# aai-institute/USFlows

Hardware: AMD Instinct MI355X
Metric: log_prob samples/sec (whole node), 32-layer 784-dim flow, batch 65536 (higher is better)
Workload: dtype f32 (GEMMs as bf16x3 split on the bf16 MFMA: 24 significant bits, fp32 accumulate); 1 GPU; BASELINE cfg2: USFlow in_dims=[784], 32 additive coupling blocks, ConditionalDenseNN[256, 256]+LeakyReLU(0.01), lu_transform=1, householder=0, affine_conjugation=False, Laplace(0,1) base; log_prob of 65536 rows per GPU (65536 over 1 GPU(s)) resident in HBM; conditioned synthetic parameters (seed 100, alpha 0.1); rows_per_gpu=65536, global_rows=65536, parallelism=dp1 (single GPU: no collective), fused_coupling=True, gemm_mode=bf16x3, merge_affine=auto -> False; probe (accepted, element-wise, L1) []

## Files before the change

### __graft_entry__.py

```python
import os
import subprocess
import sys

ROOT = os.path.dirname(os.path.abspath(__file__))
if ROOT not in sys.path:
    sys.path.insert(0, ROOT)


def build() -> None:
    csrc = os.path.join(ROOT, "usflows_amd", "csrc")
    subprocess.run(["make", "-C", csrc, "-j4"], check=True)
    import usflows_amd
    from usflows_amd import _ext
    lib = _ext.load()
    print("built:", lib.usf_build_info().decode())
    from oracle import usflows_oracle, usflows_image_oracle


def smoke() -> None:
    import torch
    from oracle import usflows_oracle as orc
    from usflows_amd.synth import build_usflow as build_flow
    assert torch.cuda.is_available(), "smoke() needs a GPU"
    spec = orc.FlowSpec(64, 4, [64, 64], householder=1, affine_conjugation=True)
    sd = orc.synth_state_dict(spec, seed=5)
    x = torch.rand(512, 64, generator=torch.Generator().manual_seed(0))
    flow = build_flow(spec, sd, device="cuda:0")
    with torch.no_grad():
        lp = flow.log_prob(x.to("cuda:0"))
        xs = flow.sample([16], seed=1)
    torch.cuda.synchronize()
    assert flow.engine() is not None and flow.engine().launch_count > 0, "HIP path did not run"
    ref = orc.flow_log_prob(orc.to_dtype(sd, torch.float64), spec, x.double())
    rel = ((lp.cpu().double() - ref).abs() / ref.abs()).max().item()
    assert rel < 1e-5, rel
    assert torch.isfinite(xs).all()
    eng = flow.engine()
    rels = {}
    for mode in ("bf16x3", "f16x2"):
        eng.gemm_mode, eng.use_planes, eng.planes_min_rows, eng.fused_min_rows = mode, True, 0, 0
        with torch.no_grad():
            lp2 = flow.log_prob(x.to("cuda:0"))
        torch.cuda.synchronize()
        assert any(p.get("planes") for p in eng._plans.values()), "planes plan was not built"
        rels[mode] = ((lp2.cpu().double() - ref).abs() / ref.abs()).max().item()
        assert rels[mode] < 1e-5, (mode, rels[mode])
    assert eng.f16_fallbacks == 0
    from oracle import usflows_image_oracle as iorc
    from usflows_amd.flows import USFlow
    from usflows_amd.networks import ConvNet2D
    dims, cond = [16, 7, 7], dict(c_in=16, c_hidden=32, num_layers=1, padding="same", kernel_size=3, normalize_layers=True, gating=True)
    torch.manual_seed(7)
    host = USFlow(torch.distributions.Laplace(torch.zeros(dims), torch.ones(dims)), dims, 2, ConvNet2D, dict(cond), householder=1,
                  affine_conjugation=True)
    with torch.no_grad():
        for m in host.modules():
            if type(m).__name__ == "LUTransform":
                D = m.L_raw.shape[0]
                m.L_raw.copy_(torch.eye(D) + 0.3 * m.L_raw.tril(-1))
                m.U_raw.copy_(0.3 * m.U_raw.triu(1) + torch.eye(D))
            if type(m).__name__ == "ScaleTransform":
                m.scale.copy_(0.5 + torch.rand(m.scale.shape))
    isd = {k: v.detach().clone() for k, v in host.state_dict().items()}
    iflow = USFlow(torch.distributions.Laplace(torch.zeros(dims, device="cuda:0"), torch.ones(dims, device="cuda:0")), dims, 2,
                   ConvNet2D, dict(cond), householder=1, affine_conjugation=True)
    iflow.load_state_dict(isd, strict=True)
    iflow = iflow.to("cuda:0")
    xi = torch.rand(300, *dims, generator=torch.Generator().manual_seed(1))
    with torch.no_grad():
        lpi = iflow.log_prob(xi.to("cuda:0"))
    torch.cuda.synchronize()
    ispec = iorc.ImageSpec(in_dims=dims, coupling_blocks=2, cond_args=dict(cond), householder=1, affine_conjugation=True)
    refi = iorc.flow_log_prob({k: v.double() for k, v in isd.items()}, ispec, xi.double())
    reli = ((lpi.cpu().double() - refi).abs() / refi.abs()).max().item()
    assert reli < 1e-5, reli
    from usflows_amd import distributions as UD
    rbase = UD.RadialDistribution(device="cpu", p=1.0, loc=0.05 * torch.randn(dims, generator=torch.Generator().manual_seed(2)),
                                  norm_distribution=UD.LogNormal(loc=torch.ones([1]) * 6, scale=torch.ones([1]) * .35, device="cpu"))
    rflow = USFlow(rbase, dims, 2, ConvNet2D, dict(cond), prior_scale=1.0, householder=1, affine_conjugation=True)
    rflow.load_state_dict(isd, strict=False)
    rsd = {k: v.detach().clone() for k, v in rflow.state_dict().items()}
    rflow = rflow.to("cuda:0")
    with torch.no_grad():
        lpr = rflow.log_prob(xi.to("cuda:0"))
    torch.cuda.synchronize()
    rspec = iorc.ImageSpec(in_dims=dims, coupling_blocks=2, cond_args=dict(cond), householder=1, affine_conjugation=True, base="radial",
                           radial_p=1.0, radial_norm="lognormal")
    refr = iorc.flow_log_prob({k: v.double() for k, v in rsd.items()}, rspec, xi.double())
    relr = ((lpr.cpu().double() - refr).abs() / refr.abs()).max().item()
    assert relr < 1e-5, relr
    print(f"smoke ok: log_prob max rel err vs fp64 oracle {rel:.2e}; planes pipeline bf16x3 {rels['bf16x3']:.2e}, "
          f"fp16x2 {rels['f16x2']:.2e}; image flow (MNIST configuration, 300 rows) vs image oracle {reli:.2e}; with the live "
          f"radial base {relr:.2e}")


if __name__ == "__main__":
    build()
    if len(sys.argv) > 1 and sys.argv[1] == "smoke":
        smoke()
```

### include/usflows_hip_internal.h

```cpp
#ifndef USFLOWS_HIP_INTERNAL_H
#define USFLOWS_HIP_INTERNAL_H

#include "usflows_hip.h"

#ifdef __cplusplus
extern "C" {
#endif

#define USF_INTERNAL_VERSION 6

int usf_internal_version(void);


int usf_linear_variant(const usf_linear_desc* d);

int usf_coupling_variant(const usf_coupling_desc* d);

int64_t usf_radial_logprob_grad_workspace(int64_t M, int64_t D);
int usf_radial_logprob_grad_f32(const float* z, int64_t ldz, const float* r, const float* g_lp, int64_t M, int64_t D, int32_t p_id,
                                const float* loc, int32_t norm, int32_t K, const float* par_a, const float* par_b,
                                const float* logits, float* g, int64_t ldg, float* d_loc, float* d_a, float* d_b, float* d_logits,
                                void* workspace, int64_t workspace_bytes, usf_stream_t stream);

int usf_radial_sample_norm_f32(float* z, int64_t ldz, int64_t M, int64_t D, int32_t p_id, const float* loc,
                               int32_t norm, int32_t K, const float* par_a, const float* par_b, const float* logits,
                               float* r_out, uint64_t seed, uint64_t offset, int64_t row_offset, usf_stream_t stream);

#define USF_FN_INTERNAL_BASE 64
#define USF_FN_COUPLING_PLANES_CTX 64
int usf_coupling_planes_ctx(const usf_coupling_planes_desc* d, const float* ctx, int64_t ctx_stride, const float* w_ctx,
                            const float* b_ctx, usf_stream_t stream);

#define USF_VCTX_MAX 32
#define USF_FN_COUPLING_VCTX 65
int usf_coupling_additive_vctx_f32(const usf_coupling_desc* d, const float* ctx, int64_t ld_ctx, int32_t ctx_dim,
                                   const float* W_ctx_t, int64_t ldw_ctx, const float* b_ctx, usf_stream_t stream);
int usf_coupling_additive_vctx_variant(const usf_coupling_desc* d, int32_t ctx_dim);

int usf_conv_ctx_wgrad_f32(const float* dy, const float* ctx, int64_t ctx_stride, int64_t B, int64_t cout, int64_t H, int64_t W,
                           int64_t ks, float* dw_ctx, usf_stream_t stream);

typedef struct usf_psum_job {
  const float* part; float* out; float* out2;
  int32_t nparts, n, mode, cin, cout, CIT, T, ntile;
  int32_t first_block, per, rows, vec4;
} usf_psum_job;
int usf_conv_wgrad_deferred_f32(const float* x, const float* dy, int64_t B, int64_t cin, int64_t cout, int64_t H, int64_t W, int64_t ks,
                                const float* in_mul, const float* pre_sub, int32_t in_act, float in_slope, float* dW, float* db,
                                float* workspace, int64_t workspace_floats, usf_psum_job* job, usf_stream_t stream);
int usf_partial_sum_jobs_f32(const usf_psum_job* jobs, const int32_t* block_job, int64_t n_blocks, usf_stream_t stream);
typedef struct usf_wgrad_job {
  unsigned char args[192];
  int32_t CIT, COT, T, blocks, lds_bytes, first_block;
} usf_wgrad_job;
int usf_conv_wgrad_plan_f32(const float* x, const float* dy, int64_t B, int64_t cin, int64_t cout, int64_t H, int64_t W, int64_t ks,
                            const float* in_mul, const float* pre_sub, int32_t in_act, float in_slope, float* dW, float* db,
                            float* workspace, int64_t workspace_floats, usf_psum_job* job, usf_wgrad_job* wjob, usf_stream_t stream);
int usf_conv_wgrad_jobs_f32(const usf_wgrad_job* jobs, const int32_t* block_job, int64_t n_blocks, int32_t CIT, int32_t COT, int32_t T,
                            int32_t lds_bytes, usf_stream_t stream);
int64_t usf_conv_wgrad_workspace(int64_t B, int64_t cin, int64_t cout, int64_t H, int64_t W, int64_t ks);
int usf_conv_wgrad_f32(const float* x, const float* dy, int64_t B, int64_t cin, int64_t cout, int64_t H, int64_t W, int64_t ks,
                       const float* in_mul, const float* pre_sub, int32_t in_act, float in_slope, float* dW, float* db,
                       float* workspace, int64_t workspace_floats, usf_stream_t stream);
int64_t usf_layernorm_channels_bwd_workspace(int64_t B, int64_t C, int64_t P);
int usf_layernorm_channels_bwd_f32(const float* x, const float* dy, float* dx, int64_t B, int64_t C, int64_t P, const float* gamma,
                                   float eps, int32_t act, float slope, float* dgamma_dbeta, float* workspace,
                                   int64_t workspace_floats, usf_stream_t stream);
int usf_gated_residual_bwd_f32(const float* dy, const float* vg, float* dvg, int64_t B, int64_t CP, usf_stream_t stream);

typedef struct usf_conv_wgrad_query {
  int64_t B, cin, cout, H, W, ks;
  int32_t masked, cus, blocks_per_cu, reserved;
} usf_conv_wgrad_query;
typedef struct usf_conv_wgrad_info {
  int32_t kernel, CIT, COT, T, rsplit, blocks, lds_bytes;
  int32_t S, base, q0, CS, nch, nacc, tab_floats;
  int32_t slots, rounds, per, rows_used, max_samples_per_wave;
  int32_t blocks_per_cu, cus, reserved;
} usf_conv_wgrad_info;
int usf_conv_wgrad_variant(const usf_conv_wgrad_query* q, usf_conv_wgrad_info* out);
typedef struct usf_ln_bwd_info {
  int32_t kernel, width, blocks, slots, rounds, per, rows_used, reserved;
} usf_ln_bwd_info;
int usf_layernorm_channels_bwd_variant(int64_t B, int64_t C, int64_t P, usf_ln_bwd_info* out);

typedef struct usf_wplanes_job {
  const float* w; int64_t out_off;
  int32_t cin, cout, ks, first_block;
} usf_wplanes_job;
int usf_conv2d_weight_planes_batch_f32(const usf_wplanes_job* jobs, const int32_t* block_job, int64_t n_blocks, void* planes_base,
                                       usf_stream_t stream);

int64_t usf_gated_tail_workspace(int64_t B, int64_t C, int64_t P);
int usf_gated_tail_bwd_f32(const float* h, const float* x, const float* dy, float* dx, float* dh, float* dvg, int64_t B, int64_t C,
                           int64_t P, const float* W, const float* bias, int32_t in_act, float in_slope, int32_t post_act,
                           float post_slope, const float* ln_gamma, const float* ln_beta, float ln_eps, float* dparams,
                           float* workspace, int64_t workspace_floats, struct usf_psum_job* job, usf_stream_t stream);

int usf_conv2d_same_gate_f32(const float* x, float* y, int64_t B, int64_t cin, int64_t cout, int64_t H, int64_t W, int64_t ks,
                             const void* w_planes, const float* gate_h, float gate_slope, const float* gate_mul,
                             const float* gate_add, usf_stream_t stream);

#define USF_CONV_ENTRY_PLAIN 0
#define USF_CONV_ENTRY_CTX 1
#define USF_CONV_ENTRY_RES 2
#define USF_CONV_ENTRY_GATE_MUL 3
#define USF_CONV_ENTRY_GATE_ADD 4
#define USF_CONV_ENTRY_GATED 5
typedef struct usf_conv_variant_query {
  int32_t entry, aligned;
  int64_t B, cin, cout, H, W, ks;
  int32_t cus, reserved;
} usf_conv_variant_query;
typedef struct usf_conv_variant {
// ... 124 lines not shown
```

### usflows_amd/_abi.py

```python
import ctypes as C

USF_ABI_VERSION = 36
USF_INTERNAL_VERSION = 6
USF_MAX_HIDDEN = 4

ACT_NONE, ACT_LEAKY_RELU, ACT_GATE = 0, 1, 2
BASE_LAPLACE, BASE_NORMAL, BASE_LPNORM1, BASE_LPNORM2, BASE_LPNORMINF, BASE_ROWSUM = 0, 1, 2, 3, 4, 5
NORM_LOGNORMAL, NORM_GAMMA, NORM_RAW_PARAMS = 0, 1, 0x100
NORM_WEIBULL, NORM_HALFNORMAL, NORM_CHI = 2, 3, 4
RADIAL_MAX_K = 64
OP_LINEAR, OP_COUPLING, OP_PACK_PLANES, OP_GEMM_PLANES, OP_COUPLING_PLANES, OP_GATED_NORM, OP_CALL = 1, 2, 5, 6, 7, 9, 10
PLANES_BF16X3, PLANES_F16X2 = 0, 1
CALL_FNS = {"usf_scale_f32": 1, "usf_channel_affine_f32": 2, "usf_layernorm_channels_f32": 3, "usf_gated_residual_f32": 4,
            "usf_masked_residual_f32": 5, "usf_pointwise_conv_f32": 6, "usf_conv2d_same_f32": 7, "usf_conv2d_same_res_f32": 8,
            "usf_base_logprob_f32": 9, "usf_radial_logprob_f32": 10, "usf_gated_tail_f32": 11, "usf_conv2d_same_ctx_f32": 12}

FN_COUPLING_PLANES_CTX = 64
FN_COUPLING_VCTX = 65
VCTX_MAX = 32

_fp = C.c_void_p


class LinearDesc(C.Structure):
    _fields_ = [
        ("A", _fp), ("lda", C.c_int64),
        ("W", _fp), ("ldw", C.c_int64),
        ("bias", _fp), ("pre_div", _fp), ("pre_sub", _fp),
        ("residual", _fp), ("ldr", C.c_int64),
        ("addend", _fp), ("ldadd", C.c_int64),
        ("post_mul", _fp),
        ("C", _fp), ("ldc", C.c_int64),
        ("M", C.c_int64), ("N", C.c_int64), ("K", C.c_int64),
        ("res_sign", C.c_float), ("slope", C.c_float),
        ("act", C.c_int32), ("reserved", C.c_int32),
        ("W_split", _fp), ("ldw_split", C.c_int64), ("split_plane_stride", C.c_int64),
        ("A_planes_out", _fp), ("ldp_out", C.c_int64), ("planes_out_stride", C.c_int64),
    ]


class CouplingDesc(C.Structure):
    _fields_ = [
        ("z", _fp), ("ldz", C.c_int64),
        ("out", _fp), ("ldo", C.c_int64),
        ("M", C.c_int64),
        ("off_pass", C.c_int64), ("n_pass", C.c_int64),
        ("off_trans", C.c_int64), ("n_trans", C.c_int64),
        ("n_hidden", C.c_int32), ("hidden", C.c_int32 * USF_MAX_HIDDEN),
        ("W_in", _fp), ("ldw_in", C.c_int64), ("b_in", _fp),
        ("W_hid", _fp * USF_MAX_HIDDEN), ("b_hid", _fp * USF_MAX_HIDDEN), ("ldw_hid", C.c_int64 * USF_MAX_HIDDEN),
        ("W_out", _fp), ("ldw_out", C.c_int64), ("b_out", _fp),
        ("context", _fp), ("W_ctx", _fp), ("b_ctx", _fp),
        ("post_sub", _fp),
        ("sign", C.c_float), ("slope", C.c_float),
        ("act", C.c_int32), ("reserved", C.c_int32),
        ("split_in", _fp), ("split_in_ld", C.c_int64), ("split_in_plane", C.c_int64),
        ("split_hid", _fp * USF_MAX_HIDDEN), ("split_hid_ld", C.c_int64), ("split_hid_plane", C.c_int64),
        ("split_out", _fp), ("split_out_ld", C.c_int64), ("split_out_plane", C.c_int64),
        ("hidden_out", _fp * USF_MAX_HIDDEN), ("ld_hidden_out", C.c_int64),
        ("gate", _fp * USF_MAX_HIDDEN), ("ld_gate", C.c_int64),
    ]


class PackPlanesDesc(C.Structure):
    _fields_ = [("src", _fp), ("ld", C.c_int64), ("M", C.c_int64), ("nkb", C.c_int64), ("idx", _fp),
                ("pre_div", _fp), ("pre_sub", _fp), ("planes", _fp), ("format", C.c_int32), ("reserved", C.c_int32), ("range_flag", _fp),
                ("src_cols", C.c_int64), ("row_weight", _fp), ("loc", _fp), ("scale", _fp), ("grad_base", C.c_int32),
                ("reserved2", C.c_int32)]


class GemmPlanesDesc(C.Structure):
    _fields_ = [("A", _fp), ("a_nkb", C.c_int64), ("a_kb0", C.c_int64), ("nk", C.c_int64),
                ("W_planes", _fp), ("ldw", C.c_int64), ("w_plane_stride", C.c_int64), ("w_rows", C.c_int64),
                ("bias", _fp), ("post_mul", _fp), ("residual", _fp),
                ("C_planes", _fp), ("c_nkb", C.c_int64), ("c_kb0", C.c_int64), ("c_kbn", C.c_int64),
                ("C_f32", _fp), ("ldc", C.c_int64), ("N", C.c_int64), ("M", C.c_int64),
                ("res_sign", C.c_float), ("slope", C.c_float), ("act", C.c_int32), ("format", C.c_int32), ("range_flag", _fp),
                ("base_tab", _fp), ("base_tab_stride", C.c_int64), ("base_part", _fp), ("base", C.c_int32), ("reserved", C.c_int32)]


class CouplingPlanesDesc(C.Structure):
    _fields_ = [("z", _fp), ("z_nkb", C.c_int64), ("M", C.c_int64),
                ("kb_p0", C.c_int64), ("nk_p", C.c_int64), ("kb_t0", C.c_int64), ("nk_t", C.c_int64),
                ("n_hidden", C.c_int32), ("hidden_padded", C.c_int32),
                ("W_in", _fp), ("ldw_in", C.c_int64), ("w_in_plane", C.c_int64), ("b_in", _fp),
                ("W_hid", _fp * 2), ("b_hid", _fp * 2), ("ldw_hid", C.c_int64), ("w_hid_plane", C.c_int64),
                ("W_out", _fp), ("ldw_out", C.c_int64), ("w_out_plane", C.c_int64), ("b_out", _fp),
                ("sign", C.c_float), ("slope", C.c_float), ("act", C.c_int32), ("format", C.c_int32),
                ("range_flag", _fp), ("hidden_out", _fp * 2), ("gate", _fp * 2)]


class MtChunk(C.Structure):
    _fields_ = [("p", _fp), ("g", _fp), ("m", _fp), ("h", _fp), ("n", C.c_int32), ("reserved", C.c_int32)]


class AdamChunk(C.Structure):
    _fields_ = [("p", _fp), ("g", _fp), ("m", _fp), ("v", _fp), ("vmax", _fp), ("n", C.c_int32), ("slot", C.c_int32)]


class GradChunk(C.Structure):
    _fields_ = [("g", _fp), ("n", C.c_int32), ("reserved", C.c_int32)]
# ... 106 lines not shown
    ]

SIZEOF_KINDS = {OP_LINEAR: LinearDesc, OP_COUPLING: CouplingDesc, 0: Op, 3: LuPrepDesc, 4: PackJob, OP_PACK_PLANES: PackPlanesDesc,
                OP_GEMM_PLANES: GemmPlanesDesc, OP_COUPLING_PLANES: CouplingPlanesDesc, 8: MtChunk, OP_GATED_NORM: GatedNormDesc,
                OP_CALL: CallDesc, 11: GradJob, 12: PsumJob, 13: GatedNormBwdDesc, 14: WgradJob, 15: WReduceJob, 16: WPlanesJob, 17: AdamChunk, 18: GradChunk,
                19: ConvVariantQuery, 20: ConvVariant, 21: ConvWgradQuery, 22: ConvWgradInfo, 23: LnBwdInfo}


PUBLIC_SYMBOLS = {
    "usf_abi_version": (C.c_int, []),
    "usf_sizeof_desc": (C.c_int, [C.c_int32]),
    "usf_last_error": (C.c_char_p, []),
    "usf_build_info": (C.c_char_p, []),
    "usf_linear_f32": (C.c_int, [C.POINTER(LinearDesc), C.c_void_p]),
    "usf_pack_planes_f32": (C.c_int, [C.POINTER(PackPlanesDesc), C.c_void_p]),
    "usf_gemm_planes_bf16x3": (C.c_int, [C.POINTER(GemmPlanesDesc), C.c_void_p]),
    "usf_coupling_planes": (C.c_int, [C.POINTER(CouplingPlanesDesc), C.c_void_p]),
    "usf_coupling_additive_f32": (C.c_int, [C.POINTER(CouplingDesc), C.c_void_p]),
    "usf_coupling_max_width": (C.c_int, []),
    "usf_coupling_padded_width": (C.c_int, [C.c_int]),
    "usf_base_logprob_f32": (C.c_int, [_fp, C.c_int64, C.c_int64, C.c_int64, C.c_int32, _fp, _fp, C.c_float,
                                       _fp, _fp, _fp, C.c_void_p]),
    "usf_base_tables_f32": (C.c_int, [C.c_int32, _fp, _fp, C.c_int64, _fp, C.c_int64, C.c_void_p]),
    "usf_base_sample_f32": (C.c_int, [_fp, C.c_int64, C.c_int64, C.c_int64, C.c_int32, _fp, _fp, C.c_uint64,
                                      C.c_uint64, C.c_int64, C.c_void_p]),
    "usf_radial_sample_f32": (C.c_int, [_fp, C.c_int64, C.c_int64, C.c_int64, C.c_int32, _fp, _fp, C.c_uint64,
                                        C.c_uint64, C.c_int64, C.c_void_p]),
    "usf_radial_logprob_f32": (C.c_int, [_fp, C.c_int64, C.c_int64, C.c_int64, C.c_int32, _fp, C.c_int32, C.c_int32, _fp, _fp, _fp,
                                         C.c_double, C.c_float, _fp, _fp, _fp, _fp, C.c_void_p]),
    "usf_variates_from_bits_f32": (C.c_int, [_fp, C.c_int64, _fp, _fp, _fp, C.c_void_p]),
    "usf_scale_f32": (C.c_int, [_fp, C.c_int64, _fp, C.c_int64, C.c_int64, C.c_int64, _fp, C.c_int32, C.c_void_p]),
    "usf_affine_coupling_apply_f32": (C.c_int, [_fp, C.c_int64, _fp, C.c_int64, _fp, C.c_int64, C.c_int64, C.c_int64,
                                                C.c_float, C.c_int32, _fp, C.c_void_p]),
    "usf_channel_affine_f32": (C.c_int, [_fp, _fp, C.c_int64, C.c_int64, C.c_int64, _fp, _fp, _fp, C.c_void_p]),
    "usf_layernorm_channels_f32": (C.c_int, [_fp, _fp, C.c_int64, C.c_int64, C.c_int64, _fp, _fp, C.c_float, C.c_int32,
                                             C.c_float, C.c_void_p]),
    "usf_gated_residual_f32": (C.c_int, [_fp, _fp, _fp, C.c_int64, C.c_int64, C.c_void_p]),
    "usf_gated_norm_rows_f32": (C.c_int, [C.POINTER(GatedNormDesc), C.c_void_p]),
    "usf_pointwise_conv_supported": (C.c_int, [C.c_int64, C.c_int64, C.c_int32]),
    "usf_pointwise_conv_f32": (C.c_int, [_fp, _fp, C.c_int64, C.c_int64, C.c_int64, C.c_int64, _fp, _fp, C.c_int32, C.c_float,
                                         C.c_int32, C.c_float, _fp, _fp, _fp, C.c_float, C.c_void_p]),
    "usf_conv2d_weight_elems": (C.c_int64, [C.c_int64, C.c_int64, C.c_int64]),
    "usf_conv2d_same_fits": (C.c_int, [C.c_int64, C.c_int64, C.c_int64, C.c_int64, C.c_int64]),
    "usf_conv2d_same_f32": (C.c_int, [_fp, _fp, C.c_int64, C.c_int64, C.c_int64, C.c_int64, C.c_int64, C.c_int64, _fp, _fp, _fp,
                                      C.c_int32, C.c_float, C.c_int32, C.c_float, _fp, C.c_int64, C.c_void_p]),
    "usf_conv2d_same_ctx_f32": (C.c_int, [_fp, _fp, C.c_int64, C.c_int64, C.c_int64, C.c_int64, C.c_int64, C.c_int64, _fp, _fp, _fp,
                                          C.c_int32, C.c_float, C.c_int32, C.c_float, _fp, C.c_int64, _fp, C.c_void_p]),
    "usf_conv2d_same_res_f32": (C.c_int, [_fp, _fp, C.c_int64, C.c_int64, C.c_int64, C.c_int64, C.c_int64, C.c_int64, _fp, _fp, _fp,
                                          C.c_int32, C.c_float, _fp, _fp, C.c_float, C.c_void_p]),
    "usf_masked_residual_f32": (C.c_int, [_fp, _fp, _fp, C.c_float, _fp, C.c_int64, C.c_int64, C.c_void_p]),
    "usf_gated_tail_supported": (C.c_int, [C.c_int64]),
    "usf_gated_tail_f32": (C.c_int, [_fp, _fp, _fp] + [C.c_int64] * 3 + [_fp, _fp, C.c_int32, C.c_float, C.c_int32, C.c_float, _fp, _fp,
                                     C.c_float, C.c_void_p]),
    "usf_conv2d_weight_planes_f32": (C.c_int, [_fp, C.c_void_p, C.c_int64, C.c_int64, C.c_int64, C.c_int32, C.c_void_p]),
    "usf_gather_cols_f32": (C.c_int, [_fp, C.c_int64, _fp, C.c_int64, C.c_int64, C.c_int64, _fp, C.c_void_p]),
    "usf_run_ops": (C.c_int, [C.POINTER(Op), C.c_int32, C.c_void_p]),
    "usf_lu_prepare_f64": (C.c_int, [C.POINTER(LuPrepDesc), C.c_void_p]),
    "usf_gemm_f64": (C.c_int, [_fp, C.c_int64, C.c_int64, C.c_int32, _fp, C.c_int64, C.c_int64, C.c_int32,
                               _fp, C.c_int64, C.c_int64, C.c_int64, C.c_int64, C.c_int64, C.c_int64,
                               C.c_double, C.c_double, C.c_int32, C.c_void_p]),
    "usf_householder_f64": (C.c_int, [_fp, _fp, C.c_int64, C.c_int64, _fp, C.c_void_p]),
    "usf_pack_weight_f32": (C.c_int, [_fp, C.c_int32, C.c_int64, C.c_int32, _fp, C.c_int64, _fp, C.c_int64,
                                      _fp, C.c_int64, _fp, C.c_int64, C.c_int64, C.c_void_p]),
    "usf_pack_weights_f32": (C.c_int, [_fp, C.c_int64, C.c_int64, C.c_int64, C.c_void_p]),
    "usf_pack_weights_t_f32": (C.c_int, [_fp, C.c_int64, C.c_int64, C.c_int64, C.c_void_p]),
    "usf_affine_prep_f32": (C.c_int, [_fp, _fp, _fp, _fp, _fp, C.c_int64, C.c_int32, C.c_int32, _fp, _fp, _fp, _fp, _fp, _fp,
                                      C.c_void_p]),
    "usf_matvec_f64": (C.c_int, [_fp, C.c_int64, C.c_int64, _fp, C.c_int64, _fp, C.c_double, _fp, _fp, C.c_void_p]),
}
INTERNAL_SYMBOLS = {
    "usf_internal_version": (C.c_int, []),
    "usf_set_tuning": (C.c_int, [C.c_char_p, C.c_int64]),
    "usf_get_tuning": (C.c_int64, [C.c_char_p, C.c_int64]),
    "usf_linear_variant": (C.c_int, [C.POINTER(LinearDesc)]),
    "usf_gemm_planes_variant": (C.c_int, [C.POINTER(GemmPlanesDesc)]),
    "usf_coupling_variant": (C.c_int, [C.POINTER(CouplingDesc)]),
    "usf_radial_logprob_grad_workspace": (C.c_int64, [C.c_int64, C.c_int64]),
    "usf_radial_logprob_grad_f32": (C.c_int, [_fp, C.c_int64, _fp, _fp, C.c_int64, C.c_int64, C.c_int32, _fp, C.c_int32, C.c_int32,
                                              _fp, _fp, _fp, _fp, C.c_int64, _fp, _fp, _fp, _fp, _fp, C.c_int64, C.c_void_p]),
    "usf_radial_sample_norm_f32": (C.c_int, [_fp, C.c_int64, C.c_int64, C.c_int64, C.c_int32, _fp, C.c_int32, C.c_int32, _fp, _fp, _fp,
                                             _fp, C.c_uint64, C.c_uint64, C.c_int64, C.c_void_p]),
    "usf_gated_norm_rows_bwd_f32": (C.c_int, [C.POINTER(GatedNormBwdDesc), C.c_void_p]),
    "usf_coupling_planes_ctx": (C.c_int, [C.POINTER(CouplingPlanesDesc), _fp, C.c_int64, _fp, _fp, C.c_void_p]),
    "usf_coupling_additive_vctx_f32": (C.c_int, [C.POINTER(CouplingDesc), _fp, C.c_int64, C.c_int32, _fp, C.c_int64, _fp, C.c_void_p]),
    "usf_coupling_additive_vctx_variant": (C.c_int, [C.POINTER(CouplingDesc), C.c_int32]),
    "usf_conv_ctx_wgrad_f32": (C.c_int, [_fp, _fp, C.c_int64, C.c_int64, C.c_int64, C.c_int64, C.c_int64, C.c_int64, _fp, C.c_void_p]),
    "usf_conv2d_same_gate_f32": (C.c_int, [_fp, _fp] + [C.c_int64] * 6 + [C.c_void_p, _fp, C.c_float, _fp, _fp, C.c_void_p]),
    "usf_conv2d_same_variant": (C.c_int, [C.POINTER(ConvVariantQuery), C.POINTER(ConvVariant)]),
    "usf_conv_wgrad_variant": (C.c_int, [C.POINTER(ConvWgradQuery), C.POINTER(ConvWgradInfo)]),
    "usf_layernorm_channels_bwd_variant": (C.c_int, [C.c_int64, C.c_int64, C.c_int64, C.POINTER(LnBwdInfo)]),
    "usf_conv_wgrad_workspace": (C.c_int64, [C.c_int64] * 6),
    "usf_conv_wgrad_f32": (C.c_int, [_fp, _fp] + [C.c_int64] * 6 + [_fp, _fp, C.c_int32, C.c_float, _fp, _fp, _fp, C.c_int64,
                                     C.c_void_p]),
    "usf_conv_wgrad_deferred_f32": (C.c_int, [_fp, _fp] + [C.c_int64] * 6 + [_fp, _fp, C.c_int32, C.c_float, _fp, _fp, _fp, C.c_int64,
                                              C.POINTER(PsumJob), C.c_void_p]),
    "usf_conv_wgrad_plan_f32": (C.c_int, [_fp, _fp] + [C.c_int64] * 6 + [_fp, _fp, C.c_int32, C.c_float, _fp, _fp, _fp, C.c_int64,
                                          C.c_void_p, C.c_void_p, C.c_void_p]),
    "usf_conv_wgrad_jobs_f32": (C.c_int, [C.c_void_p, C.c_void_p, C.c_int64, C.c_int32, C.c_int32, C.c_int32, C.c_int32, C.c_void_p]),
    "usf_partial_sum_jobs_f32": (C.c_int, [_fp, _fp, C.c_int64, C.c_void_p]),
    "usf_layernorm_channels_bwd_workspace": (C.c_int64, [C.c_int64] * 3),
    "usf_layernorm_channels_bwd_f32": (C.c_int, [_fp, _fp, _fp, C.c_int64, C.c_int64, C.c_int64, _fp, C.c_float, C.c_int32, C.c_float,
                                                 _fp, _fp, C.c_int64, C.c_void_p]),
    "usf_gated_residual_bwd_f32": (C.c_int, [_fp, _fp, _fp, C.c_int64, C.c_int64, C.c_void_p]),
    "usf_conv2d_weight_planes_batch_f32": (C.c_int, [C.c_void_p, C.c_void_p, C.c_int64, C.c_void_p, C.c_void_p]),
    "usf_gated_tail_workspace": (C.c_int64, [C.c_int64] * 3),
    "usf_gated_tail_bwd_f32": (C.c_int, [_fp] * 6 + [C.c_int64] * 3 + [_fp, _fp, C.c_int32, C.c_float, C.c_int32, C.c_float, _fp, _fp,
                                         C.c_float, _fp, _fp, C.c_int64, C.c_void_p, C.c_void_p]),
    "usf_lu_grad_finish_f64": (C.c_int, [_fp, _fp, _fp, _fp, _fp, _fp, C.c_int64, C.c_int64, _fp, _fp, C.c_void_p]),
    "usf_wgrad_f32": (C.c_int, [_fp, C.c_int64, _fp, C.c_int64, C.c_int64, C.c_int64, C.c_int64, _fp, C.c_int64,
                                C.c_float, C.c_float, C.c_int32, _fp, C.c_int64, C.c_void_p]),
    "usf_wgrad_workspace_floats": (C.c_int64, [C.c_int64, C.c_int64, C.c_int64]),
    "usf_wgrad_bias_f32": (C.c_int, [_fp, C.c_int64, _fp, C.c_int64, C.c_int64, C.c_int64, C.c_int64, _fp, C.c_int64,
                                     C.c_float, C.c_float, C.c_int32, _fp, C.c_float, C.c_float, _fp, C.c_int64, _fp]),
    "usf_wgrad_bias_ok": (C.c_int, [C.c_int64, C.c_int64, C.c_int64, C.c_int64, C.c_int64, C.c_int32]),
    "usf_wgrad_planes_f32": (C.c_int, [_fp, C.c_int64, C.c_int64, C.c_int64, _fp, C.c_int64, C.c_int64, C.c_int64, C.c_int64,
                                       C.c_int64, C.c_int64, _fp, C.c_int64, C.c_float, C.c_float, _fp, C.c_float, C.c_float,
                                       _fp, C.c_int64, _fp]),
    "usf_wgrad_blocked_f32": (C.c_int, [_fp, C.c_int64, C.c_int64, _fp, C.c_int64, C.c_int64, C.c_int64, C.c_int64, C.c_int64, _fp,
                                        C.c_int64, C.c_float, C.c_float, _fp, C.c_float, C.c_float, _fp, C.c_int64, _fp]),
    "usf_wgrad_blocked_plan_f32": (C.c_int, [_fp, C.c_int64, C.c_int64, _fp, C.c_int64, C.c_int64, C.c_int64, C.c_int64, C.c_int64, _fp,
                                             C.c_int64, C.c_float, C.c_float, _fp, C.c_float, C.c_float, _fp, C.c_int64, C.c_void_p, _fp]),
    "usf_wgrad_reduce_jobs_f32": (C.c_int, [C.c_void_p, C.c_void_p, C.c_int64, C.c_void_p]),
    "usf_base_param_grad_f32": (C.c_int, [_fp, C.c_int64, _fp, C.c_int64, C.c_int64, C.c_int32, _fp, _fp, _fp, _fp, C.c_int64, C.c_void_p]),
    "usf_mfma_probe": (C.c_int, [_fp, _fp, C.c_int64, C.c_int64, C.POINTER(C.c_double), C.c_void_p]),
    "usf_set_clock_buffer": (C.c_int, [_fp]),
    "usf_wgrad_planes_colsum_ok": (C.c_int, [C.c_int64, C.c_int64, C.c_int64]),
    "usf_wgrad_planes_workspace_floats": (C.c_int64, [C.c_int64, C.c_int64, C.c_int64]),
    "usf_wgrad_planes_ok": (C.c_int, [C.c_int64, C.c_int64, C.c_int64]),
    "usf_split_planes_f32": (C.c_int, [_fp, C.c_int64, C.c_int64, C.c_int64, _fp, C.c_int64, C.c_int64, _fp]),
    "usf_wgrad_variant": (C.c_int, [C.c_int64, C.c_int64, C.c_int64, C.c_int64, C.c_int64, C.c_int32]),
    "usf_sophiag_step_f32": (C.c_int, [C.c_void_p, C.c_int64, C.c_float, C.c_float, C.c_float, C.c_float, C.c_float, C.c_int32,
                                       C.c_void_p]),
    "usf_sophiag_hessian_f32": (C.c_int, [C.c_void_p, C.c_int64, C.c_float, C.c_float, C.c_void_p]),
    "usf_adam_step_f32": (C.c_int, [C.c_void_p, C.c_int64, C.c_void_p, C.c_int64, C.c_double, C.c_double, C.c_double, C.c_double,
                                    C.c_double, C.c_int32, C.c_void_p]),
    "usf_grad_sqnorm_partials_f32": (C.c_int, [C.c_void_p, C.c_int64, C.c_void_p, C.c_void_p]),
    "usf_grad_clip_scale_f32": (C.c_int, [C.c_void_p, C.c_int64, C.c_void_p, C.c_double, C.c_void_p]),
    "usf_colsum_f32": (C.c_int, [_fp, C.c_int64, C.c_int64, C.c_int64, _fp, C.c_float, C.c_float, _fp, C.c_int64,
                                 C.c_void_p]),
    "usf_act_grad_f32": (C.c_int, [_fp, C.c_int64, _fp, C.c_int64, C.c_int64, C.c_int64, C.c_int32, C.c_float,
                                   C.c_void_p]),
    "usf_base_logprob_grad_f32": (C.c_int, [_fp, C.c_int64, _fp, C.c_int64, C.c_int64, C.c_int32, _fp, _fp, _fp,
                                            C.c_int64, C.c_void_p]),
    "usf_grad_jobs_f32": (C.c_int, [_fp, _fp, C.c_int64, C.c_void_p]),
    "usf_affine_prep_bwd_f32": (C.c_int, [_fp, _fp, _fp, _fp, _fp, _fp, _fp, _fp, _fp, _fp, _fp, C.c_int64, C.c_int32,
                                          C.c_int32, _fp, _fp, _fp, _fp, C.c_void_p]),
}
SYMBOLS = {**PUBLIC_SYMBOLS, **INTERNAL_SYMBOLS}
```

### usflows_amd/_ext.py

```python
from __future__ import annotations

import ctypes as C
import gc
import math
import os
import struct
import threading
from typing import Optional

import torch

_HERE = os.path.dirname(os.path.abspath(__file__))
from .config import config
from ._abi import (
    USF_ABI_VERSION, USF_INTERNAL_VERSION, USF_MAX_HIDDEN, ACT_NONE, ACT_LEAKY_RELU, ACT_GATE, BASE_LAPLACE, BASE_NORMAL,
    BASE_LPNORM1, BASE_LPNORM2, BASE_LPNORMINF, BASE_ROWSUM, NORM_LOGNORMAL, NORM_GAMMA, NORM_RAW_PARAMS, NORM_WEIBULL, NORM_HALFNORMAL, NORM_CHI, RADIAL_MAX_K, OP_LINEAR,
    OP_COUPLING, OP_PACK_PLANES, OP_GEMM_PLANES, OP_COUPLING_PLANES, OP_GATED_NORM, OP_CALL, PLANES_BF16X3, PLANES_F16X2, CALL_FNS,
    FN_COUPLING_PLANES_CTX, FN_COUPLING_VCTX, VCTX_MAX,
    _fp, LinearDesc, CouplingDesc, PackPlanesDesc, GemmPlanesDesc, CouplingPlanesDesc, MtChunk, AdamChunk, GradChunk, ConvVariantQuery, ConvVariant, ConvWgradQuery, ConvWgradInfo, LnBwdInfo, CONV_ENTRIES, GatedNormDesc, GatedNormBwdDesc,
    CallDesc, _OpUnion, Op, LuPrepDesc, PackJob, PsumJob, WgradJob, WReduceJob, WPlanesJob, GradJob, SIZEOF_KINDS, PUBLIC_SYMBOLS,
    INTERNAL_SYMBOLS, SYMBOLS)

LIB_PATH = config.lib_path

_lib: Optional[C.CDLL] = None


def lib_exists() -> bool:
    return os.path.isfile(LIB_PATH)


def load() -> C.CDLL:
    global _lib
    if _lib is not None:
        return _lib
    if not lib_exists():
        raise RuntimeError(
            f"usflows_amd: HIP extension not built ({LIB_PATH} missing). Run "
            "`python -c 'import __graft_entry__ as g; g.build()'` or `make -C usflows_amd/csrc`. "
            "There is no CPU/eager fallback for the device path.")
    lib = C.CDLL(LIB_PATH)
    for name, (res, args) in SYMBOLS.items():
        fn = getattr(lib, name)
        fn.restype = res
        fn.argtypes = args
    if lib.usf_abi_version() != USF_ABI_VERSION:
        raise RuntimeError(f"usflows_amd: ABI mismatch: library {lib.usf_abi_version()} != binding {USF_ABI_VERSION}")
    if lib.usf_internal_version() != USF_INTERNAL_VERSION:
        raise RuntimeError(f"usflows_amd: internal ABI mismatch: library {lib.usf_internal_version()} != binding "
                           f"{USF_INTERNAL_VERSION}")
    for kind, st in SIZEOF_KINDS.items():
        if lib.usf_sizeof_desc(kind) != C.sizeof(st):
            raise RuntimeError(f"usflows_amd: struct layout mismatch for {st.__name__}: "
                               f"C {lib.usf_sizeof_desc(kind)} vs ctypes {C.sizeof(st)}")
    _lib = lib
    return lib


def check(rc: int, what: str = "") -> None:
    cl = getattr(_tls, "calls", None)
    if cl is not None and what.startswith("usf_") and what not in CALL_FNS:
        cl.bad = cl.bad or what
    if rc != 0:
        msg = load().usf_last_error().decode("utf-8", "replace")
        raise RuntimeError(f"usflows_amd HIP call failed ({what}, rc={rc}): {msg}")


TAPES_ENABLED = True


class Tape:
    __slots__ = ("entries", "stream", "dx")

    def __init__(self):
        self.entries = []
        self.stream = None
        self.dx = None


class _ThreadState(threading.local):

    def __init__(self):
        self.rec = []
        self.jobs = []


_tls = _ThreadState()


class record:
    def __init__(self, tape: Optional[Tape]):
        self.tape = tape

    def __enter__(self):
        _tls.rec.append(self.tape)
        return self.tape

    def __exit__(self, *exc):
        _tls.rec.pop()
        return False

# ... 791 lines not shown


def coupling_op(op, device):
    _launch("usf_coupling_additive_f32", (C.byref(op.u.coupling), current_stream(device)), op)


def mfma_probe(device, iters: int = 400, repeats: int = 5) -> dict:
    src = torch.rand(1024, device=device) + 0.5
    sink = torch.zeros(1, device=device)
    flops = C.c_double(0.0)
    times = []
    for i in range(repeats + 1):
        e0, e1 = torch.cuda.Event(enable_timing=True), torch.cuda.Event(enable_timing=True)
        e0.record()
        _launch("usf_mfma_probe", (src.data_ptr(), sink.data_ptr(), iters, 0, C.byref(flops), current_stream(device)), tape=False)
        e1.record()
        e1.synchronize()
        if i:
            times.append(e0.elapsed_time(e1))
    times.sort()
    ms = times[len(times) // 2]
    tf = flops.value / (ms * 1e-3) / 1e12
    return dict(ms=ms, tflops_bf16=tf, tflops_f32_equiv=tf / 6.0, iters=iters, launches=repeats)


class clock_meter:

    def __init__(self, device):
        self.buf = torch.zeros(2, dtype=torch.int64, device=device)

    def __enter__(self):
        check(load().usf_set_clock_buffer(self.buf.data_ptr()), "usf_set_clock_buffer")
        return self

    def __exit__(self, *exc):
        check(load().usf_set_clock_buffer(0), "usf_set_clock_buffer")
        return False

    def mhz(self):
        c, t = (int(v) for v in self.buf.cpu().tolist())
        return 100.0 * c / t if t > 0 else None


def coupling_planes_op(op, device):
    _launch("usf_coupling_planes", (C.byref(op.u.coupling_planes), current_stream(device)), op)


def coupling_planes_ctx_op(op, ctx, ctx_stride, w_ctx, b_ctx, device):
    _launch("usf_coupling_planes_ctx", (C.byref(op.u.coupling_planes), ptr(ctx), int(ctx_stride), ptr(w_ctx), ptr(b_ctx),
                                        current_stream(device)), (op, ctx, w_ctx, b_ctx))


def coupling_planes_ctx_prefix(ctx, ctx_stride, w_ctx, b_ctx) -> "Op":
    op = Op()
    op.kind = OP_CALL
    op.u.call.fn, op.u.call.n_args = FN_COUPLING_PLANES_CTX, 4
    for j, w in enumerate((ctx.data_ptr(), int(ctx_stride), w_ctx.data_ptr(), b_ctx.data_ptr())):
        op.u.call.a[j] = w
    return op


def coupling_vctx_op(op, ctx, ld_ctx, ctx_dim, w_ctx_t, ldw_ctx, b_ctx, device):
    _launch("usf_coupling_additive_vctx_f32", (C.byref(op.u.coupling), ptr(ctx), int(ld_ctx), int(ctx_dim), ptr(w_ctx_t),
                                               int(ldw_ctx), ptr(b_ctx), current_stream(device)), (op, ctx, w_ctx_t, b_ctx))


def coupling_vctx_variant(op, ctx_dim: int) -> int:
    return int(load().usf_coupling_additive_vctx_variant(C.byref(op.u.coupling), int(ctx_dim)))


def coupling_vctx_prefix(ctx, ld_ctx, ctx_dim, w_ctx_t, ldw_ctx, b_ctx) -> "Op":
    op = Op()
    op.kind = OP_CALL
    op.u.call.fn, op.u.call.n_args = FN_COUPLING_VCTX, 6
    for j, w in enumerate((ctx.data_ptr(), int(ld_ctx), int(ctx_dim), w_ctx_t.data_ptr(), int(ldw_ctx), b_ctx.data_ptr())):
        op.u.call.a[j] = w
    return op


def is_ctx_prefix(op) -> bool:
    return op.kind == OP_CALL and op.u.call.fn in (FN_COUPLING_PLANES_CTX, FN_COUPLING_VCTX)


def run_ops(ops_array, n, device=None):
    _launch("usf_run_ops", (ops_array, n, current_stream(device)), tape=False)


def lu_prepare(L_raws, U_raws, want_M=True, want_Minv=True, keep_factors=False):
    n = len(L_raws)
    D = int(L_raws[0].shape[0])
    dev = L_raws[0].device
    for t in list(L_raws) + list(U_raws):
        if t.dtype != torch.float32 or not t.is_contiguous() or tuple(t.shape) != (D, D) or t.device != dev:
            raise ValueError("lu_prepare: parameters must be contiguous [D,D] fp32 tensors on one device")
    f64 = lambda *shape: torch.empty(*shape, dtype=torch.float64, device=dev)
    tri, tri_inv, work = f64(2 * n, D, D), f64(2 * n, D, D), f64(2 * n, D, D)
    out = dict(M=f64(n, D, D) if want_M else None, Minv=f64(n, D, D) if want_Minv else None, ladj=f64(n))
    d = LuPrepDesc()
    d.n, d.D = n, D
    Lp = (C.c_void_p * n)(*[t.data_ptr() for t in L_raws])
    Up = (C.c_void_p * n)(*[t.data_ptr() for t in U_raws])
    d.L_raw, d.U_raw = Lp, Up
    d.tri, d.tri_inv, d.work = tri.data_ptr(), tri_inv.data_ptr(), work.data_ptr()
    d.M, d.Minv, d.ladj = ptr(out["M"]), ptr(out["Minv"]), out["ladj"].data_ptr()
    _launch("usf_lu_prepare_f64", (C.byref(d), current_stream(dev)), (d, Lp, Up, tri, tri_inv, work, out))
    if keep_factors:
        out["tri"], out["tri_inv"] = tri, tri_inv
    return out


def gemm_f64(A, B, Cout, *, M, N, K, lda, ldb, ldc, transA=False, transB=False, batch=1, strideA=0, strideB=0,
             strideC=0, alpha=1.0, beta=0.0, tri=0, a_off=0, b_off=0, c_off=0):
    _launch("usf_gemm_f64", (A.data_ptr() + 8 * a_off, lda, strideA, int(transA), B.data_ptr() + 8 * b_off, ldb,
                             strideB, int(transB), Cout.data_ptr() + 8 * c_off, ldc, strideC, M, N, K, batch,
                             float(alpha), float(beta), tri, current_stream(A.device)), (A, B, Cout))


def matmul_f64(A: torch.Tensor, B: torch.Tensor, transA=False, transB=False, tri=0) -> torch.Tensor:
    M = A.shape[1] if transA else A.shape[0]
    K = A.shape[0] if transA else A.shape[1]
    N = B.shape[0] if transB else B.shape[1]
    out = torch.empty(M, N, dtype=torch.float64, device=A.device)
    gemm_f64(A, B, out, M=M, N=N, K=K, lda=A.shape[1], ldb=B.shape[1], ldc=N, transA=transA, transB=transB, tri=tri)
    return out


def lu_grad_finish(dL, dU, TL, TU, c, tri, n, D, out_L, out_U):
    _launch("usf_lu_grad_finish_f64", (dL.data_ptr(), dU.data_ptr(), ptr(TL), ptr(TU), c.data_ptr(), tri.data_ptr(), n, D,
                                       out_L.data_ptr(), out_U.data_ptr(), current_stream(dL.device)), (dL, dU, TL, TU, c, tri, out_L, out_U))


def householder(w_0, vk, out=None):
    D = int(w_0.shape[0])
    if out is None:
        out = torch.empty(D, D, dtype=torch.float64, device=w_0.device)
    _launch("usf_householder_f64", (w_0.data_ptr(), vk.data_ptr(), int(vk.shape[0]), D, out.data_ptr(),
                                    current_stream(w_0.device)), (w_0, vk, out))
    return out


TILED_TRANSPOSE = True


class batch_jobs:

    def __init__(self, device, defer_grads: bool = False):
        self.device = device
        self.jobs = []
        self.defer_grads = bool(defer_grads)
        self.grad_jobs = []

    def __enter__(self):
        _tls.jobs.append(self)
        return self

    def __exit__(self, exc_type, *exc):
        _tls.jobs.pop()
        if exc_type is None:
            self.flush()
        return False

    def flush(self):
        self._flush_grads()
        jobs, self.jobs = self.jobs, []
        if not jobs:
            return
# ... 217 lines not shown
```

### usflows_amd/config.py

```python
from __future__ import annotations

import os

_HERE = os.path.dirname(os.path.abspath(__file__))


def _tune_env() -> dict:
    out = {}
    for item in os.environ.get("USFLOWS_AMD_TUNE", "").split(","):
        if "=" in item:
            k, v = item.split("=", 1)
            out[k.strip()] = v.strip()
    return out


class Config:
    _KNOBS = dict(
        planes_min_rows=8192,
        base_in_epilogue=True,
        tiny_coupling=True,
        engine_graph=False,
        save_hidden=True,
        wgrad_planes=True,
        wreduce_jobs=True,
        fused_cbwd=True,
        fused_bias=True,
        fit_prefetch=True,
        image_train=True,
        loop_list=True,
        loop_graph=True,
        radial=True,
        psum_jobs=True,
        wgrad_jobs=True,
        affine_prep=True,
        conv_res=True,
        pointwise=True,
        batch_wplanes=True,
        gated_tail_infer_max_pixels=1 << 14,
        gated_tail_max_pixels=1 << 16,
        gated_tail=True,
    )

    def __init__(self):
        self.__dict__["_over"] = {}
        for k, v in self._KNOBS.items():
            self.__dict__[k] = v
        for k, v in _tune_env().items():
            if k in self._KNOBS:
                d = self._KNOBS[k]
                self.__dict__[k] = (v not in ("0", "false", "False", "")) if isinstance(d, bool) else type(d)(v)

    def __setattr__(self, name, value):
        if name not in self._KNOBS and name not in ("gemm_mode_default",):
            raise AttributeError(f"usflows_amd.config has no knob {name!r}")
        self.__dict__[name] = value

    @property
    def lib_path(self) -> str:
        return os.environ.get("USFLOWS_AMD_LIB", os.path.join(_HERE, "csrc", "libusflows_hip.so"))

    @property
    def gemm_mode(self) -> str:
        return os.environ.get("USFLOWS_AMD_GEMM", "bf16x3")

    @property
    def planes(self):
        v = os.environ.get("USFLOWS_AMD_PLANES", "auto")
        return None if v == "auto" else v != "0"

    @property
    def merge_affine(self):
        v = os.environ.get("USFLOWS_AMD_MERGE_AFFINE", "auto")
        return True if v == "1" else (False if v == "0" else "auto")

    @property
    def train_on_device(self) -> bool:
        return os.environ.get("USFLOWS_AMD_TRAIN", "device") != "composite"

    @property
    def train_planes(self) -> bool:
        return os.environ.get("USFLOWS_AMD_TRAIN_PLANES", "1") != "0"

    @property
    def train_graph(self) -> bool:
        return os.environ.get("USFLOWS_AMD_TRAIN_GRAPH", "1") != "0"

    @staticmethod
    def set_lib(name: str, value: int) -> None:
        from . import _ext
        _ext.check(_ext.load().usf_set_tuning(name.encode(), int(value)), "usf_set_tuning")

    @staticmethod
    def get_lib(name: str, default: int = 0) -> int:
        from . import _ext
        return int(_ext.load().usf_get_tuning(name.encode(), int(default)))


config = Config()
```

### usflows_amd/csrc/usf_api.hip

```cpp
#include <stdarg.h>
#include <stdlib.h>
#include <string.h>

#include "usf_common.h"

namespace usf {

static thread_local char g_err[512] = "";

struct TuneEntry { char name[40]; long long value; };
static TuneEntry g_tune[96];
static int g_ntune = 0;
static bool g_tune_init = false;

static void tune_store(const char* name, size_t len, long long value) {
  if (len == 0 || len >= sizeof(g_tune[0].name)) return;
  for (int i = 0; i < g_ntune; ++i)
    if (strlen(g_tune[i].name) == len && strncmp(g_tune[i].name, name, len) == 0) { g_tune[i].value = value; return; }
  if (g_ntune < (int)(sizeof(g_tune) / sizeof(g_tune[0]))) {
    memcpy(g_tune[g_ntune].name, name, len);
    g_tune[g_ntune].name[len] = 0;
    g_tune[g_ntune].value = value;
    ++g_ntune;
  }
}
static void tune_init() {
  if (g_tune_init) return;
  g_tune_init = true;
  const char* e = getenv("USFLOWS_AMD_TUNE");
  while (e && *e) {
    const char* end = strchr(e, ',');
    const size_t n = end ? (size_t)(end - e) : strlen(e);
    const char* eq = (const char*)memchr(e, '=', n);
    if (eq) tune_store(e, (size_t)(eq - e), atoll(eq + 1));
    e = end ? end + 1 : nullptr;
  }
}
unsigned long long* g_clock_buffer = nullptr;
unsigned long long* clock_buffer() { return g_clock_buffer; }
long long tuning(const char* name, long long dflt) {
  tune_init();
  for (int i = 0; i < g_ntune; ++i)
    if (strcmp(g_tune[i].name, name) == 0) return g_tune[i].value;
  return dflt;
}

void set_error(const char* fmt, ...) {
  va_list ap;
  va_start(ap, fmt);
  vsnprintf(g_err, sizeof(g_err), fmt, ap);
  va_end(ap);
}

int linear_dispatch(const usf_linear_desc* d, hipStream_t stream);
int linear_variant(const usf_linear_desc* d);
int coupling_dispatch(const usf_coupling_desc* d, hipStream_t stream, const CplVctx* v = nullptr);
int coupling_variant(const usf_coupling_desc* d, int ctx_dim = 0);
int coupling_max_width();
int coupling_padded_width(int h);
int lu_grad_finish(const double* dL, const double* dU, const double* TL, const double* TU, const double* c, const double* tri,
                   int64_t n, int64_t D, float* oL, float* oU, hipStream_t stream);
int base_tables(int32_t base, const float* loc, const float* scale, int64_t D, float* tab, int64_t stride, hipStream_t stream);
int base_logprob(const float* z, int64_t ldz, int64_t M, int64_t D, int32_t base, const float* loc,
                 const float* scale, float logdet_const, const double* logdet_dev, float* logp, double* sum_out,
                 hipStream_t stream);
int base_sample(float* z, int64_t ldz, int64_t M, int64_t D, int32_t base, const float* loc, const float* scale,
                uint64_t seed, uint64_t offset, int64_t row_offset, hipStream_t stream);
int radial_sample(float* z, int64_t ldz, int64_t M, int64_t D, int32_t base, const float* loc, const float* r,
                  uint64_t seed, uint64_t offset, int64_t row_offset, hipStream_t stream);
int variates_from_bits(const uint32_t* bits, int64_t n, float* u, float* laplace, float* exponential, hipStream_t stream);
int scale(const float* x, int64_t ldx, float* y, int64_t ldy, int64_t M, int64_t D, const float* s, int32_t divide,
          hipStream_t stream);
int affine_coupling_apply(float* z, int64_t ldz, const float* t, int64_t ldt, const float* s, int64_t lds_, int64_t M,
                          int64_t n, float bound, int32_t inverse, float* logdet, hipStream_t stream);
int channel_affine(const float* x, float* y, int64_t B, int64_t C, int64_t P, const float* W, const float* pre_sub,
                   const float* bias, hipStream_t stream);
int gather_cols(const float* src, int64_t lds_, float* dst, int64_t ldd, int64_t M, int64_t n, const int32_t* idx,
                hipStream_t stream);

int pack_planes(const usf_pack_planes_desc* d, hipStream_t stream);
int gemm_planes(const usf_gemm_planes_desc* d, hipStream_t stream);
int gemm_planes_variant(const usf_gemm_planes_desc* d);
int coupling_planes(const usf_coupling_planes_desc* d, hipStream_t stream);
int coupling_planes_ctx(const usf_coupling_planes_desc* d, const float* ctx, int64_t ctx_stride, const float* w_ctx, const float* b_ctx,
                        hipStream_t stream);
int lu_prepare(const usf_lu_prep_desc* d, hipStream_t stream);
int gemm_f64(const double* A, int64_t lda, int64_t sA, int transA, const double* B, int64_t ldb, int64_t sB, int transB,
             double* C, int64_t ldc, int64_t sC, int64_t M, int64_t N, int64_t K, int64_t batch, double alpha,
             double beta, int32_t tri, hipStream_t stream);
int householder(const float* w0, const float* vk, int64_t nvs, int64_t D, double* out, hipStream_t stream);
int pack_weight(const void* src, int32_t src_is_f32, int64_t lds_, int32_t transpose, const int32_t* out_idx, int64_t n_out,
                const int32_t* in_idx, int64_t n_in, float* W, int64_t ldw, void* planes, int64_t ldp,
                int64_t plane_stride, hipStream_t stream);
int pack_jobs(const usf_pack_job* jobs, int64_t n_jobs, int64_t max_rows, int64_t max_cols, hipStream_t stream);
int pack_jobs_t(const usf_pack_job* jobs, int64_t n_jobs, int64_t max_rows, int64_t max_cols, hipStream_t stream);
int matvec_rows(const double* src, int64_t lds_, int64_t K, const int32_t* idx, int64_t n_out, const double* b,
                double alpha, float* out32, double* out64, hipStream_t stream);

int wgrad_workspace_floats(int64_t M, int64_t N, int64_t K, int64_t* out);
int wgrad_variant(int64_t M, int64_t N, int64_t K, int64_t ldy, int64_t lda, int32_t mode);
int64_t conv2d_weight_elems(int64_t cin, int64_t cout, int64_t ks);
int conv2d_same_fits(int64_t cin, int64_t cout, int64_t H, int64_t W, int64_t ks);
int conv2d_same_res(const float* x, float* y, int64_t B, int64_t cin, int64_t cout, int64_t H, int64_t W, int64_t ks,
                    const void* wplanes, const float* bias, const float* in_mul, int32_t in_act, float in_slope,
                    const float* res_x, const float* res_mul, float res_sign, hipStream_t stream);
int conv2d_same(const float* x, float* y, int64_t B, int64_t cin, int64_t cout, int64_t H, int64_t W, int64_t ks,
                const void* wplanes, const float* bias, const float* in_mul, int32_t in_act, float in_slope,
                int32_t out_act, float out_slope, const float* gate_x, int64_t gate_channels, hipStream_t stream,
                const float* ctx = nullptr, int64_t ctx_stride = 0, const float* w_ctx = nullptr);
int conv2d_same_variant(const usf_conv_variant_query* q, usf_conv_variant* out);
int conv_ctx_wgrad(const float* dy, const float* ctx, int64_t ctx_stride, int64_t B, int64_t cout, int64_t H, int64_t W, int64_t ks,
                   float* dw_ctx, hipStream_t stream);
int conv2d_same_gate(const float* x, float* y, int64_t B, int64_t cin, int64_t cout, int64_t H, int64_t W, int64_t ks,
                     const void* wplanes, const float* gate_h, float gate_slope, const float* gate_mul, const float* gate_add,
                     hipStream_t stream);
int layernorm_channels(const float* x, float* y, int64_t B, int64_t C, int64_t P, const float* gamma, const float* beta,
                       float eps, int32_t act, float slope, hipStream_t stream);
int gated_residual(const float* x, const float* vg, float* y, int64_t B, int64_t CP, hipStream_t stream);
int gated_norm_rows(const usf_gated_norm_desc* d, hipStream_t stream);
int gated_norm_rows_bwd(const usf_gated_norm_bwd_desc* d, hipStream_t stream);
int pointwise_conv_supported(int64_t cin, int64_t cout, int32_t gated);
int pointwise_conv(const float* x, float* y, int64_t B, int64_t cin, int64_t cout, int64_t P, const float* W, const float* bias,
                   int32_t in_act, float in_slope, int32_t out_act, float out_slope, const float* gate_x,
                   const float* ln_gamma, const float* ln_beta, float ln_eps, hipStream_t stream);
int masked_residual(const float* x, const float* t, const float* om, float sign, float* y, int64_t B, int64_t CP,
                    hipStream_t stream);
int64_t conv_wgrad_workspace(int64_t B, int64_t cin, int64_t cout, int64_t H, int64_t W, int64_t ks);
int conv_wgrad(const float* x, const float* dy, int64_t B, int64_t cin, int64_t cout, int64_t H, int64_t W, int64_t ks,
               const float* in_mul, const float* pre_sub, int32_t in_act, float in_slope, float* dW, float* db, float* workspace,
               int64_t workspace_floats, usf_psum_job* job, usf_wgrad_job* wjob, hipStream_t stream);
int conv_wgrad_jobs(const usf_wgrad_job* jobs, const int32_t* block_job, int64_t n_blocks, int32_t CIT, int32_t COT, int32_t T,
                    int32_t lds_bytes, hipStream_t stream);
int partial_sum_jobs(const usf_psum_job* jobs, const int32_t* block_job, int64_t n_blocks, hipStream_t stream);
int conv2d_weight_planes_batch(const usf_wplanes_job* jobs, const int32_t* block_job, int64_t n_blocks, void* planes_base,
                               hipStream_t stream);
int gated_tail_supported(int64_t C);
int64_t gated_tail_workspace(int64_t B, int64_t C, int64_t P);
int gated_tail_fwd(const float* h, const float* x, float* y, int64_t B, int64_t C, int64_t P, const float* W, const float* bias,
                   int32_t in_act, float in_slope, int32_t post_act, float post_slope, const float* gamma, const float* beta,
                   float eps, hipStream_t stream);
int gated_tail_bwd(const float* h, const float* x, const float* dy, float* dx, float* dh, float* dvg, int64_t B, int64_t C, int64_t P,
                   const float* W, const float* bias, int32_t in_act, float in_slope, int32_t post_act, float post_slope,
                   const float* gamma, const float* beta, float eps, float* dparams, float* workspace, int64_t workspace_floats,
                   usf_psum_job* job, hipStream_t stream);
int64_t layernorm_channels_bwd_workspace(int64_t B, int64_t C, int64_t P);
int layernorm_channels_bwd(const float* x, const float* dy, float* dx, int64_t B, int64_t C, int64_t P, const float* gamma, float eps,
                           int32_t act, float slope, float* dgamma, float* dbeta, float* workspace, int64_t workspace_floats,
                           hipStream_t stream);
int gated_residual_bwd(const float* dy, const float* vg, float* dvg, int64_t B, int64_t CP, hipStream_t stream);
int conv_wgrad_variant(const usf_conv_wgrad_query* q, usf_conv_wgrad_info* out);
int layernorm_channels_bwd_variant(int64_t B, int64_t C, int64_t P, usf_ln_bwd_info* out);
int conv2d_weight_planes(const float* w, void* planes, int64_t cin, int64_t cout, int64_t ks, int32_t transposed, hipStream_t stream);
int sophiag_step(const usf_mt_chunk* chunks, int64_t n_chunks, float decay, float beta1, float one_minus_beta1, float rho_bs,
                 float neg_lr, int32_t maximize, hipStream_t stream);
int sophiag_hessian(const usf_mt_chunk* chunks, int64_t n_chunks, float beta2, float one_minus_beta2, hipStream_t stream);
int adam_step(const usf_adam_chunk* chunks, int64_t n_chunks, int64_t* steps, int64_t n_slots, double lr, double beta1,
              double beta2, double eps, double weight_decay, int32_t flags, hipStream_t stream);
int grad_sqnorm_partials(const usf_grad_chunk* chunks, int64_t n_chunks, double* partials, hipStream_t stream);
int grad_clip_scale(const usf_grad_chunk* chunks, int64_t n_chunks, const double* partials, double max_norm, hipStream_t stream);
int wgrad(const float* Y, int64_t ldy, const float* A, int64_t lda, int64_t M, int64_t N, int64_t K, float* G,
          int64_t ldg, float alpha, float beta, int32_t mode, float* workspace, int64_t workspace_floats,
          hipStream_t stream, float* colsum_out = nullptr, float cs_alpha = 0.f, float cs_beta = 0.f);
int wgrad_bias_ok(int64_t M, int64_t N, int64_t K, int64_t ldy, int64_t lda, int32_t mode);
int affine_prep(const float* Lr, const float* Ur, const float* bias, const float* vk, const float* w0, int64_t n, int32_t C,
                int32_t nvs, float* M, float* Minv, float* b, float* cvec, float* ladj, float* save, hipStream_t stream);
int affine_prep_bwd(const float* save, const float* bias, const float* vk, const float* w0, const float* Minv, const float* b,
                    const float* dM, const float* dMinv, const float* db, const float* dc, const float* dladj, int64_t n,
                    int32_t C, int32_t nvs, float* dLr, float* dUr, float* dbias, float* dvk, hipStream_t stream);
// ... 13 lines not shown
                    const float* scale, float* d_loc_scale, float* workspace, int64_t workspace_floats, hipStream_t stream);
int mfma_probe(const float* src1024, float* sink, int64_t iters, int64_t blocks, double* flops_out, hipStream_t stream);
int colsum(const float* Y, int64_t ldy, int64_t M, int64_t N, float* out, float alpha, float beta, float* workspace,
           int64_t workspace_floats, hipStream_t stream);
int act_grad(float* d, int64_t ldd, const float* h, int64_t ldh, int64_t M, int64_t H, int32_t act, float slope,
             hipStream_t stream);
int base_grad(const float* z, int64_t ldz, const float* g_lp, int64_t M, int64_t D, int32_t base, const float* loc,
              const float* scale, float* g, int64_t ldg, hipStream_t stream);
int radial_logprob(const float* z, int64_t ldz, int64_t M, int64_t D, int32_t p_id, const float* loc, int32_t norm, int32_t K,
                   const float* par_a, const float* par_b, const float* logits, double logdv_const, float logdet_const,
                   const double* logdet_dev, float* logp, float* r_out, double* sum_out, hipStream_t stream);
int64_t radial_grad_workspace(int64_t M, int64_t D);
int radial_grad(const float* z, int64_t ldz, const float* r, const float* g_lp, int64_t M, int64_t D, int32_t p_id,
                const float* loc, int32_t norm, int32_t K, const float* par_a, const float* par_b, const float* logits, float* g,
                int64_t ldg, float* d_loc, float* d_a, float* d_b, float* d_logits, void* workspace, int64_t workspace_bytes,
                hipStream_t stream);
int radial_sample_norm(float* z, int64_t ldz, int64_t M, int64_t D, int32_t p_id, const float* loc, int32_t norm, int32_t K,
                       const float* par_a, const float* par_b, const float* logits, float* r_out, uint64_t seed, uint64_t offset,
                       int64_t row_offset, hipStream_t stream);

}

extern "C" {

int usf_abi_version(void) { return USF_ABI_VERSION; }
int usf_internal_version(void) { return USF_INTERNAL_VERSION; }
int usf_set_tuning(const char* name, int64_t value) {
  if (!name || !*name || strlen(name) >= sizeof(usf::g_tune[0].name)) { usf::set_error("usf_set_tuning: bad name"); return -1; }
  usf::tune_init();
  usf::tune_store(name, strlen(name), (long long)value);
  return 0;
}
int64_t usf_get_tuning(const char* name, int64_t dflt) { return name ? (int64_t)usf::tuning(name, (long long)dflt) : dflt; }
int usf_sizeof_desc(int32_t kind) {
  switch (kind) {
    case USF_OP_LINEAR: return (int)sizeof(usf_linear_desc);
    case USF_OP_COUPLING: return (int)sizeof(usf_coupling_desc);
    case 0: return (int)sizeof(usf_op);
    case 3: return (int)sizeof(usf_lu_prep_desc);
    case 4: return (int)sizeof(usf_pack_job);
    case USF_OP_PACK_PLANES: return (int)sizeof(usf_pack_planes_desc);
    case USF_OP_GEMM_PLANES: return (int)sizeof(usf_gemm_planes_desc);
    case USF_OP_COUPLING_PLANES: return (int)sizeof(usf_coupling_planes_desc);
    case 8: return (int)sizeof(usf_mt_chunk);
    case USF_OP_GATED_NORM: return (int)sizeof(usf_gated_norm_desc);
    case USF_OP_CALL: return (int)sizeof(usf_call_desc);
    case 11: return (int)sizeof(usf_grad_job);
    case 12: return (int)sizeof(usf_psum_job);
    case 13: return (int)sizeof(usf_gated_norm_bwd_desc);
    case 14: return (int)sizeof(usf_wgrad_job);
    case 15: return (int)sizeof(usf_wreduce_job);
    case 16: return (int)sizeof(usf_wplanes_job);
    case 17: return (int)sizeof(usf_adam_chunk);
    case 18: return (int)sizeof(usf_grad_chunk);
    case 19: return (int)sizeof(usf_conv_variant_query);
    case 20: return (int)sizeof(usf_conv_variant);
    case 21: return (int)sizeof(usf_conv_wgrad_query);
    case 22: return (int)sizeof(usf_conv_wgrad_info);
    case 23: return (int)sizeof(usf_ln_bwd_info);
    default: return -1;
  }
}
const char* usf_last_error(void) { return usf::g_err; }
const char* usf_build_info(void) { return "libusflows_hip gfx950 f32-mfma (" __DATE__ " " __TIME__ ")"; }

int usf_linear_f32(const usf_linear_desc* d, usf_stream_t stream) {
  return usf::linear_dispatch(d, (hipStream_t)stream);
}

int usf_linear_variant(const usf_linear_desc* d) { return usf::linear_variant(d); }

int usf_coupling_additive_f32(const usf_coupling_desc* d, usf_stream_t stream) {
  return usf::coupling_dispatch(d, (hipStream_t)stream);
}

int usf_pack_planes_f32(const usf_pack_planes_desc* d, usf_stream_t stream) { return usf::pack_planes(d, (hipStream_t)stream); }
int usf_gemm_planes_bf16x3(const usf_gemm_planes_desc* d, usf_stream_t stream) { return usf::gemm_planes(d, (hipStream_t)stream); }

int usf_coupling_planes(const usf_coupling_planes_desc* d, usf_stream_t stream) { return usf::coupling_planes(d, (hipStream_t)stream); }
int usf_coupling_planes_ctx(const usf_coupling_planes_desc* d, const float* ctx, int64_t ctx_stride, const float* w_ctx, const float* b_ctx,
                            usf_stream_t stream) {
  return usf::coupling_planes_ctx(d, ctx, ctx_stride, w_ctx, b_ctx, (hipStream_t)stream);
}
int usf_gemm_planes_variant(const usf_gemm_planes_desc* d) { return usf::gemm_planes_variant(d); }
int usf_coupling_variant(const usf_coupling_desc* d) { return usf::coupling_variant(d); }
int usf_coupling_additive_vctx_f32(const usf_coupling_desc* d, const float* ctx, int64_t ld_ctx, int32_t ctx_dim, const float* W_ctx_t,
                                   int64_t ldw_ctx, const float* b_ctx, usf_stream_t stream) {
  const usf::CplVctx v = {ctx, ld_ctx, (int)ctx_dim, W_ctx_t, ldw_ctx, b_ctx};
  return usf::coupling_dispatch(d, (hipStream_t)stream, &v);
}
int usf_coupling_additive_vctx_variant(const usf_coupling_desc* d, int32_t ctx_dim) {
  return usf::coupling_variant(d, (ctx_dim > 0 && ctx_dim <= USF_VCTX_MAX) ? (int)ctx_dim : 0);
}
int usf_coupling_max_width(void) { return usf::coupling_max_width(); }
int usf_coupling_padded_width(int h) { return usf::coupling_padded_width(h); }

int usf_base_tables_f32(int32_t base, const float* loc, const float* scale, int64_t D, float* tab, int64_t stride, usf_stream_t stream) {
  return usf::base_tables(base, loc, scale, D, tab, stride, (hipStream_t)stream);
}
int usf_base_logprob_f32(const float* z, int64_t ldz, int64_t M, int64_t D, int32_t base, const float* loc,
                         const float* scale, float logdet_const, const double* logdet_dev, float* logp, double* sum_out,
                         usf_stream_t stream) {
  return usf::base_logprob(z, ldz, M, D, base, loc, scale, logdet_const, logdet_dev, logp, sum_out, (hipStream_t)stream);
}

int usf_base_sample_f32(float* z, int64_t ldz, int64_t M, int64_t D, int32_t base, const float* loc,
                        const float* scale, uint64_t seed, uint64_t offset, int64_t row_offset, usf_stream_t stream) {
  return usf::base_sample(z, ldz, M, D, base, loc, scale, seed, offset, row_offset, (hipStream_t)stream);
}

int usf_radial_sample_f32(float* z, int64_t ldz, int64_t M, int64_t D, int32_t base, const float* loc, const float* r,
                          uint64_t seed, uint64_t offset, int64_t row_offset, usf_stream_t stream) {
  return usf::radial_sample(z, ldz, M, D, base, loc, r, seed, offset, row_offset, (hipStream_t)stream);
}

int usf_variates_from_bits_f32(const uint32_t* bits, int64_t n, float* u, float* laplace, float* exponential,
                               usf_stream_t stream) {
  return usf::variates_from_bits(bits, n, u, laplace, exponential, (hipStream_t)stream);
}

int usf_scale_f32(const float* x, int64_t ldx, float* y, int64_t ldy, int64_t M, int64_t D, const float* s,
                  int32_t divide, usf_stream_t stream) {
  return usf::scale(x, ldx, y, ldy, M, D, s, divide, (hipStream_t)stream);
}

int usf_affine_coupling_apply_f32(float* z, int64_t ldz, const float* t, int64_t ldt, const float* s, int64_t lds, int64_t M,
                                  int64_t n, float bound, int32_t inverse, float* logdet, usf_stream_t stream) {
  return usf::affine_coupling_apply(z, ldz, t, ldt, s, lds, M, n, bound, inverse, logdet, (hipStream_t)stream);
}

int usf_channel_affine_f32(const float* x, float* y, int64_t B, int64_t C, int64_t P, const float* W,
                           const float* pre_sub, const float* bias, usf_stream_t stream) {
  return usf::channel_affine(x, y, B, C, P, W, pre_sub, bias, (hipStream_t)stream);
}

int usf_gather_cols_f32(const float* src, int64_t lds_, float* dst, int64_t ldd, int64_t M, int64_t n,
                        const int32_t* idx, usf_stream_t stream) {
  return usf::gather_cols(src, lds_, dst, ldd, M, n, idx, (hipStream_t)stream);
}

int usf_lu_prepare_f64(const usf_lu_prep_desc* d, usf_stream_t stream) { return usf::lu_prepare(d, (hipStream_t)stream); }

int usf_gemm_f64(const double* A, int64_t lda, int64_t strideA, int32_t transA, const double* B, int64_t ldb,
                 int64_t strideB, int32_t transB, double* C, int64_t ldc, int64_t strideC, int64_t M, int64_t N,
                 int64_t K, int64_t batch, double alpha, double beta, int32_t tri, usf_stream_t stream) {
  return usf::gemm_f64(A, lda, strideA, transA, B, ldb, strideB, transB, C, ldc, strideC, M, N, K, batch, alpha, beta,
                       tri, (hipStream_t)stream);
}

int usf_lu_grad_finish_f64(const double* dL, const double* dU, const double* TL, const double* TU, const double* c,
                           const double* tri, int64_t n, int64_t D, float* dL_out, float* dU_out, usf_stream_t stream) {
  return usf::lu_grad_finish(dL, dU, TL, TU, c, tri, n, D, dL_out, dU_out, (hipStream_t)stream);
}
int usf_householder_f64(const float* w_0, const float* vk, int64_t nvs, int64_t D, double* out, usf_stream_t stream) {
  return usf::householder(w_0, vk, nvs, D, out, (hipStream_t)stream);
}

int usf_pack_weight_f32(const void* src, int32_t src_is_f32, int64_t ld_src, int32_t transpose, const int32_t* out_idx, int64_t n_out,
                        const int32_t* in_idx, int64_t n_in, float* W, int64_t ldw, void* planes, int64_t ld_planes,
                        int64_t plane_stride, usf_stream_t stream) {
  return usf::pack_weight(src, src_is_f32, ld_src, transpose, out_idx, n_out, in_idx, n_in, W, ldw, planes, ld_planes, plane_stride,
                          (hipStream_t)stream);
}

int usf_pack_weights_f32(const usf_pack_job* jobs, int64_t n_jobs, int64_t max_rows, int64_t max_cols,
                         usf_stream_t stream) {
// ... 269 lines not shown
  auto F = [&](int i) { float f; uint32_t u = (uint32_t)a[i]; memcpy(&f, &u, 4); return f; };
  auto Dbl = [&](int i) { double d; uint64_t u = a[i]; memcpy(&d, &u, 8); return d; };
  static const int nargs[] = {0, 8, 8, 10, 5, 7, 16, 17, 16, 11, 17, 15, 18};
  static_assert(sizeof(nargs) / sizeof(nargs[0]) == USF_FN_CONV2D_SAME_CTX + 1, "one entry per public function id");
  static_assert(USF_FN_CONV2D_SAME_CTX < USF_FN_INTERNAL_BASE, "a public function id ran into the internal range");
  if (c->fn < 1 || c->fn > USF_FN_CONV2D_SAME_CTX || c->n_args != nargs[c->fn]) {
    usf::set_error("usf_run_ops: call op with unknown function %d or %d arguments", c->fn, c->n_args);
    return -2;
  }
  switch (c->fn) {
    case USF_FN_SCALE: return usf_scale_f32(P(0), I(1), Q(2), I(3), I(4), I(5), P(6), J(7), stream);
    case USF_FN_CHANNEL_AFFINE: return usf_channel_affine_f32(P(0), Q(1), I(2), I(3), I(4), P(5), P(6), P(7), stream);
    case USF_FN_LAYERNORM_CHANNELS: return usf_layernorm_channels_f32(P(0), Q(1), I(2), I(3), I(4), P(5), P(6), F(7), J(8), F(9), stream);
    case USF_FN_GATED_RESIDUAL: return usf_gated_residual_f32(P(0), P(1), Q(2), I(3), I(4), stream);
    case USF_FN_MASKED_RESIDUAL: return usf_masked_residual_f32(P(0), P(1), P(2), F(3), Q(4), I(5), I(6), stream);
    case USF_FN_POINTWISE_CONV:
      return usf_pointwise_conv_f32(P(0), Q(1), I(2), I(3), I(4), I(5), P(6), P(7), J(8), F(9), J(10), F(11), P(12), P(13), P(14), F(15), stream);
    case USF_FN_GATED_TAIL:
      return usf_gated_tail_f32(P(0), P(1), Q(2), I(3), I(4), I(5), P(6), P(7), J(8), F(9), J(10), F(11), P(12), P(13), F(14), stream);
    case USF_FN_CONV2D_SAME:
      return usf_conv2d_same_f32(P(0), Q(1), I(2), I(3), I(4), I(5), I(6), I(7), (const void*)(uintptr_t)a[8], P(9), P(10), J(11), F(12),
                                 J(13), F(14), P(15), I(16), stream);
    case USF_FN_CONV2D_SAME_CTX:
      return usf_conv2d_same_ctx_f32(P(0), Q(1), I(2), I(3), I(4), I(5), I(6), I(7), (const void*)(uintptr_t)a[8], P(9), P(10), J(11),
                                     F(12), J(13), F(14), P(15), I(16), P(17), stream);
    case USF_FN_CONV2D_SAME_RES: {
      const int rc = usf_conv2d_same_res_f32(P(0), Q(1), I(2), I(3), I(4), I(5), I(6), I(7), (const void*)(uintptr_t)a[8], P(9), P(10), J(11),
                                             F(12), P(13), P(14), F(15), stream);
      if (rc == 1) usf::set_error("usf_run_ops: recorded usf_conv2d_same_res_f32 call is not served by the fused form any more");
      return rc;
    }
    case USF_FN_BASE_LOGPROB:
      return usf_base_logprob_f32(P(0), I(1), I(2), I(3), J(4), P(5), P(6), F(7), reinterpret_cast<const double*>((uintptr_t)a[8]), Q(9),
                                  reinterpret_cast<double*>((uintptr_t)a[10]), stream);
    case USF_FN_RADIAL_LOGPROB:
      return usf_radial_logprob_f32(P(0), I(1), I(2), I(3), J(4), P(5), J(6), J(7), P(8), P(9), P(10), Dbl(11), F(12),
                                    reinterpret_cast<const double*>((uintptr_t)a[13]), Q(14), Q(15),
                                    reinterpret_cast<double*>((uintptr_t)a[16]), stream);
  }
#undef P
#undef Q
#undef I
#undef J
  return -2;
}

int usf_run_ops(const usf_op* ops, int32_t n_ops, usf_stream_t stream) {
  if (n_ops < 0 || (n_ops > 0 && !ops)) { usf::set_error("usf_run_ops: bad op list"); return -1; }
  for (int32_t i = 0; i < n_ops; ++i) {
    int rc;
    switch (ops[i].kind) {
      case USF_OP_LINEAR: rc = usf::linear_dispatch(&ops[i].u.linear, (hipStream_t)stream); break;
      case USF_OP_COUPLING: rc = usf::coupling_dispatch(&ops[i].u.coupling, (hipStream_t)stream); break;
      case USF_OP_PACK_PLANES: rc = usf::pack_planes(&ops[i].u.pack_planes, (hipStream_t)stream); break;
      case USF_OP_GEMM_PLANES: rc = usf::gemm_planes(&ops[i].u.gemm_planes, (hipStream_t)stream); break;
      case USF_OP_COUPLING_PLANES: rc = usf::coupling_planes(&ops[i].u.coupling_planes, (hipStream_t)stream); break;
      case USF_OP_GATED_NORM: rc = usf::gated_norm_rows(&ops[i].u.gated_norm, (hipStream_t)stream); break;
      case USF_OP_CALL:
        if (ops[i].u.call.fn == USF_FN_COUPLING_PLANES_CTX) {
          const usf_call_desc* c = &ops[i].u.call;
          if (c->n_args != 4 || i + 1 >= n_ops || ops[i + 1].kind != USF_OP_COUPLING_PLANES) {
            usf::set_error("usf_run_ops: op %d (USF_FN_COUPLING_PLANES_CTX) needs 4 arguments and a USF_OP_COUPLING_PLANES op behind it", i);
            return -2;
          }
          rc = usf::coupling_planes_ctx(&ops[i + 1].u.coupling_planes, reinterpret_cast<const float*>((uintptr_t)c->a[0]), (int64_t)c->a[1],
                                        reinterpret_cast<const float*>((uintptr_t)c->a[2]), reinterpret_cast<const float*>((uintptr_t)c->a[3]),
                                        (hipStream_t)stream);
          ++i;
          break;
        }
        if (ops[i].u.call.fn == USF_FN_COUPLING_VCTX) {
          const usf_call_desc* c = &ops[i].u.call;
          if (c->n_args != 6 || i + 1 >= n_ops || ops[i + 1].kind != USF_OP_COUPLING) {
            usf::set_error("usf_run_ops: op %d (USF_FN_COUPLING_VCTX) needs 6 arguments and a USF_OP_COUPLING op behind it", i);
            return -2;
          }
          const usf::CplVctx v = {reinterpret_cast<const float*>((uintptr_t)c->a[0]), (int64_t)c->a[1], (int)(int64_t)c->a[2],
                                  reinterpret_cast<const float*>((uintptr_t)c->a[3]), (int64_t)c->a[4],
                                  reinterpret_cast<const float*>((uintptr_t)c->a[5])};
          rc = usf::coupling_dispatch(&ops[i + 1].u.coupling, (hipStream_t)stream, &v);
          ++i;
          break;
        }
        rc = run_call(&ops[i].u.call, stream);
        break;
      default: usf::set_error("usf_run_ops: op %d has unknown kind %d", i, ops[i].kind); return -2;
    }
    if (rc != 0) return rc;
  }
  return 0;
}

}
```

### usflows_amd/csrc/usf_coupling_planes.hip

```cpp
#include <stdlib.h>

#include "usf_common.h"

namespace usf {

typedef __bf16 cp_bf16x8 __attribute__((ext_vector_type(8)));
typedef _Float16 cp_f16x8 __attribute__((ext_vector_type(8)));
#define USF_CP_F16_GUARD 65000.0f
#ifndef USF_CP_ADDR32
#define USF_CP_ADDR32 1
#endif

__device__ __forceinline__ void cp_pin(unsigned& off) { asm("" : "+v"(off)); }
template <class V> __device__ __forceinline__ V cp_load(const void* uniform, unsigned off) {
  return *reinterpret_cast<const V*>(reinterpret_cast<const char*>(uniform) + off);
}
template <class V> __device__ __forceinline__ void cp_store(void* uniform, unsigned off, const V v) {
  *reinterpret_cast<V*>(reinterpret_cast<char*>(uniform) + off) = v;
}

__device__ __forceinline__ float max_with_product(float x, float sx) {
  float r;
  asm("v_max_f32 %0, %1, %2" : "=v"(r) : "v"(x), "v"(sx));
  return r;
}

template <int NPL> struct CPlanes;
template <> struct CPlanes<3> {
  typedef cp_bf16x8 vec;
  static __device__ __forceinline__ f32x4 mfma(vec a, vec b, f32x4 c) { return __builtin_amdgcn_mfma_f32_16x16x32_bf16(a, b, c, 0, 0, 0); }
  static __device__ __forceinline__ void split(const f32x4 x0, const f32x4 x1, vec (&o)[3]) {
#pragma unroll
    for (int j = 0; j < 8; ++j) {
      const float x = (j < 4) ? x0[j & 3] : x1[j & 3];
      const __bf16 h = (__bf16)x;
      const float r = x - (float)h;
      const __bf16 m = (__bf16)r;
      o[0][j] = h; o[1][j] = m; o[2][j] = (__bf16)(r - (float)m);
    }
  }
  static __device__ __forceinline__ void split1(const float x, const int j, vec (&o)[3]) {
    const __bf16 h = (__bf16)x;
    const float r = x - (float)h;
    const __bf16 m = (__bf16)r;
    o[0][j] = h; o[1][j] = m; o[2][j] = (__bf16)(r - (float)m);
  }
  static __device__ __forceinline__ void mm(f32x4& acc, const vec (&w)[3], const vec (&a)[3]) {
    acc = mfma(w[2], a[0], acc); acc = mfma(w[1], a[1], acc); acc = mfma(w[0], a[2], acc);
    acc = mfma(w[1], a[0], acc); acc = mfma(w[0], a[1], acc); acc = mfma(w[0], a[0], acc);
  }
};
template <> struct CPlanes<2> {
  typedef cp_f16x8 vec;
  static __device__ __forceinline__ f32x4 mfma(vec a, vec b, f32x4 c) { return __builtin_amdgcn_mfma_f32_16x16x32_f16(a, b, c, 0, 0, 0); }
  static __device__ __forceinline__ void split(const f32x4 x0, const f32x4 x1, vec (&o)[2]) {
#pragma unroll
    for (int j = 0; j < 8; ++j) {
      const float x = (j < 4) ? x0[j & 3] : x1[j & 3];
      const _Float16 h = (_Float16)x;
      o[0][j] = h; o[1][j] = (_Float16)(x - (float)h);
    }
  }
  static __device__ __forceinline__ void split1(const float x, const int j, vec (&o)[2]) {
    const _Float16 h = (_Float16)x;
    o[0][j] = h; o[1][j] = (_Float16)(x - (float)h);
  }
  static __device__ __forceinline__ void mm(f32x4& acc, const vec (&w)[2], const vec (&a)[2]) {
    acc = mfma(w[1], a[0], acc); acc = mfma(w[0], a[1], acc); acc = mfma(w[0], a[0], acc);
  }
};

struct CplPArgs {
  char* z; int z_nkb, npanels, M;
  int kb_p0, nk_p, kb_t0, nk_t;
  const char* Win; int64_t ld_in, pl_in; const float* b_in;
  const char* Whid[2]; int64_t ld_hid, pl_hid; const float* b_hid[2];
  const char* Wout; int64_t ld_out, pl_out; const float* b_out;
  float sign, slope; int act;
  int act_max;
  int32_t* range_flag;
  int descend;
  unsigned long long* dbg;
  char* hout[2]; const char* gate[2];
  const float* ctx; int ctx_stride; const float* w_ctx; const float* b_ctx;
};

#ifdef USF_STAMP
#define CSTAMP(v) unsigned long long v = __builtin_amdgcn_s_memtime(); __builtin_amdgcn_sched_barrier(0)
#else
#define CSTAMP(v)
#endif

template <int NPL, int NH, int MODE = 0, bool CTX = false>
__global__ __launch_bounds__(512, 2) void coupling_planes_kernel(const CplPArgs p) {
  typedef CPlanes<NPL> PT;
  typedef typename PT::vec vec8;
  constexpr int T = 16;
  constexpr int HP = 16 * T;
  constexpr int KS = T / 2;
  constexpr int NT = 512;
  constexpr int SLOTS = NPL * 4 * HP;
  constexpr int NST = SLOTS / NT;
  constexpr int NPP = NST / NPL;
  constexpr int NC = HP / 8;
  constexpr int NPR = (NPL == 3) ? 6 : 3;
#ifndef USF_CP_AHEAD
#define USF_CP_AHEAD 3
#endif
  constexpr int AHEAD = USF_CP_AHEAD;
  __shared__ __attribute__((aligned(16))) float lds[2][SLOTS * 4];

  const int tid = threadIdx.x;
  const int lane = tid & 63;
  constexpr bool A32 = USF_CP_ADDR32 != 0;
  const int wave = A32 ? __builtin_amdgcn_readfirstlane(tid >> 6) : (tid >> 6);
  const int lj = lane & 15, lg = lane >> 4;
  unsigned loff = (unsigned)lane * 16u;
  unsigned goff = (unsigned)lg * 16u;
  const int panel = (p.descend ? (int)(gridDim.x - 1 - blockIdx.x) : (int)blockIdx.x) * 8 + wave;
  const int panc = min(panel, p.npanels - 1);
  const bool live = panel < p.npanels;
  const bool live_z = CTX ? (live && 16 * panel + lj < p.M) : live;
  const f32x4 zero4 = {0.f, 0.f, 0.f, 0.f};
  constexpr unsigned CHB = NPL * 1024u;
  const size_t zbase = ((size_t)panc * p.z_nkb) * CHB + (size_t)lane * 16;
  char* const zrow = p.z + ((size_t)panc * p.z_nkb) * CHB;
  auto k_off = [&](int64_t ld) { return 2u * ((unsigned)(tid >> 2) * (unsigned)ld + 8u * (unsigned)(tid & 3)); };
  auto n_off = [&](int64_t ld) { return 2u * ((unsigned)(tid / NC) * (unsigned)ld + 8u * (unsigned)(tid % NC)); };

  int kdst[NPP];
  unsigned krow[NPP];
#pragma unroll
  for (int i = 0; i < NPP; ++i) {
    const int idx = tid + NT * i;
    const int r = idx >> 2, c = idx & 3;
    kdst[i] = 4 * (c * HP + (r ^ (2 * c)));
    krow[i] = (unsigned)r;
  }
  auto issue_k = [&](const char* W, int64_t ld, int64_t pl, int k0, unsigned& off, f32x4 (&st)[NST]) {
    if constexpr (A32) cp_pin(off);
#pragma unroll
    for (int q = 0; q < NPL; ++q)
#pragma unroll
      for (int i = 0; i < NPP; ++i) {
        if constexpr (A32)
          st[q * NPP + i] = cp_load<f32x4>(W + 2 * (q * pl + (int64_t)((NT / 4) * i) * ld + k0), off);
        else
          st[q * NPP + i] = *reinterpret_cast<const f32x4*>(W + 2 * (q * pl + (int64_t)krow[i] * ld + k0 + 8 * ((tid + NT * i) & 3)));
      }
  };
  auto store_k = [&](int buf, const f32x4 (&st)[NST]) {
#pragma unroll
    for (int q = 0; q < NPL; ++q)
#pragma unroll
      for (int i = 0; i < NPP; ++i) *reinterpret_cast<f32x4*>(&lds[buf][q * 16 * HP + kdst[i]]) = st[q * NPP + i];
  };
  auto n_rc = [&](int i, int& r, int& c) { const int idx = tid + NT * i; r = idx / NC; c = idx % NC; };
  auto issue_n = [&](const char* W, int64_t ld, int64_t pl, int n0, unsigned& off, f32x4 (&st)[NST]) {
    if constexpr (A32) cp_pin(off);
#pragma unroll
    for (int q = 0; q < NPL; ++q)
#pragma unroll
      for (int i = 0; i < NPP; ++i) {
        if constexpr (A32) {
          st[q * NPP + i] = cp_load<f32x4>(W + 2 * (q * pl + (int64_t)(n0 + (NT / NC) * i) * ld), off);
        } else {
          int r, c; n_rc(i, r, c);
          st[q * NPP + i] = *reinterpret_cast<const f32x4*>(W + 2 * (q * pl + (int64_t)(n0 + r) * ld + 8 * c));
        }
      }
  };
  auto store_n = [&](int buf, const f32x4 (&st)[NST]) {
#pragma unroll
    for (int q = 0; q < NPL; ++q)
#pragma unroll
      for (int i = 0; i < NPP; ++i) {
        int r, c; n_rc(i, r, c);
// ... 101 lines not shown
#pragma unroll
      for (int ks = 0; ks < KS; ++ks) {
        const vec8 hv = A32 ? cp_load<vec8>(p.gate[l] + (hrow + (size_t)ks * CHB), loff)
                            : *reinterpret_cast<const vec8*>(p.gate[l] + hbase + (size_t)ks * CHB);
#pragma unroll
        for (int t = 0; t < 4; ++t) {
          X[2 * ks][t] = gate_apply(X[2 * ks][t], (float)hv[t], p.slope);
          X[2 * ks + 1][t] = gate_apply(X[2 * ks + 1][t], (float)hv[4 + t], p.slope);
        }
      }
      return;
    }
    if (p.act_max) {
#pragma unroll
      for (int ht = 0; ht < T; ++ht) {
#pragma unroll
        for (int t = 0; t < 4; ++t) X[ht][t] = max_with_product(X[ht][t], X[ht][t] * p.slope);
        guard(X[ht]);
      }
      return;
    }
#pragma unroll
    for (int ht = 0; ht < T; ++ht) {
#pragma unroll
      for (int t = 0; t < 4; ++t) X[ht][t] = act_apply(X[ht][t], p.act, p.slope);
      guard(X[ht]);
    }
  };
  auto save_hidden = [&](int l, int ks, const vec8 (&x)[NPL]) {
    if (MODE != 0 && live) {
      if constexpr (A32) cp_pin(loff);
#pragma unroll
      for (int q = 0; q < NPL; ++q) {
        if constexpr (A32) cp_store<vec8>(p.hout[l] + (hrow + (size_t)ks * CHB + q * 1024), loff, x[q]);
        else *reinterpret_cast<vec8*>(p.hout[l] + hbase + (size_t)ks * CHB + q * 1024) = x[q];
      }
    }
  };
  activate(X1, 0);
  CSTAMP(c1);

  auto hidden_layer = [&](f32x4 (&Xin)[T], f32x4 (&Xout)[T], int l) {
    vec8 xc[NPL], xn[NPL];
    PT::split(Xin[0], Xin[1], xc);
#pragma unroll
    for (int ks = 0; ks < KS; ++ks) {
      save_hidden(l, ks, xc);
      const int buf = g & 1;
      const bool last = (ks + 1 == KS);
      const bool next_is_hidden = (l + 2 < NH);
      if (!last) issue_k(p.Whid[l], p.ld_hid, p.pl_hid, (ks + 1) * 32, koff_hid, st);
      else if (next_is_hidden) issue_k(p.Whid[l + 1], p.ld_hid, p.pl_hid, 0, koff_hid, st);
      else issue_n(p.Wout, p.ld_out, p.pl_out, 0, noff, st);
      mfma_slab(buf, Xout, xc);
      if (!last) PT::split(Xin[2 * ks + 2], Xin[2 * ks + 3], xn);
      CP_PIN_SLAB(NST, (NPL == 3) ? 5 : 3);
      __builtin_amdgcn_sched_barrier(0);
      if (!last || next_is_hidden) store_k(buf ^ 1, st); else store_n(buf ^ 1, st);
      if (!last) {
#pragma unroll
        for (int q = 0; q < NPL; ++q) xc[q] = xn[q];
      }
      __syncthreads();
      ++g;
    }
    activate(Xout, l + 1);
  };
  if (NH >= 2) {
#pragma unroll
    for (int t = 0; t < T; ++t) X2[t] = bias4(p.b_hid[0], t);
    hidden_layer(X1, X2, 0);
  }
  if (NH >= 3) {
#pragma unroll
    for (int t = 0; t < T; ++t) X1[t] = bias4(p.b_hid[1], t);
    hidden_layer(X2, X1, 1);
  }

  CSTAMP(c2);
  auto output_layer = [&](f32x4 (&X)[T]) {
    vec8 xp[KS][NPL];
#pragma unroll
    for (int ks = 0; ks < KS; ++ks) { PT::split(X[2 * ks], X[2 * ks + 1], xp[ks]); save_hidden(NH - 1, ks, xp[ks]); }
    vec8 res[NPL];
    f32x4 bo[2];
    auto issue_res = [&](int nt) {
      if constexpr (A32) { cp_pin(loff); cp_pin(goff); }
#pragma unroll
      for (int q = 0; q < NPL; ++q) {
        if constexpr (A32) res[q] = cp_load<vec8>(zrow + ((size_t)(p.kb_t0 + nt) * CHB + q * 1024), loff);
        else res[q] = *reinterpret_cast<const vec8*>(p.z + zbase + (size_t)(p.kb_t0 + nt) * CHB + q * 1024);
      }
#pragma unroll
      for (int u = 0; u < 2; ++u) {
        if constexpr (A32) bo[u] = cp_load<f32x4>(p.b_out + nt * 32 + 16 * u, goff);
        else bo[u] = *reinterpret_cast<const f32x4*>(p.b_out + nt * 32 + 16 * u + 4 * lg);
      }
    };
    auto epilogue = [&](int nt, const auto& ac, const auto& rs) {
      f32x4 v[2];
#pragma unroll
      for (int u = 0; u < 2; ++u) {
#pragma unroll
        for (int e = 0; e < 4; ++e) {
          float r = (float)rs[0][4 * u + e] + (float)rs[1][4 * u + e];
          if (NPL == 3) r = r + (float)rs[NPL - 1][4 * u + e];
          v[u][e] = __builtin_fmaf(p.sign, ac[u][e], r);
        }
        guard(v[u]);
      }
      vec8 o[NPL];
      PT::split(v[0], v[1], o);
      if (live_z) {
        if constexpr (A32) cp_pin(loff);
#pragma unroll
        for (int q = 0; q < NPL; ++q) {
          if constexpr (A32) cp_store<vec8>(zrow + ((size_t)(p.kb_t0 + nt) * CHB + q * 1024), loff, o[q]);
          else *reinterpret_cast<vec8*>(p.z + zbase + (size_t)(p.kb_t0 + nt) * CHB + q * 1024) = o[q];
        }
      }
    };
    issue_res(0);
    auto block = [&](int nt) {
      const int buf = g & 1;
      issue_n(p.Wout, p.ld_out, p.pl_out, min(nt + 1, p.nk_t - 1) * 32, noff, st);
      f32x4 acc[2] = {bo[0], bo[1]};
#pragma unroll
      for (int ks = 0; ks < KS; ++ks) {
        const int x = 2 * ((4 * ks + lg) & 7);
#pragma unroll
        for (int u = 0; u < 2; ++u) {
          const float* wf = &lds[buf][4 * ((4 * ks + lg) * 32 + u * 16 + (lj ^ x))];
          vec8 w[NPL];
#pragma unroll
          for (int q = 0; q < NPL; ++q) w[q] = *reinterpret_cast<const vec8*>(wf + 4 * (q * NC * 32));
          PT::mm(acc[u], w, xp[ks]);
        }
      }
      __builtin_amdgcn_sched_group_barrier(0x100, NPL * AHEAD, 0);
#pragma unroll
      for (int i = 0; i < 2 * KS; ++i) {
        __builtin_amdgcn_sched_group_barrier(0x008, NPR, 0);
        if (i + AHEAD < 2 * KS) __builtin_amdgcn_sched_group_barrier(0x100, NPL, 0);
        if (i < NST + NPL + 2) __builtin_amdgcn_sched_group_barrier(0x020, 1, 0);
      }
      __builtin_amdgcn_sched_barrier(0);
      store_n(buf ^ 1, st);
      epilogue(nt, acc, res);
      issue_res(min(nt + 1, p.nk_t - 1));
      __syncthreads();
      ++g;
    };
    for (int nt = 0; nt < p.nk_t; ++nt) block(nt);
  };
  if (NH == 2) output_layer(X2); else output_layer(X1);
#ifdef USF_STAMP
  CSTAMP(c3);
  if (p.dbg && lane == 0) {
    unsigned long long* o = p.dbg + (size_t)((blockIdx.x % 2048) * 8 + wave) * 4;
    o[0] = c1 - c0; o[1] = c2 - c1; o[2] = c3 - c2; o[3] = 1;
  }
#endif
  if (NPL == 2 && p.range_flag && bad && live && (16 * panel + lj) < p.M) atomicOr(p.range_flag, 1);
#undef CP_PIN_SLAB
}



#ifdef USF_STAMP
unsigned long long* g_cdbg = nullptr;
#endif

int coupling_planes_ctx(const usf_coupling_planes_desc* d, const float* ctx, int64_t ctx_stride, const float* w_ctx,
                        const float* b_ctx, hipStream_t stream) {
  if (!d) { set_error("usf_coupling_planes: null descriptor"); return -1; }
  if (ctx) {
    if (d->act == USF_ACT_GATE) { set_error("usf_coupling_planes_ctx: USF_ACT_GATE takes no context (the context enters no data gradient)"); return -2; }
    if (ctx_stride != 0 && ctx_stride != 1) { set_error("usf_coupling_planes_ctx: ctx_stride must be 0 or 1 (got %lld)", (long long)ctx_stride); return -2; }
    if (!w_ctx || !b_ctx || !aligned16(w_ctx) || !aligned16(b_ctx)) {
      set_error("usf_coupling_planes_ctx: w_ctx / b_ctx must be [256] fp32 vectors, 16-byte aligned");
      return -2;
    }
  }
  if (d->M < 0 || d->M > 0x7fffffff || d->z_nkb <= 0 || d->n_hidden < 1 || d->n_hidden > 3 || d->nk_p <= 0 || d->nk_t <= 0 ||
      d->kb_p0 < 0 || d->kb_t0 < 0 || d->kb_p0 + d->nk_p > d->z_nkb || d->kb_t0 + d->nk_t > d->z_nkb) {
    set_error("usf_coupling_planes: bad sizes / block ranges");
    return -2;
  }
  if (d->M == 0) return 0;
  if (d->format != USF_PLANES_BF16X3 && d->format != USF_PLANES_F16X2) { set_error("usf_coupling_planes: unknown format %d", d->format); return -2; }
  if (!d->z || !d->W_in || !d->W_out || !d->b_in || !d->b_out) { set_error("usf_coupling_planes: null pointer"); return -1; }
  for (int i = 0; i + 1 < d->n_hidden; ++i)
    if (!d->W_hid[i] || !d->b_hid[i]) { set_error("usf_coupling_planes: hidden layer %d missing", i); return -1; }
  if (d->hidden_padded != 256) { set_error("usf_coupling_planes: weights must be padded to a hidden width of 256 (got %d)", d->hidden_padded); return -2; }
  if (d->ldw_in < 32 * d->nk_p || (d->n_hidden > 1 && d->ldw_hid < 256) || d->ldw_out < 256 || (d->ldw_in & 7) || (d->ldw_hid & 7) ||
      (d->ldw_out & 7) || !aligned16(d->z) || !aligned16(d->W_in) || !aligned16(d->W_out) || !aligned16(d->b_in) || !aligned16(d->b_out)) {
    set_error("usf_coupling_planes: weight-image contract violated (ldw_in >= 32 nk_p, ldw_hid / ldw_out >= 256, multiples of 8, 16-byte aligned)");
    return -2;
  }
  const int64_t npl = d->format == USF_PLANES_F16X2 ? 2 : 3;
  const int64_t npanels = (d->M + 15) / 16;
  if (2 * npl * d->w_in_plane >= (1LL << 40)) { set_error("usf_coupling_planes: operand too large"); return -3; }
  {
    const int64_t lim = 1LL << 32, chb = npl * 1024;
    const bool z_big = d->z_nkb >= lim / chb || npanels * d->z_nkb * chb >= lim;
    const bool h_big = (d->hidden_out[0] || d->hidden_out[1]) && npanels * 8 * chb >= lim;
    auto w_big = [&](int64_t ld, int64_t plane, int64_t rows) {
      return ld < 0 || plane < 0 || ld >= lim / (2 * rows) || plane >= lim / (2 * npl);
    };
    if (z_big || h_big || w_big(d->ldw_in, d->w_in_plane, 256) || (d->n_hidden > 1 && w_big(d->ldw_hid, d->w_hid_plane, 256)) ||
        w_big(d->ldw_out, d->w_out_plane, 32 * d->nk_t)) {
      set_error("usf_coupling_planes: a buffer of 4 GiB or more (z: %lld panels x %lld blocks x %lld bytes; weights: ld %lld / %lld / %lld)",
                (long long)npanels, (long long)d->z_nkb, (long long)chb, (long long)d->ldw_in, (long long)d->ldw_hid, (long long)d->ldw_out);
      return -3;
    }
  }
  CplPArgs a;
  a.z = reinterpret_cast<char*>(d->z); a.z_nkb = (int)d->z_nkb; a.npanels = (int)npanels; a.M = (int)d->M;
  a.kb_p0 = (int)d->kb_p0; a.nk_p = (int)d->nk_p; a.kb_t0 = (int)d->kb_t0; a.nk_t = (int)d->nk_t;
  a.Win = reinterpret_cast<const char*>(d->W_in); a.ld_in = d->ldw_in; a.pl_in = d->w_in_plane; a.b_in = d->b_in;
  for (int i = 0; i < 2; ++i) {
    const bool used = i + 1 < d->n_hidden;
    a.Whid[i] = reinterpret_cast<const char*>(used ? d->W_hid[i] : d->W_in);
    a.b_hid[i] = used ? d->b_hid[i] : d->b_in;
  }
  a.ld_hid = d->ldw_hid; a.pl_hid = d->w_hid_plane;
  a.Wout = reinterpret_cast<const char*>(d->W_out); a.ld_out = d->ldw_out; a.pl_out = d->w_out_plane; a.b_out = d->b_out;
  a.sign = d->sign; a.slope = d->slope; a.act = d->act; a.range_flag = d->range_flag;
  a.act_max = (d->act == USF_ACT_LEAKY_RELU && d->slope >= 0.0f && d->slope <= 1.0f && !__builtin_signbit(d->slope) &&
               tuning("coupling_act_max", 1) != 0) ? 1 : 0;
  a.descend = (int)tuning("coupling_descend", 1);
  a.ctx = ctx; a.ctx_stride = (int)ctx_stride; a.w_ctx = w_ctx; a.b_ctx = b_ctx;
  a.dbg = nullptr;
#ifdef USF_STAMP
  a.dbg = g_cdbg;
#endif
  const dim3 grid((unsigned)((npanels + 7) / 8));
  const bool want_h = d->hidden_out[0] != nullptr || d->hidden_out[1] != nullptr;
  const bool gated = d->act == USF_ACT_GATE;
  if (d->act != USF_ACT_NONE && d->act != USF_ACT_LEAKY_RELU && !gated) { set_error("usf_coupling_planes: bad act %d", d->act); return -2; }
  for (int i = 0; i < 2; ++i) { a.hout[i] = nullptr; a.gate[i] = nullptr; }
  if (want_h || gated) {
    if (npl != 3 || d->n_hidden > 2) { set_error("usf_coupling_planes: hidden_out / USF_ACT_GATE need the bf16x3 format and n_hidden <= 2"); return -2; }
    if (gated && !want_h) { set_error("usf_coupling_planes: USF_ACT_GATE needs hidden_out (the gradients at the hidden pre-activations)"); return -2; }
    for (int i = 0; i < d->n_hidden; ++i) {
      if (!d->hidden_out[i] || !aligned16(d->hidden_out[i]) || (gated && (!d->gate[i] || !aligned16(d->gate[i])))) {
        set_error("usf_coupling_planes: hidden_out[l] (and gate[l] with USF_ACT_GATE) must be set for every hidden layer, 16-byte aligned");
        return -2;
      }
      a.hout[i] = reinterpret_cast<char*>(d->hidden_out[i]);
      a.gate[i] = reinterpret_cast<const char*>(gated ? d->gate[i] : nullptr);
    }
    const dim3 block(512);
#define USF_CPT(NH_, MODE_) hipLaunchKernelGGL((coupling_planes_kernel<3, NH_, MODE_>), grid, block, 0, stream, a)
#define USF_CPTC(NH_) hipLaunchKernelGGL((coupling_planes_kernel<3, NH_, 1, true>), grid, block, 0, stream, a)
    if (gated) { if (d->n_hidden == 1) USF_CPT(1, 2); else USF_CPT(2, 2); }
    else if (ctx) { if (d->n_hidden == 1) USF_CPTC(1); else USF_CPTC(2); }
    else { if (d->n_hidden == 1) USF_CPT(1, 1); else USF_CPT(2, 1); }
#undef USF_CPTC
#undef USF_CPT
    return check_launch("usf_coupling_planes");
  }
  const dim3 block(512);
#define USF_CPL(NPL_, NH_) hipLaunchKernelGGL((coupling_planes_kernel<NPL_, NH_>), grid, block, 0, stream, a)
#define USF_CPLC(NPL_, NH_) hipLaunchKernelGGL((coupling_planes_kernel<NPL_, NH_, 0, true>), grid, block, 0, stream, a)
  if (ctx) {
    if (npl == 2) {
      switch (d->n_hidden) { case 1: USF_CPLC(2, 1); break; case 2: USF_CPLC(2, 2); break; default: USF_CPLC(2, 3); break; }
    } else {
      switch (d->n_hidden) { case 1: USF_CPLC(3, 1); break; case 2: USF_CPLC(3, 2); break; default: USF_CPLC(3, 3); break; }
    }
  } else if (npl == 2) {
    switch (d->n_hidden) { case 1: USF_CPL(2, 1); break; case 2: USF_CPL(2, 2); break; default: USF_CPL(2, 3); break; }
  } else {
    switch (d->n_hidden) { case 1: USF_CPL(3, 1); break; case 2: USF_CPL(3, 2); break; default: USF_CPL(3, 3); break; }
  }
#undef USF_CPLC
#undef USF_CPL
  return check_launch("usf_coupling_planes");
}

int coupling_planes(const usf_coupling_planes_desc* d, hipStream_t stream) { return coupling_planes_ctx(d, nullptr, 0, nullptr, nullptr, stream); }

}
```

### usflows_amd/csrc/usf_planes.hip

```cpp
#include <stdlib.h>

#include <type_traits>

#include "usf_common.h"

namespace usf {

typedef __bf16 bf16x8 __attribute__((ext_vector_type(8)));
typedef _Float16 f16x8 __attribute__((ext_vector_type(8)));
typedef unsigned u32x4 __attribute__((ext_vector_type(4)));
#define USF_F16_GUARD 65000.0f
#define USF_PL_LOAD_A(ptr) (*(ptr))
#define USF_PL_STORE_C(v, ptr) (*(ptr) = (v))

template <int NPL> struct Planes;
template <> struct Planes<3> {
  typedef bf16x8 vec;
  static __device__ __forceinline__ f32x4 mfma(vec a, vec b, f32x4 c) { return __builtin_amdgcn_mfma_f32_16x16x32_bf16(a, b, c, 0, 0, 0); }
  static __device__ __forceinline__ void split(const float (&x)[8], vec (&o)[3]) {
#pragma unroll
    for (int j = 0; j < 8; ++j) {
      const __bf16 h = (__bf16)x[j];
      const float r = x[j] - (float)h;
      const __bf16 m = (__bf16)r;
// ... 120 lines not shown
#pragma unroll
    for (int u = 0; u < 8; ++u) {
      const int l = 32 * kb + 16 * (u >> 2) + 4 * lg + (u & 3);
      const int c = t_idx[l];
      float v = 0.f;
      if (c >= 0 && row_live) {
        v = tile[lj * S + c];
        if (has_div) v = v / t_div[l];
        if (has_sub) v = v - t_sub[l];
      }
      x[u] = v;
    }
    if (NPL == 2) {
#pragma unroll
      for (int u = 0; u < 8; ++u) bad = bad || !(fabsf(x[u]) < USF_F16_GUARD);
    }
    typename PT::vec o[NPL];
    PT::split(x, o);
    char* out = dst + ((int64_t)((int64_t)p * nkb + kb) * NPL) * 1024 + lane * 16;
#pragma unroll
    for (int q = 0; q < NPL; ++q) *reinterpret_cast<typename PT::vec*>(out + q * 1024) = o[q];
  }
  if (NPL == 2 && range_flag && bad) atomicOr(range_flag, 1);
}

int pack_planes(const usf_pack_planes_desc* d, hipStream_t stream) {
  if (!d) { set_error("usf_pack_planes_f32: null descriptor"); return -1; }
  if (d->M < 0 || d->nkb <= 0 || d->M > 0x7fffffff || d->nkb > 0x7fffff || d->ld < 1) { set_error("usf_pack_planes_f32: bad sizes"); return -2; }
  if (d->M == 0) return 0;
  if (!d->src || !d->idx || !d->planes) { set_error("usf_pack_planes_f32: null pointer"); return -1; }
  if (!aligned16(d->planes)) { set_error("usf_pack_planes_f32: planes must be 16-byte aligned"); return -2; }
  if (d->format != USF_PLANES_BF16X3 && d->format != USF_PLANES_F16X2) { set_error("usf_pack_planes_f32: unknown format %d", d->format); return -2; }
  const int64_t npanels = (d->M + 15) / 16;
  const int64_t chunks = npanels * d->nkb;
  const int64_t blocks = (chunks + 3) / 4;
  if (blocks > 0x7fffffffLL) { set_error("usf_pack_planes_f32: grid too large"); return -3; }
  if (d->grad_base != 0) {
    if (d->src_cols <= 0 || !d->row_weight || !d->loc || !d->scale || d->format != USF_PLANES_BF16X3 ||
        (d->grad_base != 1 + USF_BASE_LAPLACE && d->grad_base != 1 + USF_BASE_NORMAL)) {
      set_error("usf_pack_planes_f32: grad_base needs src_cols, row_weight, loc, scale, the bf16x3 format and a Laplace / Normal base");
      return -2;
    }
  }
  const int rows_env = (int)tuning("pack_rows", 1);
  const size_t lds = ((size_t)16 * (size_t)(d->src_cols + 1) + (size_t)3 * 32 * (size_t)d->nkb) * sizeof(float);
  if (d->src_cols > 0 && d->src_cols <= d->ld && lds <= 65536 && (rows_env || d->grad_base != 0)) {
    const int vec = (aligned16(d->src) && (d->ld & 3) == 0) ? 1 : 0;
    char* out = reinterpret_cast<char*>(d->planes);
    const int wide = (int)tuning("pack_wide", 1);
#define USF_PPR(NPL_, GRAD_, NT_) hipLaunchKernelGGL((pack_planes_rows_kernel<NPL_, GRAD_, NT_>), dim3((unsigned)npanels), dim3(NT_), lds, stream, \
                             d->src, d->ld, (int)d->M, (int)d->nkb, (int)d->src_cols, d->idx, d->pre_div, d->pre_sub, out, d->range_flag,  \
                             d->row_weight, d->loc, d->scale, (int)d->grad_base, vec)
#define USF_PPW(NPL_, GRAD_) do { if (wide) USF_PPR(NPL_, GRAD_, 512); else USF_PPR(NPL_, GRAD_, 256); } while (0)
    if (d->grad_base != 0) USF_PPW(3, true);
    else if (d->format == USF_PLANES_F16X2) USF_PPW(2, false);
    else USF_PPW(3, false);
#undef USF_PPW
#undef USF_PPR
    return check_launch("usf_pack_planes_f32");
  }
  if (d->grad_base != 0) { set_error("usf_pack_planes_f32: grad_base needs 16 (src_cols + 1) floats to fit 64 KB of LDS"); return -2; }
  if (d->format == USF_PLANES_F16X2)
    hipLaunchKernelGGL(pack_planes_kernel<2>, dim3((unsigned)blocks), dim3(256), 0, stream, d->src, d->ld, (int)d->M, (int)npanels,
                       (int)d->nkb, d->idx, d->pre_div, d->pre_sub, reinterpret_cast<char*>(d->planes), d->range_flag);
  else
    hipLaunchKernelGGL(pack_planes_kernel<3>, dim3((unsigned)blocks), dim3(256), 0, stream, d->src, d->ld, (int)d->M, (int)npanels,
                       (int)d->nkb, d->idx, d->pre_div, d->pre_sub, reinterpret_cast<char*>(d->planes), d->range_flag);
  return check_launch("usf_pack_planes_f32");
}

struct PlArgs {
  const char* A; const char* Wp; const float* bias; const float* post_mul;
  const char* R; char* Cp; float* Cf;
  int64_t ldc, plane_stride;
  int ldwp, wrows;
  int M, npanels;
  int a_nkb, a_kb0, nk;
  int c_nkb, c_kb0, c_kbn;
  int N, nbm, nbn, nvb;
  float res_sign, slope; int act;
  int32_t* range_flag;
  int skip_dead;
  const float* b_tab; float* b_part; int b_stride; int b_base;
  unsigned long long* clk;
  unsigned long long* dbg;
  unsigned long long* span;
};

template <int NPL, int TN, bool F32OUT>
__global__ __launch_bounds__(512, 2) void gemm_planes_kernel(const PlArgs p) {
  typedef Planes<NPL> PT;
  typedef typename PT::vec vec8;
  constexpr int NT = 512;
  constexpr int BN = TN * 32;
  constexpr int FT = 2 * TN;
  constexpr unsigned CHB = NPL * 1024u;
  constexpr int CS = BN;
  constexpr int NSLOT = NPL * 4 * BN;
  constexpr int NWV = (NSLOT + NT - 1) / NT;
  constexpr int STG = NPL * 4 * CS * 4;
  constexpr int NB = 3;
  static_assert(NWV * NT - NSLOT <= NSLOT, "surplus threads wrap once");
  __shared__ __attribute__((aligned(16))) float wring[NB * STG];

  const int tid0 = threadIdx.x;
#ifdef USF_STAMP
  if (p.span && tid0 == 0) atomicMin(p.span, __builtin_amdgcn_s_memrealtime());
#endif
  unsigned long long clk_c0 = 0, clk_r0 = 0;
#ifndef USF_NO_CLOCK
  if (p.clk) { clk_c0 = __builtin_amdgcn_s_memtime(); clk_r0 = __builtin_amdgcn_s_memrealtime(); }
#endif

  for (int bid = blockIdx.x; bid < p.nvb; bid += gridDim.x) {
  int tid = tid0;
  asm volatile("" : "+v"(tid));
  const int lane = tid & 63;
  const int wave = tid >> 6;
  const int lj = lane & 15, lg = lane >> 4;
  const int xcd = bid & 7;
  const int seq = bid >> 3;
  const int pg = (seq / p.nbn) * 8 + xcd;
  const int bn = seq % p.nbn;
  if (pg >= p.nbm) continue;
  if (bid != (int)blockIdx.x) __syncthreads();
  const int n0 = bn * BN;
  int pw[2];
  pw[0] = pg * 16 + wave * 2;
  pw[1] = pw[0] + 1;

  bool dead = false;
  if (p.skip_dead && bn == p.nbn - 1 && n0 + BN <= p.wrows) {
    const int spr = 4 * p.nk;
    const int nscan = NPL * 16 * spr;
    const char* const wz = p.Wp + 2 * ((int64_t)(n0 + BN - 16) * p.ldwp);
    unsigned nz = 0;
    for (int e0 = tid; e0 < nscan; e0 += 4 * NT) {
      u32x4 v[4];
#pragma unroll
      for (int i = 0; i < 4; ++i) {
        const int e = min(e0 + i * NT, nscan - 1);
        const int pl = e / (16 * spr), rem = e - pl * (16 * spr);
        const int r = rem / spr, c = rem - r * spr;
        v[i] = *reinterpret_cast<const u32x4*>(wz + 2 * (pl * p.plane_stride + (int64_t)r * p.ldwp + 8 * c));
      }
#pragma unroll
      for (int i = 0; i < 4; ++i) nz |= v[i][0] | v[i][1] | v[i][2] | v[i][3];
    }
    dead = __builtin_amdgcn_readfirstlane(__syncthreads_or(nz != 0)) == 0;
  }
  auto tile = [&](auto dead_c) {
  unsigned aoff[2];
#pragma unroll
  for (int b = 0; b < 2; ++b)
    aoff[b] = ((unsigned)min(pw[b], p.npanels - 1) * (unsigned)p.a_nkb + (unsigned)p.a_kb0) * CHB + (unsigned)lane * 16u;
  auto issue_a = [&](int kb, vec8 (&dst)[2][NPL]) {
#pragma unroll
    for (int b = 0; b < 2; ++b)
#pragma unroll
      for (int q = 0; q < NPL; ++q)
        dst[b][q] = USF_PL_LOAD_A(reinterpret_cast<const vec8*>(p.A + (aoff[b] + (unsigned)kb * CHB + (unsigned)q * 1024u)));
  };

  unsigned wsrc[NWV];
  int wdst[NWV];
#pragma unroll
  for (int i = 0; i < NWV; ++i) {
    const int idx = tid + NT * i;
    const int idc = (idx < NSLOT) ? idx : idx - NSLOT;
    const int pl = idc / (4 * BN), rem = idc % (4 * BN);
    const int r = rem >> 2, ch = rem & 3;
    wsrc[i] = (unsigned)(2 * (pl * p.plane_stride + (int64_t)min(n0 + r, p.wrows - 1) * p.ldwp + 8 * ch));
// ... 132 lines not shown
      else __builtin_amdgcn_sched_group_barrier(0x100, 2 * NPL, 0);
      if (pr == MID + 1) {
        __builtin_amdgcn_sched_group_barrier(0x008, 2 * NPR, 0);
        __builtin_amdgcn_sched_group_barrier(0x020, NWV, 0);
        __builtin_amdgcn_sched_group_barrier(0x008, 2 * NPR, 0);
      } else if (DEAD && pr == NP - 1) {
        __builtin_amdgcn_sched_group_barrier(0x008, 2 * NPR, 0);
      } else {
        __builtin_amdgcn_sched_group_barrier(0x008, 4 * NPR, 0);
      }
    }
    __builtin_amdgcn_sched_barrier(0);
    LSTAMP(l4);
    LACC(0, l0, l1); LACC(1, l1, l2); LACC(2, l2, l3); LACC(3, l3, l4);
  };
  PSTAMP(t1);
    int s = 0, ring = 0;
    for (; s + 2 <= nslab; s += 2) {
      slab(dead_c, s, ring, pa, pb, fr, f2);
      ring = (ring == 2) ? 0 : ring + 1;
      if (NP & 1) slab(dead_c, s + 1, ring, pb, pa, f2, fr); else slab(dead_c, s + 1, ring, pb, pa, fr, f2);
      ring = (ring == 2) ? 0 : ring + 1;
    }
    if (s < nslab) slab(dead_c, s, ring, pa, pb, fr, f2);
  PSTAMP(t2);

  bool bad = false;
  if (p.act == USF_ACT_LEAKY_RELU) {
#pragma unroll
    for (int ft = 0; ft < FT; ++ft)
#pragma unroll
      for (int b = 0; b < 2; ++b)
#pragma unroll
        for (int j = 0; j < 4; ++j) acc[ft][b][j] = act_apply(acc[ft][b][j], USF_ACT_LEAKY_RELU, p.slope);
  }
  if (F32OUT) {
    const bool vec_ok = ((p.ldc & 3) == 0) && ((reinterpret_cast<uintptr_t>(p.Cf) & 15u) == 0);
#pragma unroll
    for (int b = 0; b < 2; ++b) {
      const int row = 16 * pw[b] + lj;
      float bsum = 0.f;
#pragma unroll
      for (int ft = 0; ft < FT; ++ft) {
        const int col = n0 + 16 * ft + 4 * lg;
        f32x4 v = acc[ft][b];
        if (p.post_mul) v = v * *reinterpret_cast<const f32x4*>(p.post_mul + min(col, p.wrows - 4));
        if (p.b_part) {
          const float* t = p.b_tab + min(col, p.b_stride - 4);
          const f32x4 bl = *reinterpret_cast<const f32x4*>(t);
          const f32x4 bi = *reinterpret_cast<const f32x4*>(t + p.b_stride);
          const f32x4 bc = *reinterpret_cast<const f32x4*>(t + 2 * p.b_stride);
#pragma unroll
          for (int j = 0; j < 4; ++j) {
            const float d = (v[j] - bl[j]) * bi[j];
            const float term = (p.b_base == USF_BASE_LAPLACE) ? bc[j] - fabsf(d) : bc[j] - 0.5f * d * d;
            bsum += (col + j < p.N) ? term : 0.f;
          }
        }
        if (NPL == 2 && row < p.M && col < p.N) {
#pragma unroll
          for (int j = 0; j < 4; ++j) bad = bad || (col + j < p.N && !(fabsf(v[j]) < 3.0e38f));
        }
        if (p.Cf != nullptr && row < p.M && col < p.N) {
          float* dst = p.Cf + (int64_t)row * p.ldc + col;
          if (vec_ok && col + 3 < p.N) {
            *reinterpret_cast<f32x4*>(dst) = v;
          } else {
#pragma unroll
            for (int j = 0; j < 4; ++j)
              if (col + j < p.N) dst[j] = v[j];
          }
        }
      }
      if (p.b_part) {
        bsum += __shfl_xor(bsum, 16);
        bsum += __shfl_xor(bsum, 32);
        if (lg == 0 && row < p.M) p.b_part[(int64_t)row * 8 + bn] = bsum;
      }
    }
  } else {
#pragma unroll
    for (int t = 0; t < TN; ++t) {
      const int kbo = bn * TN + t;
#pragma unroll
      for (int b = 0; b < 2; ++b) {
        if (kbo < p.c_kbn && pw[b] < p.npanels) {
          const size_t off = (((size_t)pw[b] * p.c_nkb + (p.c_kb0 + kbo)) * NPL) * 1024 + (size_t)lane * 16;
          float x[8];
#pragma unroll
          for (int u = 0; u < 8; ++u) x[u] = acc[2 * t + (u >> 2)][b][u & 3];
          if (p.R) {
            vec8 r[NPL];
#pragma unroll
            for (int q = 0; q < NPL; ++q) r[q] = *reinterpret_cast<const vec8*>(p.R + off + q * 1024);
#pragma unroll
            for (int u = 0; u < 8; ++u) {
              float rv = (float)r[0][u] + (float)r[1][u];
              if (NPL == 3) rv = rv + (float)r[NPL - 1][u];
              x[u] = rv + p.res_sign * x[u];
            }
          }
          if (NPL == 2) {
#pragma unroll
            for (int u = 0; u < 8; ++u) bad = bad || (16 * pw[b] + lj < p.M && !(fabsf(x[u]) < USF_F16_GUARD));
          }
          vec8 o[NPL];
          PT::split(x, o);
#ifdef USF_NOSTORE
          if (o[0][0] == (decltype(o[0][0] + o[0][0]))1234.5f && o[1][1] == (decltype(o[0][0] + o[0][0]))77.f)
#endif
          {
#pragma unroll
            for (int q = 0; q < NPL; ++q) USF_PL_STORE_C(o[q], reinterpret_cast<vec8*>(p.Cp + off + q * 1024));
          }
        }
      }
    }
  }
  if (NPL == 2 && p.range_flag && bad) atomicOr(p.range_flag, 1);
#ifdef USF_STAMP
  PSTAMP(t3);
  if (p.dbg && lane == 0) {
    unsigned long long* o = p.dbg + (size_t)((bid % 2048) * 8 + wave) * 8;
    o[0] = t1 - t0; o[1] = t2 - t1; o[2] = t3 - t2; o[3] = t3 - t0; o[4] = 1; o[5] = __builtin_amdgcn_s_memrealtime() - rt0;
    o[6] = rt0; o[7] = __builtin_amdgcn_s_memrealtime();
#if USF_STAMP >= 2
    unsigned long long* o2 = p.dbg + 16384 * 8 + (size_t)((bid % 2048) * 8 + wave) * 8;
    for (int i = 0; i < 4; ++i) o2[i] = ph[i];
#endif
  }
#endif
  };
  if (dead) tile(std::true_type()); else tile(std::false_type());
#undef USF_MM
  }
#ifdef USF_STAMP
  if (p.span && tid0 == 0) atomicMax(p.span + 1, __builtin_amdgcn_s_memrealtime());
#endif
#ifndef USF_NO_CLOCK
  if (p.clk && tid0 == 0) {
    atomicAdd(p.clk, __builtin_amdgcn_s_memtime() - clk_c0);
    atomicAdd(p.clk + 1, __builtin_amdgcn_s_memrealtime() - clk_r0);
  }
#endif
}

#ifdef USF_STAMP
unsigned long long* g_pdbg = nullptr;
unsigned long long* g_pspan = nullptr;
#endif

template <int NPL, int TN>
static int launch_planes(PlArgs a, bool f32out, hipStream_t stream) {
  constexpr int BN = TN * 32;
  a.nbm = (a.npanels + 15) / 16;
  a.nbn = f32out ? (a.N + BN - 1) / BN : (a.c_kbn + TN - 1) / TN;
  int64_t grid = (((int64_t)a.nbm + 7) / 8) * 8 * a.nbn;
  if (grid > 0x7fffffffLL) { set_error("usf_gemm_planes: grid too large"); return -3; }
  a.nvb = (int)grid;
  const int persist = (int)tuning("planes_persist", 1);
  int cus = device_cu_count();
  cus = (cus / 8) * 8 > 0 ? (cus / 8) * 8 : 8;
  if (persist && grid > cus) grid = cus;
  if (f32out) hipLaunchKernelGGL((gemm_planes_kernel<NPL, TN, true>), dim3((unsigned)grid), dim3(512), 0, stream, a);
  else hipLaunchKernelGGL((gemm_planes_kernel<NPL, TN, false>), dim3((unsigned)grid), dim3(512), 0, stream, a);
  return check_launch("usf_gemm_planes");
}

int gemm_planes_tn(int64_t nblk) {
  const int64_t pad5 = (nblk + 4) / 5 * 5 - nblk, pad4 = (nblk + 3) / 4 * 4 - nblk;
  return pad4 < pad5 ? 4 : 5;
}

int gemm_planes_variant(const usf_gemm_planes_desc* d) {
  if (!d || d->M <= 0) return 0;
  const bool f32out = d->C_f32 != nullptr || d->base_part != nullptr;
  const int64_t nblk = f32out ? (d->N + 31) / 32 : d->c_kbn;
  if (nblk <= 0) return 0;
  return 5000 + 10 * gemm_planes_tn(nblk) + (f32out ? 1 : 0);
}

int gemm_planes(const usf_gemm_planes_desc* d, hipStream_t stream) {
  if (!d) { set_error("usf_gemm_planes_bf16x3: null descriptor"); return -1; }
  if (d->M < 0 || d->M > 0x7fffffff || d->nk <= 0 || d->a_nkb <= 0 || d->a_kb0 < 0 || d->a_kb0 + d->nk > d->a_nkb ||
      d->w_rows < 4 || d->w_rows > 0x7fffffff) {
    set_error("usf_gemm_planes_bf16x3: bad sizes (M=%lld nk=%lld a_nkb=%lld a_kb0=%lld w_rows=%lld)", (long long)d->M,
              (long long)d->nk, (long long)d->a_nkb, (long long)d->a_kb0, (long long)d->w_rows);
    return -2;
  }
  if (d->M == 0) return 0;
  const bool f32out = d->C_f32 != nullptr || d->base_part != nullptr;
  if (!d->A || !d->W_planes || (!f32out && !d->C_planes)) { set_error("usf_gemm_planes_bf16x3: null A / W / C"); return -1; }
  if (f32out && d->C_planes) { set_error("usf_gemm_planes_bf16x3: give C_planes or C_f32, not both"); return -2; }
  if (!aligned16(d->A) || !aligned16(d->W_planes) || (d->C_planes && !aligned16(d->C_planes)) ||
      (d->residual && !aligned16(d->residual)) || (d->bias && !aligned16(d->bias)) || (d->post_mul && !aligned16(d->post_mul))) {
    set_error("usf_gemm_planes_bf16x3: pointers must be 16-byte aligned");
    return -2;
  }
  if ((d->ldw & 7) || d->ldw < 32 * d->nk || (d->w_rows & 3)) { set_error("usf_gemm_planes_bf16x3: ldw must be a multiple of 8 and >= 32 nk; w_rows a multiple of 4"); return -2; }
  if (d->act != USF_ACT_NONE && d->act != USF_ACT_LEAKY_RELU) { set_error("usf_gemm_planes_bf16x3: bad act"); return -2; }
  const int64_t npanels = (d->M + 15) / 16;
  if (d->format != USF_PLANES_BF16X3 && d->format != USF_PLANES_F16X2) { set_error("usf_gemm_planes_bf16x3: unknown format %d", d->format); return -2; }
  const int64_t npl = d->format == USF_PLANES_F16X2 ? 2 : 3;
  if (npanels * d->a_nkb * npl * 1024 >= (1LL << 32) || 2 * npl * d->w_plane_stride >= (1LL << 32)) {
    set_error("usf_gemm_planes_bf16x3: operand larger than the kernel's 32-bit offsets");
    return -3;
  }
  PlArgs a;
  a.A = reinterpret_cast<const char*>(d->A); a.Wp = reinterpret_cast<const char*>(d->W_planes);
  a.bias = d->bias; a.post_mul = d->post_mul; a.R = reinterpret_cast<const char*>(d->residual);
  a.Cp = reinterpret_cast<char*>(d->C_planes); a.Cf = d->C_f32; a.ldc = d->ldc; a.plane_stride = d->w_plane_stride;
  a.ldwp = (int)d->ldw; a.wrows = (int)d->w_rows; a.M = (int)d->M; a.npanels = (int)npanels;
  a.a_nkb = (int)d->a_nkb; a.a_kb0 = (int)d->a_kb0; a.nk = (int)d->nk;
  a.c_nkb = (int)d->c_nkb; a.c_kb0 = (int)d->c_kb0; a.c_kbn = (int)d->c_kbn; a.N = (int)d->N;
  a.res_sign = d->res_sign; a.slope = d->slope; a.act = d->act; a.nbm = a.nbn = a.nvb = 0;
  a.range_flag = d->range_flag;
  a.skip_dead = (int)tuning("planes_skip_dead", 1);
  a.b_tab = d->base_tab; a.b_part = d->base_part; a.b_stride = (int)d->base_tab_stride; a.b_base = d->base;
  a.dbg = nullptr; a.span = nullptr;
  a.clk = clock_buffer();
#ifdef USF_STAMP
  a.dbg = g_pdbg; a.span = g_pspan;
  if (g_pspan) g_pspan += 2;
#endif
  int64_t nblk;
  if (f32out) {
    if (d->N <= 0 || d->N > d->w_rows || d->ldc < d->N) { set_error("usf_gemm_planes_bf16x3: bad N / ldc for fp32 output"); return -2; }
    if (d->residual) { set_error("usf_gemm_planes_bf16x3: residual needs planes output"); return -2; }
    nblk = (d->N + 31) / 32;
    if (d->base_part) {
      if (!d->base_tab || !aligned16(d->base_tab) || (d->base_tab_stride & 3) || d->base_tab_stride < ((d->N + 3) & ~(int64_t)3) ||
          d->base_tab_stride > 0x7fffffff || (d->base != USF_BASE_LAPLACE && d->base != USF_BASE_NORMAL)) {
        set_error("usf_gemm_planes_bf16x3: base density in the epilogue needs the tables of usf_base_tables_f32 (16-byte aligned, "
                  "stride a multiple of 4 and >= N) and base = USF_BASE_LAPLACE / USF_BASE_NORMAL");
        return -2;
      }
    }
  } else {
    if (d->base_part) { set_error("usf_gemm_planes_bf16x3: base_part needs the fp32-output form"); return -2; }
    if (d->c_kbn <= 0 || d->c_kb0 < 0 || d->c_kb0 + d->c_kbn > d->c_nkb || d->c_kbn * 32 > d->w_rows) {
      set_error("usf_gemm_planes_bf16x3: bad output block range (c_kb0=%lld c_kbn=%lld c_nkb=%lld w_rows=%lld)",
                (long long)d->c_kb0, (long long)d->c_kbn, (long long)d->c_nkb, (long long)d->w_rows);
      return -2;
    }
    if (npanels * d->c_nkb * npl * 1024 >= (1LL << 40)) { set_error("usf_gemm_planes_bf16x3: output too large"); return -3; }
    nblk = d->c_kbn;
  }
  const int force = (int)tuning("planes_tn", 0);
  const int tn = (force == 4 || force == 5) ? force : gemm_planes_tn(nblk);
  if (d->base_part && (d->N + 32 * tn - 1) / (32 * tn) > 8) {
    set_error("usf_gemm_planes_bf16x3: base_part holds 8 column blocks per row (N <= 1024)");
    return -2;
  }
  if (npl == 2) return tn == 4 ? launch_planes<2, 4>(a, f32out, stream) : launch_planes<2, 5>(a, f32out, stream);
  return tn == 4 ? launch_planes<3, 4>(a, f32out, stream) : launch_planes<3, 5>(a, f32out, stream);
}

}
```

### usflows_amd/engine.py

```python
from __future__ import annotations

import ctypes as C
from dataclasses import dataclass
from typing import Dict, List, Optional, Sequence, Tuple

import torch
from torch import nn

from . import _ext
from . import transforms as T
from .config import config
from ._plan_util import EngineUnsupported, _refreshed, _round_up, folded_bias
from .networks import ConditionalDenseNN, ConvNet, DenseNN
from .engine_flat import FlatPlanMixin
from .engine_planes import PlanesPlanMixin


def _activation_of(f) -> Optional[Tuple[int, float]]:
    if isinstance(f, nn.LeakyReLU):
        return _ext.ACT_LEAKY_RELU, float(f.negative_slope)
    if isinstance(f, nn.ReLU):
        return _ext.ACT_LEAKY_RELU, 0.0
    return None

# ... 140 lines not shown
                    r.update(L=out["tri"][2 * j], Ut=out["tri"][2 * j + 1], Linv=out["tri_inv"][2 * j],
                             Uinv_t=out["tri_inv"][2 * j + 1])
                res[id(l)] = r
    hh_list = list(hhs.values())
    if hh_list:
        D = int(hh_list[0].dim)
        dev = torch.device(device) if device is not None else hh_list[0].w_0.device
        Hs = torch.empty(len(hh_list), D, D, dtype=torch.float64, device=dev)
        HsT = torch.empty(len(hh_list), D, D, dtype=torch.float64, device=dev)
        zero = torch.zeros(D, dtype=torch.float64, device=dev)
        for i, h in enumerate(hh_list):
            _ext.householder(_param(h.w_0, device), _param(h.vk_householder, device), out=Hs[i])
        _ext.host_op(lambda: HsT.copy_(Hs.transpose(1, 2)))
        for i, h in enumerate(hh_list):
            res[id(h)] = dict(M=Hs[i], Minv=HsT[i], b=zero, ladj=zero.sum(), row=i)
    seq = [b for b in blocks if isinstance(b, T.SequentialAffineTransform) and id(b) not in res]
    batched = False
    if (len(seq) > 1 and len(chunks) == 1 and all(len(b.transforms) == 2 and isinstance(b.transforms[0], T.LUTransform)
                                                  and isinstance(b.transforms[1], T.HouseholderTransform) for b in seq)):
        lu_row = {id(l): j for j, l in enumerate(chunks[0]["lus"])}
        rows = [lu_row[id(b.transforms[0])] for b in seq]
        hrows = [res[id(b.transforms[1])]["row"] for b in seq]
        m = len(seq)
        if rows == list(range(rows[0], rows[0] + m)) and hrows == list(range(m)):
            out, D = chunks[0]["out"], int(seq[0].dim)
            DD, r0 = D * D, rows[0]
            f64 = lambda *shape: torch.empty(*shape, dtype=torch.float64, device=Hs.device)
            Mt, Mit, bt = f64(m, D, D), f64(m, D, D), f64(m, D)
            bat = dict(batch=m, M=D, N=D, K=D, lda=D, ldb=D, ldc=D, strideA=DD, strideB=DD, strideC=DD)
            _ext.gemm_f64(out["M"], Hs, Mt, a_off=r0 * DD, **bat)
            _ext.gemm_f64(Hs, out["Minv"], Mit, transA=True, b_off=r0 * DD, **bat)
            _ext.gemm_f64(chunks[0]["b"], Hs, bt, batch=m, M=1, N=D, K=D, lda=D, ldb=D, ldc=D, strideA=D, strideB=DD,
                          strideC=D, a_off=r0 * D)
            ct = f64(m, D)
            _ext.gemm_f64(bt, Mit, ct, batch=m, M=1, N=D, K=D, lda=D, ldb=D, ldc=D, strideA=D, strideB=DD, strideC=D, transB=True,
                          alpha=-1.0)
            for i, b in enumerate(seq):
                res[id(b)] = dict(M=Mt[i], Minv=Mit[i], b=bt[i], c=ct[i], ladj=out["ladj"][r0 + i])
            batched = True
    for b in (seq if not batched else []):
        if True:
            parts = [res[id(t)] for t in b.transforms]
            M, Minv, bias = parts[0]["M"], parts[0]["Minv"], parts[0]["b"]
            ladj = parts[0]["ladj"]
            for p_ in parts[1:]:
                M = _ext.matmul_f64(M, p_["M"])
                bm = _ext.matmul_f64(bias.reshape(1, -1), p_["M"])
                bias = _refreshed(tuple(p_["b"].shape), torch.float64, bm.device,
                                  lambda o, bm=bm, pb=p_["b"]: torch.add(bm.reshape(-1), pb, out=o))
                Minv = _ext.matmul_f64(p_["Minv"], Minv)
                ladj = _refreshed((), torch.float64, bm.device,
                                  lambda o, a=ladj, c=p_["ladj"]: torch.add(a, c, out=o))
            res[id(b)] = dict(M=M, Minv=Minv, b=bias, ladj=ladj)
            if len(parts) == 1 and "c" in parts[0]:
                res[id(b)]["c"] = parts[0]["c"]
    res["__chunks__"] = chunks
    return res


class FlowEngine(FlatPlanMixin, PlanesPlanMixin):

    def __init__(self, layers: Sequence[nn.Module]):
        self.steps = _analyze(layers)
        self.D = self._infer_dim()
        self._pack = None
        self._pack_key = None
        self._plans: Dict[tuple, dict] = {}
        self._ws: Dict[tuple, Dict[str, torch.Tensor]] = {}
        self.merge_affine = config.merge_affine
        self.merge_guard_log: List[tuple] = []
        self._virtual: List[_Step] = []
        self._virtual_ix: Dict[tuple, int] = {}
        self.launch_count = 0
        self.op_timing = None
        self.use_fused_coupling = True
        self.fused_min_rows = 14336
        self.gemm_mode = config.gemm_mode
        self.keep_factors = False
        self._f16_overflow = False
        self.f16_fallbacks = 0
        self.use_planes = config.planes
        self.planes_min_rows = int(config.planes_min_rows)
        self.planes_min_rows_bf16x3 = 24576
        self.use_train_planes = config.train_planes
        self.train_planes_min_rows = 16384
        self.ctx_planes_min_rows = None
        self.train_ctx_planes_min_rows = None
        self.use_graphs = bool(config.engine_graph)
        self.graph_max_rows = 1024
        self._layout_from_masks()

    def _infer_dim(self) -> int:
        for s in self.steps:
            if s.kind == "scale":
                return int(s.module.scale.shape[0])
            if s.kind == "affine":
                return int(s.module.dim)
            if s.kind == "coupling":
                return int(s.module.mask.shape[-1])
        raise EngineUnsupported("cannot infer dimension")

    def _layout_from_masks(self):
        D = self.D
        base = None
        self._flip = {}
        for i, s in enumerate(self.steps):
            if s.kind != "coupling":
                continue
            m = s.module.mask.detach().flatten().cpu()
            if m.numel() != D or not bool(((m == 0) | (m == 1)).all()):
                raise EngineUnsupported("coupling mask must be a 0/1 vector of length D")
            if base is None:
                base = m
            if torch.equal(m, base):
                self._flip[i] = False
            elif torch.equal(m, 1 - base):
                self._flip[i] = True
            else:
                raise EngineUnsupported("coupling masks must alternate between m and 1-m")
        if base is None:
            idx0 = torch.arange(D)
            idx1 = torch.zeros(0, dtype=torch.long)
        else:
            idx0 = torch.nonzero(base == 0).flatten()
            idx1 = torch.nonzero(base == 1).flatten()
        self.n0, self.n1 = int(idx0.numel()), int(idx1.numel())
        self.n0a, self.n1a = _round_up(self.n0, 4), _round_up(self.n1, 4)
        self.LD = max(self.n0a + self.n1a, 4)
        seg = torch.full((self.LD,), -1, dtype=torch.long)
        seg[: self.n0] = idx0
        seg[self.n0a: self.n0a + self.n1] = idx1
        self.seg_idx = seg
        self.LDn = _round_up(D, 4)
        nat = torch.full((self.LDn,), -1, dtype=torch.long)
        nat[:D] = torch.arange(D)
        self.nat_idx = nat
        self.LDp, self.LDnp = _round_up(self.LD, 32), _round_up(D, 32)
        self.segp_idx = torch.full((self.LDp,), -1, dtype=torch.long)
        self.segp_idx[: self.LD] = seg
        self.natp_idx = torch.full((self.LDnp,), -1, dtype=torch.long)
        self.natp_idx[:D] = torch.arange(D)
        self.ctx_dim = max(context_dims(self.steps), default=1)
        self.hmax = 4
        self._general_cond = False
        for s in self.steps:
            if s.kind == "coupling":
                cond = s.module.conditioner
                widths = cond.c_hidden if isinstance(cond, ConvNet) else cond.hidden_dims
                self.hmax = max(self.hmax, max(_round_up(int(h), 4) for h in widths))
                self._general_cond = self._general_cond or (isinstance(cond, ConvNet) and not cond.is_plain_mlp())

    def _params(self):
        seen, out = set(), []
        for s in self.steps:
            for p in s.module.parameters():
                if id(p) not in seen:
                    seen.add(id(p))
                    out.append(p)
        return out

    def _version_key(self, device):
        return (str(device),) + tuple((p.data_ptr(), p._version) for p in self._params())

    def refresh(self):
        self._pack, self._pack_key = None, None
        self._plans.clear()
# ... 279 lines not shown
        outs = []
        with torch.no_grad():
            for mode in (False, True):
                state[direction] = mode
                out = torch.empty(n, self.D, dtype=torch.float32, device=x.device)
                run(self._plan(direction, n, x.device, False, "user"), xs, out)
                outs.append(out.double())
            d = ((outs[1] - outs[0]).abs().max() / outs[0].abs().max().clamp_min(1e-30)).item()
            l1 = outs[0].abs().sum(-1)
            d1 = ((outs[1].abs().sum(-1) - l1).abs() / l1.clamp_min(1e-30)).max().item()
        ok = bool(d <= 1e-5 and d1 <= 1e-6)
        self.merge_guard_log.append((ok, d, d1))
        state[direction] = ok
        return ok

    def _primitive_ops(self, direction: str, merge: bool = False):
        seq = list(enumerate(self.steps))
        if direction == "backward":
            seq = seq[::-1]
        prims = []
        for i, s in seq:
            fwd = (direction == "forward") != s.inverted
            if s.kind == "scale":
                prims.append(("scale_mul" if fwd else "scale_div", i))
            elif s.kind == "affine":
                prims.append(("affine_fwd" if fwd else "affine_bwd", i))
            else:
                prims.append(("coupling_fwd" if fwd else "coupling_bwd", i))
        if not (merge and self._merge_on(direction)):
            return prims
        out, k = [], 0
        while k < len(prims):
            j = k
            while j < len(prims) and prims[j][0] in ("affine_fwd", "affine_bwd"):
                j += 1
            if j - k >= 2:
                parts = [(p_, self.steps[i_].module) for p_, i_ in prims[k:j]]
                key = tuple((p_, id(b_)) for p_, b_ in parts)
                if key not in self._virtual_ix:
                    self._virtual.append(_Step("affine", _MergedAffine(parts), False))
                    self._virtual_ix[key] = len(self.steps) + len(self._virtual) - 1
                out.append(("affine_fwd", self._virtual_ix[key]))
                k = j
            else:
                out.append(prims[k])
                k += 1
        return out

    def _affine_entry(self, pk, blk) -> dict:
        if id(blk) in pk["affine"] or not isinstance(blk, _MergedAffine):
            return pk["affine"][id(blk)]
        with self._pk_record(pk):
            _ext.flush_jobs()
            W = c = None
            for prim, b_ in blk.parts:
                a = pk["affine"][id(b_)]
                if prim == "affine_fwd":
                    Wk, ck = a["M"], a["b"]
                else:
                    Wk, ck = a["Minv"], folded_bias(a)
                if W is None:
                    W, c = Wk, ck
                else:
                    W = _ext.matmul_f64(Wk.contiguous(), W.contiguous())
                    t = torch.empty(ck.shape, dtype=torch.float64, device=ck.device)
                    _ext.matvec_f64(Wk.contiguous(), c.contiguous(), alpha=1.0, out64=t)
                    c = _refreshed(tuple(ck.shape), torch.float64, ck.device,
                                   lambda o, t=t, ck=ck: torch.add(t, ck, out=o))
            pk["affine"][id(blk)] = dict(M=W, b=c)
        return pk["affine"][id(blk)]

    def _build_plan(self, direction: str, B: int, device, has_ctx: bool, final: str, train: bool = False) -> dict:
        pk = self.pack(device)
        with self._pk_record(pk), _ext.batch_jobs(device):
            if self._planes_ok(direction, B, has_ctx, train):
                return self._build_plan_planes(direction, B, device, final, train, has_ctx)
            return self._build_plan_body(direction, B, device, has_ctx, final, train)

    def _plan(self, direction, B, device, has_ctx, final, train: bool = False):
        pk = self.pack(device)
        key = (direction, B, str(device), has_ctx, final, self.use_fused_coupling, self.gemm_mode, self.fused_min_rows,
               config.tiny_coupling, config.get_lib("coupling_tiny", 1), train, self.use_planes, self.planes_min_rows, self._planes_fmt(), self.planes_min_rows_bf16x3,
               (not train) and self._merge_on(direction), train and self.use_train_planes, train and self.train_planes_min_rows,
               has_ctx and (self.train_ctx_planes_min_rows if train else self.ctx_planes_min_rows), has_ctx and self.ctx_dim)
        plan = self._plans.get(key)
        if plan is None:
            plan = self._build_plan(direction, B, device, has_ctx, final, train)
            self._plans[key] = plan
        return plan

    def _run_guarded(self, direction, x, out, context, final):
        B = x.shape[0]
        if self.merge_affine == "auto" and context is None:
            self.resolve_merge(direction, x)
        plan = self._plan(direction, B, x.device, context is not None, final)
        self._run(plan, x, out, context)
        if plan.get("planes_fmt") == _ext.PLANES_F16X2 and int(plan["ws"]["pflag"].item()) != 0:
            plan["ws"]["pflag"].zero_()
            self.f16_fallbacks += 1
            self._f16_overflow = True
            try:
                if final.startswith("base") and not self._planes_ok(direction, B, context is not None, False):
                    return None
                plan = self._plan(direction, B, x.device, context is not None, final)
                self._run(plan, x, out, context)
            finally:
                self._f16_overflow = False
        return plan

    def _run(self, plan, x: torch.Tensor, out: Optional[torch.Tensor], context):
        ws = plan["ws"]
        ws["_gen"] = ws.get("_gen", 0) + 1
        self._execute(plan, x, out, context)

    def _execute(self, plan, x: torch.Tensor, out: Optional[torch.Tensor], context):
        if (self.use_graphs and x.shape[0] <= self.graph_max_rows and self.op_timing is None
                and not torch.cuda.is_current_stream_capturing()):
            return self._execute_graph(plan, x, out, context)
        return self._execute_plain(plan, x, out, context)

    def _execute_graph(self, plan, x, out, context):
        ws = plan["ws"]
        B = x.shape[0]
        if "x_static" not in ws:
            ws["x_static"] = torch.empty(B, self.D, dtype=torch.float32, device=x.device)
        xs = ws["x_static"]
        xs.copy_(x)
        os_ = None
        if out is not None:
            if "out_static" not in ws:
                ws["out_static"] = torch.empty(B, self.D, dtype=torch.float32, device=x.device)
            os_ = ws["out_static"]
        if context is not None:
            self._fill_context(plan, context, B)
        g = plan.get("graph")
        if g is None:
            if plan.get("graph_warm", 0) < 1:
                plan["graph_warm"] = 1
                self._execute_plain(plan, xs, os_, None)
            else:
                torch.cuda.synchronize(x.device)
                g = torch.cuda.CUDAGraph()
                with _ext.capture_without_gc(), torch.cuda.graph(g):
                    self._execute_plain(plan, xs, os_, None)
                plan["graph"] = g
                g.replay()
        else:
            g.replay()
            self.launch_count += 1
        if out is not None:
            out.copy_(os_)

    def _fill_context(self, plan, context, B: int):
        ws = plan["ws"]
        Cd = self.ctx_dim
        if Cd > 1:
            if tuple(context.shape) not in ((B, Cd), (1, Cd), (Cd,)):
                raise ValueError(f"context of shape {tuple(context.shape)}: a context_dim {Cd} flow takes [{B}, {Cd}], [1, {Cd}] "
                                 f"or [{Cd}] for {B} rows")
            ws["ctx4"][:, :Cd].copy_(context.reshape(-1, Cd).expand(B, Cd))
            return
        c = context.reshape(-1).to(torch.float32)
        if c.numel() == 1 and B > 1:
            c = c.expand(B)
        ws["ctx4"][:, 0].copy_(c)
        ws["ctx"].copy_(c)

    def _execute_plain(self, plan, x: torch.Tensor, out: Optional[torch.Tensor], context):
        ws = plan["ws"]
        B = x.shape[0]
        dev = x.device
        if context is not None:
            self._fill_context(plan, context, B)
        arr = plan["arr"]
        for idx, member, field in plan["patch_in"]:
            setattr(getattr(arr[idx].u, member), field, x.data_ptr())
        for idx, member, field in plan["patch_out"]:
            setattr(getattr(arr[idx].u, member), field, out.data_ptr())
        lib = _ext.load()
        stream = _ext.current_stream(dev)
        pos = 0

        def run_until(end):
            nonlocal pos
            if end > pos and self.op_timing is not None:
                j = pos
                while j < end:
                    op = arr[j]
                    n_run = 2 if _ext.is_ctx_prefix(op) else 1
                    if n_run == 2 and arr[j + 1].kind == _ext.OP_COUPLING:
                        c_ = arr[j + 1].u.coupling
                        tag = ("coupling_vctx", c_.M, c_.n_trans, c_.n_pass)
                    elif n_run == 2:
                        c_ = arr[j + 1].u.coupling_planes
                        tag = ("coupling_planes_ctx", c_.M, 32 * c_.nk_t, 32 * c_.nk_p)
                    elif op.kind == _ext.OP_LINEAR:
                        kind = "linear_bf16x3" if op.u.linear.W_split else "linear"
                        tag = (kind, op.u.linear.M, op.u.linear.N, op.u.linear.K)
                    elif op.kind == _ext.OP_GEMM_PLANES:
                        g_ = op.u.gemm_planes
                        tag = ("gemm_planes", g_.M, g_.N if g_.C_f32 else 32 * g_.c_kbn, 32 * g_.nk)
                    elif op.kind == _ext.OP_PACK_PLANES:
                        tag = ("pack_planes", op.u.pack_planes.M, 32 * op.u.pack_planes.nkb, 0)
                    elif op.kind == _ext.OP_COUPLING_PLANES:
                        c_ = op.u.coupling_planes
                        tag = ("coupling_planes", c_.M, 32 * c_.nk_t, 32 * c_.nk_p)
                    else:
                        tag = ("coupling", op.u.coupling.M, op.u.coupling.n_trans, op.u.coupling.n_pass)
                    e0, e1 = torch.cuda.Event(enable_timing=True), torch.cuda.Event(enable_timing=True)
                    e0.record()
                    sub = C.cast(C.byref(arr, j * C.sizeof(_ext.Op)), C.POINTER(_ext.Op))
                    _ext.check(lib.usf_run_ops(sub, n_run, stream), "usf_run_ops")
                    e1.record()
                    self.op_timing.append((tag, e0, e1))
                    j += n_run
                self.launch_count += 1
                pos = end
            elif end > pos:
                sub = C.cast(C.byref(arr, pos * C.sizeof(_ext.Op)), C.POINTER(_ext.Op))
                _ext.check(lib.usf_run_ops(sub, end - pos, stream), "usf_run_ops")
                self.launch_count += 1
                pos = end

        for g in plan["side"]:
            run_until(g[1])
            if g[0] == "scale":
                _, _, buf, ld, sc, divide, ncols = g
                _ext.scale(ws[buf], ld, ws[buf], ld, B, ncols, sc, divide)
                self.launch_count += 1
            else:
                _, _, src, dst_name, dst_layout = g
                src_t = x if src[0] == "user_in" else ws[src[0]]
                idx = self._gather_index(src[1], dst_layout, dev)
                dst_t = ws[dst_name]
                _ext.gather_cols(src_t, src[2], dst_t, dst_t.shape[1], B, dst_t.shape[1], idx)
                self.launch_count += 1
        run_until(plan["n"])
        fg = plan["final_gather"]
        if fg is not None:
            src, dst_name = fg
            src_t = ws[src[0]]
            if dst_name == "user_out":
                _ext.gather_cols(src_t, src[2], out, self.D, B, self.D, self._gather_index(src[1], "user", dev))
            else:
                _ext.gather_cols(src_t, src[2], ws[dst_name], self.LDn, B, self.LDn,
                                 self._gather_index(src[1], "nat", dev))
            self.launch_count += 1

    def _gather_index(self, src_layout: str, dst_layout: str, device) -> torch.Tensor:
        key = ("gidx", src_layout, dst_layout, str(device))
        cache = self.__dict__.setdefault("_gidx", {})
        if key not in cache:
            src_idx = self._idx(src_layout)
            pos = {int(f): c for c, f in enumerate(src_idx.tolist()) if f >= 0}
            if dst_layout == "user":
                feats = list(range(self.D))
            else:
                feats = self._idx(dst_layout).tolist()
            cache[key] = torch.tensor([pos[f] if f >= 0 else -1 for f in feats], dtype=torch.int32, device=device)
        return cache[key]

    def _check_input(self, x: torch.Tensor) -> torch.Tensor:
        if not x.is_cuda:
            raise RuntimeError("FlowEngine runs on ROCm devices only")
        if x.dim() != 2 or x.shape[1] != self.D:
            raise ValueError(f"expected input of shape [B, {self.D}], got {tuple(x.shape)}")
        if x.dtype != torch.float32:
            x = x.float()
        if not x.is_contiguous() or (x.data_ptr() % 16) != 0:
            x = x.contiguous().clone() if (x.data_ptr() % 16) != 0 else x.contiguous()
        return x

    def transform(self, x: torch.Tensor, direction: str, context: Optional[torch.Tensor] = None) -> torch.Tensor:
        x = self._check_input(x)
        B = x.shape[0]
        out = torch.empty(B, self.D, dtype=torch.float32, device=x.device)
# ... 34 lines not shown
```

### usflows_amd/engine_planes.py

```python
from __future__ import annotations

from typing import List

import torch

from . import _ext
from ._plan_util import EngineUnsupported, _image_triple, _refreshed, _round_up, affine_span, arange_padded, folded_bias
from .networks import ConditionalDenseNN, ConvNet, DenseNN


class PlanesPlanMixin:

    @staticmethod
    def _slot_feature(s_: int) -> int:
        return 16 * ((s_ & 7) >> 2) + 4 * (s_ >> 3) + (s_ & 3)

    def _phys(self, logical: torch.Tensor) -> torch.Tensor:
        n = int(logical.numel())
        perm = torch.tensor([32 * (c // 32) + self._slot_feature(c % 32) for c in range(n)], dtype=torch.long)
        return logical[perm]

    def _planes_fmt(self) -> int:
        return _ext.PLANES_F16X2 if (self.gemm_mode == "f16x2" and not self._f16_overflow) else _ext.PLANES_BF16X3

# ... 116 lines not shown
        for at, j in enumerate(reversed(range(n)) if backward else range(n)):
            role = "in" if at == 0 else ("out" if at == n - 1 else "hid")
            jkey = (i, j) if role == "hid" else (i,)
            out_sel, in_sel = (ends[j], ends[j + 1]) if backward else (ends[j + 1], ends[j])
            mats.append(self._planes_image(pk, (f"pl_c{role}_t" if backward else f"pl_c{role}",) + jkey, layers[j][0], out_sel,
                                           self._phys(in_sel), fmt, transpose=backward))
            vecs.append(zeros if backward else self._planes_vec(pk, (f"pl_c{role}b",) + jkey, layers[j][1], out_sel))
        f = dict(W_in=mats[0], hid=mats[1:-1], W_out=mats[-1], b_in=vecs[0], b_hid=vecs[1:-1], b_out=vecs[-1])
        if backward:
            f["zeros"] = zeros
        return f

    def planes_dgrad_image(self, pk, m) -> torch.Tensor:
        blk = m["blk"]
        which = "Minv" if m["prim"] == "affine_bwd" else "M"
        out_phys = self._phys(self.natp_idx if m["out_layout"] == "natp" else self.segp_idx)
        return self._planes_image(pk, ("pl_aff_t", id(blk), which, m["out_layout"]), self._affine_entry(pk, blk)[which],
                                  self.segp_idx, out_phys, _ext.PLANES_BF16X3, transpose=True)

    def planes_coupling_bwd(self, pk, m) -> dict:
        cp = pk["coupling"][m["step"]]
        if "planes_bwd" not in cp:
            cp["planes_bwd"] = self._coupling_planes_images(pk, m["step"], m, _ext.PLANES_BF16X3, backward=True)
        return cp["planes_bwd"]

    def planes_coupling_bwd_op(self, pk, m, g, g_nkb: int, B: int, gates, d_out) -> _ext.Op:
        cp = pk["coupling"][m["step"]]
        return coupling_planes_op(g, g_nkb, B, (m["kb_t0"], m["nk_t"], m["kb_p0"], m["nk_p"]),
                                  self.planes_coupling_bwd(pk, m), m["sign"], cp["slope"], _ext.ACT_GATE, _ext.PLANES_BF16X3, 0,
                                  gate=gates[::-1], hidden_out=d_out[::-1])

    def _build_plan_planes(self, direction: str, B: int, device, final: str, train: bool = False, has_ctx: bool = False) -> dict:
        p = _PlanesPlan(self, direction, B, device, final, train, has_ctx)
        k = p.head()
        while k < len(p.prims):
            prim, i = p.prims[k]
            k += p.affine(k, prim, i) if prim in ("affine_fwd", "affine_bwd") else p.coupling(prim, i)
        return p.result()


def coupling_planes_op(z, z_nkb: int, B: int, ranges, f: dict, sign, slope, act, fmt, flag, gate=(), hidden_out=()) -> _ext.Op:
    op = _ext.Op()
    op.kind = _ext.OP_COUPLING_PLANES
    c = op.u.coupling_planes
    c.z, c.z_nkb, c.M = z.data_ptr(), z_nkb, B
    c.kb_p0, c.nk_p, c.kb_t0, c.nk_t = ranges
    c.n_hidden, c.hidden_padded = len(f["hid"]) + 1, 256
    c.W_in, c.ldw_in, c.w_in_plane = _image_triple(f["W_in"])
    c.b_in = f["b_in"].data_ptr()
    for j, (Wh, bh) in enumerate(zip(f["hid"], f["b_hid"])):
        c.W_hid[j], c.ldw_hid, c.w_hid_plane = _image_triple(Wh)
        c.b_hid[j] = bh.data_ptr()
    c.W_out, c.ldw_out, c.w_out_plane = _image_triple(f["W_out"])
    c.b_out = f["b_out"].data_ptr()
    c.sign, c.slope, c.act, c.format, c.range_flag = sign, slope, act, fmt, flag
    for l, t in enumerate(gate):
        c.gate[l] = t.data_ptr()
    for l, t in enumerate(hidden_out):
        c.hidden_out[l] = t.data_ptr()
    return op


class _PlanesPlan:

    def __init__(self, eng, direction: str, B: int, device, final: str, train: bool, has_ctx: bool):
        self.eng, self.B, self.device, self.final, self.train, self.has_ctx = eng, B, device, final, train, has_ctx
        self.pk = eng.pack(device)
        ws = self.ws = eng._workspace(B, device)
        self.prims = eng._primitive_ops(direction, merge=not train)
        self.nkb = eng.LDp // 32
        self.seg_phys = eng._phys(eng.segp_idx)
        self.fmt = eng._planes_fmt()
        if "pflag" not in ws:
            ws["pflag"] = torch.zeros(1, dtype=torch.int32, device=device)
        self.flag = ws["pflag"].data_ptr() if self.fmt == _ext.PLANES_F16X2 else 0
        self.z_name, self.other_name = ("pz0", None) if train else ("pzA", "pzB")
        self.z = self.planes_buf(self.z_name, self.nkb)
        self.other = None if train else self.planes_buf(self.other_name, self.nkb)
        self.n_z = 1
        self.ops: List[_ext.Op] = []
        self.meta: List[dict] = []
        self.patch_in, self.patch_out = [], []
        self.head_scale, self.bias_in_head, self.out_buf = None, False, None

    def planes_buf(self, name: str, blocks: int) -> torch.Tensor:
        ws, n = self.ws, (-(-self.B // 16)) * blocks * 3072
        if name not in ws or ws[name].numel() < n:
            ws[name] = torch.empty(n, dtype=torch.uint8, device=self.device)
        return ws[name]

    def gemm_op(self, W: torch.Tensor, **kw) -> _ext.Op:
        op = _ext.Op()
        op.kind = _ext.OP_GEMM_PLANES
        g = op.u.gemm_planes
        g.M, g.res_sign, g.slope, g.act = self.B, 1.0, 0.0, _ext.ACT_NONE
        g.format, g.range_flag = self.fmt, self.flag
        g.W_planes, g.ldw, g.w_plane_stride = _image_triple(W)
        g.w_rows = W.shape[1]
        for k_, v_ in kw.items():
            setattr(g, k_, v_)
        return op

    def head(self) -> int:
        e, pk, prims = self.eng, self.pk, self.prims
        segp = e.segp_idx
        pack = _ext.Op()
        pack.kind = _ext.OP_PACK_PLANES
        d = pack.u.pack_planes
        d.src, d.ld, d.M, d.nkb = 0, e.D, self.B, self.nkb
        d.src_cols = e.D
        d.format, d.range_flag = self.fmt, self.flag
        d.idx = e._idx_dev("segp", self.device).data_ptr()
        d.planes = self.z.data_ptr()
        k = 0
        if prims[0][0] == "scale_div":
            self.head_scale = s0 = e._step(prims[0][1]).module
            d.pre_div = e._planes_vec(pk, ("pl_scale", id(s0), "segp"), pk["scale"][id(s0)], segp, 1.0).data_ptr()
            if prims[1][0] == "affine_bwd":
                blk = e._step(prims[1][1]).module
                d.pre_sub = e._planes_vec(pk, ("pl_b", id(blk), "segp"), pk["affine"][id(blk)]["b"], segp).data_ptr()
                self.bias_in_head = True
            k = 1
        self.patch_in.append((len(self.ops), "pack_planes", "src"))
        self.ops.append(pack)
        return k

    def affine(self, k: int, prim: str, i: int) -> int:
        e, pk, nkb = self.eng, self.pk, self.nkb
        blk = e._step(i).module
        a = e._affine_entry(pk, blk)
        fuse_post, is_last, taken = affine_span(self.prims, k)
        is_head = len(self.ops) == 1
        lay, out_sel = ("natp", e.natp_idx) if is_last else ("segp", e.segp_idx)
        if self.train:
            self.meta.append(dict(kind="affine", op=len(self.ops), prim=prim, blk=blk, in_buf=self.z_name, in_layout="segp",
                                  out_layout=lay, N=e.D if is_last else e.LD, K=e.LD,
                                  pre_scale=self.head_scale if is_head else None, post_scale=None,
                                  pre_sub_folded=bool(is_head and self.bias_in_head), is_last=is_last))
        which = "Minv" if prim == "affine_bwd" else "M"
        W = e._planes_image(pk, ("pl_aff", id(blk), which, is_last), a[which], out_sel, self.seg_phys, self.fmt)
        kw = dict(A=self.z.data_ptr(), a_nkb=nkb, a_kb0=0, nk=nkb)
        if prim == "affine_fwd":
            kw["bias"] = e._planes_vec(pk, ("pl_b", id(blk), lay), a["b"], out_sel).data_ptr()
        elif not (is_head and self.bias_in_head):
            kw["bias"] = e._planes_vec(pk, ("pl_c", id(blk), lay), folded_bias(a), out_sel).data_ptr()
        if is_last:
            if fuse_post:
                s2 = e._step(self.prims[k + 1][1]).module
                kw["post_mul"] = e._planes_vec(pk, ("pl_scale", id(s2), "natp"), pk["scale"][id(s2)], e.natp_idx, 1.0).data_ptr()
            self._final_store(kw)
        else:
            if self.train:
                self.other_name = f"pz{self.n_z}"
                self.other = self.planes_buf(self.other_name, nkb)
                self.n_z += 1
            kw.update(C_planes=self.other.data_ptr(), c_nkb=nkb, c_kb0=0, c_kbn=nkb)
            self.z, self.z_name, self.other, self.other_name = self.other, self.other_name, self.z, self.z_name
        if self.train:
            self.meta[-1]["out_buf"] = self.out_buf[0] if is_last else self.z_name
        self.ops.append(self.gemm_op(W, **kw))
        return taken

    def _final_store(self, kw: dict) -> None:
        e, ws, B, final = self.eng, self.ws, self.B, self.final
        if final == "user":
            kw.update(C_f32=0, ldc=e.D, N=e.D)
            self.patch_out.append((len(self.ops), "gemm_planes", "C_f32"))
            self.out_buf = ("user_out", "nat", e.D)
        elif final.startswith("base"):
            stride = _round_up(e.D, 4)
            if "btab" not in ws:
                ws["btab"] = torch.zeros(3 * stride, dtype=torch.float32, device=self.device)
                ws["bpart"] = torch.zeros(B, 8, dtype=torch.float32, device=self.device)
            kw.update(C_f32=0, ldc=e.D, N=e.D, base_tab=ws["btab"].data_ptr(), base_tab_stride=stride,
                      base_part=ws["bpart"].data_ptr(), base=int(final[4:]))
            self.out_buf = ("bpart", "part", 8)
        else:
            kw.update(C_f32=e._nat2(ws, B, self.device).data_ptr(), ldc=e.LDn, N=e.D)
            self.out_buf = ("nat2", "nat", e.LDn)

    def coupling(self, prim: str, i: int) -> int:
        e = self.eng
        cp = self.pk["coupling"][i]
        geo = e._coupling_geometry(cp)
        sign = 1.0 if prim == "coupling_fwd" else -1.0
        use_ctx = bool(self.has_ctx and cp["has_ctx"])
        if e._planes_coupling_fused(list(cp["raw"]["h"]), self.B, self.fmt):
            self._coupling_fused(i, cp, geo, sign, use_ctx)
        elif self.train or use_ctx:
            raise EngineUnsupported("training / a context on the planes pipeline needs the fused coupling launch")
        else:
            self._coupling_chained(i, cp, geo, sign)
        return 1

    def _coupling_fused(self, i: int, cp: dict, geo: dict, sign: float, use_ctx: bool) -> None:
        e, pk, ws = self.eng, self.pk, self.ws
        raw = cp["raw"]
        f = e._coupling_planes_images(pk, i, geo, self.fmt)
        if use_ctx:
            Wc, bc = raw["ctx"]
            rows0 = arange_padded(raw["h"][0], 256)
            w_ctx = e._planes_vec(pk, ("pl_cctxw", i), Wc, rows0)
            b_ctx = e._planes_vec(pk, ("pl_cctxb", i), bc, rows0)
            self.ops.append(_ext.coupling_planes_ctx_prefix(ws["ctx"], 1, w_ctx, b_ctx))
        hnames = [f"pHs{j}_{i}" for j in range(len(raw["h"]))] if self.train else []
        op = coupling_planes_op(self.z, self.nkb, self.B, (geo["kb_p0"], geo["nk_p"], geo["kb_t0"], geo["nk_t"]), f, sign,
                                cp["slope"], cp["act"], self.fmt, self.flag, hidden_out=[self.planes_buf(hn, 8) for hn in hnames])
        if self.train:
            self.meta.append(dict(kind="coupling", op=len(self.ops), step=i, buf=self.z_name, sign=sign, use_ctx=use_ctx,
                                  hidden_planes=hnames, **geo))
        self.ops.append(op)

    def _coupling_chained(self, i: int, cp: dict, geo: dict, sign: float) -> None:
        e, pk, z, nkb = self.eng, self.pk, self.z, self.nkb
        raw = cp["raw"]
        h = list(raw["h"])
        layers = [raw["first"]] + list(raw["hidden"]) + [raw["last"]]
        hkb = _round_up(e.hmax, 32) // 32
        hbufs = [self.planes_buf("pH1", hkb), self.planes_buf("pH2", hkb)]
        src = dict(A=z.data_ptr(), a_nkb=nkb, a_kb0=geo["kb_p0"], nk=geo["nk_p"])
        in_sel = geo["feat_p"][32 * geo["kb_p0"]: 32 * (geo["kb_p0"] + geo["nk_p"])]
        for j, (W_, b_) in enumerate(layers):
            last = j == len(layers) - 1
            if last:
                out_sel = geo["feat_t"][32 * geo["kb_t0"]: 32 * (geo["kb_t0"] + geo["nk_t"])]
                dst = dict(C_planes=z.data_ptr(), c_nkb=nkb, c_kb0=geo["kb_t0"], c_kbn=geo["nk_t"], residual=z.data_ptr(), res_sign=sign)
            else:
                hj = _round_up(h[j], 32)
                out_sel = arange_padded(h[j], hj)
                buf = hbufs[j % 2]
                dst = dict(C_planes=buf.data_ptr(), c_nkb=hkb, c_kb0=0, c_kbn=hj // 32, act=cp["act"], slope=cp["slope"])
            Wimg = e._planes_image(pk, ("pl_mlp", i, j), W_, out_sel, e._phys(in_sel), self.fmt)
            bvec = e._planes_vec(pk, ("pl_mlpb", i, j), b_, out_sel)
            self.ops.append(self.gemm_op(Wimg, bias=bvec.data_ptr(), **src, **dst))
            if not last:
                src, in_sel = dict(A=buf.data_ptr(), a_nkb=hkb, a_kb0=0, nk=hj // 32), out_sel

    def result(self) -> dict:
        ops, out_buf = self.ops, self.out_buf
        arr = (_ext.Op * len(ops))(*ops)
        n_part = 0
        if out_buf[1] == "part":
            tn = (_ext.load().usf_gemm_planes_variant(arr[len(ops) - 1].u.gemm_planes) - 5000) // 10
            n_part = -(-self.eng.D // (32 * tn))
        return dict(arr=arr, n=len(ops), patch_in=self.patch_in, patch_out=self.patch_out, side=[], final_gather=None,
                    n_part=n_part, out_buf=out_buf, ws=self.ws, pk=self.pk, meta=self.meta, planes=True, planes_fmt=self.fmt,
                    planes_train=bool(self.train), has_ctx=bool(self.has_ctx))
```

Measured before the change: 3.479 million samples/s.

## Pass coupling residual as fp32 side buffer from preceding planes GEMM

The planes GEMM that comes before a fused coupling now also writes the transformed-half blocks as packed fp32 into a side buffer. The coupling kernel then reads its residual from that buffer (two f32x4 loads) instead of loading and summing the 2 or 3 bf16/f16 split planes. This cuts the coupling's residual-load work and summing, but adds extra fp32 writes in the GEMM epilogue, plus a workspace buffer and new kernel template variants. It is enabled by default for inference at 8192 rows or more without context.

```diff
diff --git a/__graft_entry__.py b/__graft_entry__.py
--- a/__graft_entry__.py
+++ b/__graft_entry__.py
@@ -37,6 +37,7 @@
     assert torch.isfinite(xs).all()
     eng = flow.engine()
     rels = {}
+    eng.planes_side_min_rows = 0
     for mode in ("bf16x3", "f16x2"):
         eng.gemm_mode, eng.use_planes, eng.planes_min_rows, eng.fused_min_rows = mode, True, 0, 0
         with torch.no_grad():
diff --git a/include/usflows_hip_internal.h b/include/usflows_hip_internal.h
--- a/include/usflows_hip_internal.h
+++ b/include/usflows_hip_internal.h
@@ -30,6 +30,12 @@
 #define USF_FN_COUPLING_PLANES_CTX 64
 int usf_coupling_planes_ctx(const usf_coupling_planes_desc* d, const float* ctx, int64_t ctx_stride, const float* w_ctx,
                             const float* b_ctx, usf_stream_t stream);
+
+#define USF_FN_GEMM_PLANES_SIDE 66
+#define USF_FN_COUPLING_PLANES_SIDE 67
+int usf_gemm_planes_side(const usf_gemm_planes_desc* d, void* side, int64_t side_kb0, int64_t side_kbn, int64_t both_kb0,
+                         int64_t both_kbn, usf_stream_t stream);
+int usf_coupling_planes_side(const usf_coupling_planes_desc* d, const void* side, int64_t side_nkb, usf_stream_t stream);
 
 #define USF_VCTX_MAX 32
 #define USF_FN_COUPLING_VCTX 65
diff --git a/usflows_amd/_abi.py b/usflows_amd/_abi.py
--- a/usflows_amd/_abi.py
+++ b/usflows_amd/_abi.py
@@ -17,6 +17,8 @@
 
 FN_COUPLING_PLANES_CTX = 64
 FN_COUPLING_VCTX = 65
+FN_GEMM_PLANES_SIDE = 66
+FN_COUPLING_PLANES_SIDE = 67
 VCTX_MAX = 32
 
 _fp = C.c_void_p
@@ -289,6 +291,8 @@
                                              _fp, C.c_uint64, C.c_uint64, C.c_int64, C.c_void_p]),
     "usf_gated_norm_rows_bwd_f32": (C.c_int, [C.POINTER(GatedNormBwdDesc), C.c_void_p]),
     "usf_coupling_planes_ctx": (C.c_int, [C.POINTER(CouplingPlanesDesc), _fp, C.c_int64, _fp, _fp, C.c_void_p]),
+    "usf_gemm_planes_side": (C.c_int, [C.POINTER(GemmPlanesDesc), _fp, C.c_int64, C.c_int64, C.c_int64, C.c_int64, C.c_void_p]),
+    "usf_coupling_planes_side": (C.c_int, [C.POINTER(CouplingPlanesDesc), _fp, C.c_int64, C.c_void_p]),
     "usf_coupling_additive_vctx_f32": (C.c_int, [C.POINTER(CouplingDesc), _fp, C.c_int64, C.c_int32, _fp, C.c_int64, _fp, C.c_void_p]),
     "usf_coupling_additive_vctx_variant": (C.c_int, [C.POINTER(CouplingDesc), C.c_int32]),
     "usf_conv_ctx_wgrad_f32": (C.c_int, [_fp, _fp, C.c_int64, C.c_int64, C.c_int64, C.c_int64, C.c_int64, C.c_int64, _fp, C.c_void_p]),
diff --git a/usflows_amd/_ext.py b/usflows_amd/_ext.py
--- a/usflows_amd/_ext.py
+++ b/usflows_amd/_ext.py
@@ -16,7 +16,7 @@
     USF_ABI_VERSION, USF_INTERNAL_VERSION, USF_MAX_HIDDEN, ACT_NONE, ACT_LEAKY_RELU, ACT_GATE, BASE_LAPLACE, BASE_NORMAL,
     BASE_LPNORM1, BASE_LPNORM2, BASE_LPNORMINF, BASE_ROWSUM, NORM_LOGNORMAL, NORM_GAMMA, NORM_RAW_PARAMS, NORM_WEIBULL, NORM_HALFNORMAL, NORM_CHI, RADIAL_MAX_K, OP_LINEAR,
     OP_COUPLING, OP_PACK_PLANES, OP_GEMM_PLANES, OP_COUPLING_PLANES, OP_GATED_NORM, OP_CALL, PLANES_BF16X3, PLANES_F16X2, CALL_FNS,
-    FN_COUPLING_PLANES_CTX, FN_COUPLING_VCTX, VCTX_MAX,
+    FN_COUPLING_PLANES_CTX, FN_COUPLING_VCTX, FN_GEMM_PLANES_SIDE, FN_COUPLING_PLANES_SIDE, VCTX_MAX,
     _fp, LinearDesc, CouplingDesc, PackPlanesDesc, GemmPlanesDesc, CouplingPlanesDesc, MtChunk, AdamChunk, GradChunk, ConvVariantQuery, ConvVariant, ConvWgradQuery, ConvWgradInfo, LnBwdInfo, CONV_ENTRIES, GatedNormDesc, GatedNormBwdDesc,
     CallDesc, _OpUnion, Op, LuPrepDesc, PackJob, PsumJob, WgradJob, WReduceJob, WPlanesJob, GradJob, SIZEOF_KINDS, PUBLIC_SYMBOLS,
     INTERNAL_SYMBOLS, SYMBOLS)
@@ -974,6 +974,36 @@
     return op.kind == OP_CALL and op.u.call.fn in (FN_COUPLING_PLANES_CTX, FN_COUPLING_VCTX)
 
 
+def gemm_planes_side_op(op, side, side_kb0, side_kbn, both_kb0, both_kbn, device):
+    _launch("usf_gemm_planes_side", (C.byref(op.u.gemm_planes), ptr(side), int(side_kb0), int(side_kbn), int(both_kb0), int(both_kbn),
+                                     current_stream(device)), (op, side))
+
+
+def coupling_planes_side_op(op, side, side_nkb, device):
+    _launch("usf_coupling_planes_side", (C.byref(op.u.coupling_planes), ptr(side), int(side_nkb), current_stream(device)), (op, side))
+
+
+def _side_prefix(fn: int, words) -> "Op":
+    op = Op()
+    op.kind = OP_CALL
+    op.u.call.fn, op.u.call.n_args = fn, len(words)
+    for j, w in enumerate(words):
+        op.u.call.a[j] = w
+    return op
+
+
+def gemm_planes_side_prefix(side, side_kb0, side_kbn, both_kb0, both_kbn) -> "Op":
+    return _side_prefix(FN_GEMM_PLANES_SIDE, (side.data_ptr(), int(side_kb0), int(side_kbn), int(both_kb0), int(both_kbn)))
+
+
+def coupling_planes_side_prefix(side, side_nkb) -> "Op":
+    return _side_prefix(FN_COUPLING_PLANES_SIDE, (side.data_ptr(), int(side_nkb)))
+
+
+def is_side_prefix(op) -> bool:
+    return op.kind == OP_CALL and op.u.call.fn in (FN_GEMM_PLANES_SIDE, FN_COUPLING_PLANES_SIDE)
+
+
 def run_ops(ops_array, n, device=None):
     _launch("usf_run_ops", (ops_array, n, current_stream(device)), tape=False)
 
diff --git a/usflows_amd/config.py b/usflows_amd/config.py
--- a/usflows_amd/config.py
+++ b/usflows_amd/config.py
@@ -17,6 +17,7 @@
 class Config:
     _KNOBS = dict(
         planes_min_rows=8192,
+        planes_side_f32=True,
         base_in_epilogue=True,
         tiny_coupling=True,
         engine_graph=False,
diff --git a/usflows_amd/csrc/usf_api.hip b/usflows_amd/csrc/usf_api.hip
--- a/usflows_amd/csrc/usf_api.hip
+++ b/usflows_amd/csrc/usf_api.hip
@@ -84,6 +84,9 @@
 int coupling_planes(const usf_coupling_planes_desc* d, hipStream_t stream);
 int coupling_planes_ctx(const usf_coupling_planes_desc* d, const float* ctx, int64_t ctx_stride, const float* w_ctx, const float* b_ctx,
                         hipStream_t stream);
+int gemm_planes_side(const usf_gemm_planes_desc* d, void* side, int64_t side_kb0, int64_t side_kbn, int64_t both_kb0, int64_t both_kbn,
+                     hipStream_t stream);
+int coupling_planes_side(const usf_coupling_planes_desc* d, const void* side, int64_t side_nkb, hipStream_t stream);
 int lu_prepare(const usf_lu_prep_desc* d, hipStream_t stream);
 int gemm_f64(const double* A, int64_t lda, int64_t sA, int transA, const double* B, int64_t ldb, int64_t sB, int transB,
              double* C, int64_t ldc, int64_t sC, int64_t M, int64_t N, int64_t K, int64_t batch, double alpha,
@@ -263,6 +266,15 @@
                             usf_stream_t stream) {
   return usf::coupling_planes_ctx(d, ctx, ctx_stride, w_ctx, b_ctx, (hipStream_t)stream);
 }
+int usf_gemm_planes_side(const usf_gemm_planes_desc* d, void* side, int64_t side_kb0, int64_t side_kbn, int64_t both_kb0,
+                         int64_t both_kbn, usf_stream_t stream) {
+  if (!side) { usf::set_error("usf_gemm_planes_side: null side buffer"); return -1; }
+  return usf::gemm_planes_side(d, side, side_kb0, side_kbn, both_kb0, both_kbn, (hipStream_t)stream);
+}
+int usf_coupling_planes_side(const usf_coupling_planes_desc* d, const void* side, int64_t side_nkb, usf_stream_t stream) {
+  if (!side) { usf::set_error("usf_coupling_planes_side: null side buffer"); return -1; }
+  return usf::coupling_planes_side(d, side, side_nkb, (hipStream_t)stream);
+}
 int usf_gemm_planes_variant(const usf_gemm_planes_desc* d) { return usf::gemm_planes_variant(d); }
 int usf_coupling_variant(const usf_coupling_desc* d) { return usf::coupling_variant(d); }
 int usf_coupling_additive_vctx_f32(const usf_coupling_desc* d, const float* ctx, int64_t ld_ctx, int32_t ctx_dim, const float* W_ctx_t,
@@ -698,6 +710,25 @@
           ++i;
           break;
         }
+        if (ops[i].u.call.fn == USF_FN_GEMM_PLANES_SIDE || ops[i].u.call.fn == USF_FN_COUPLING_PLANES_SIDE) {
+          const usf_call_desc* c = &ops[i].u.call;
+          const bool gemm = c->fn == USF_FN_GEMM_PLANES_SIDE;
+          if (c->n_args != (gemm ? 5 : 2) || i + 1 >= n_ops || ops[i + 1].kind != (gemm ? USF_OP_GEMM_PLANES : USF_OP_COUPLING_PLANES)) {
+            usf::set_error("usf_run_ops: op %d (%s) needs %d arguments and a %s op behind it", i,
+                           gemm ? "USF_FN_GEMM_PLANES_SIDE" : "USF_FN_COUPLING_PLANES_SIDE", gemm ? 5 : 2,
+                           gemm ? "USF_OP_GEMM_PLANES" : "USF_OP_COUPLING_PLANES");
+            return -2;
+          }
+          void* side = reinterpret_cast<void*>((uintptr_t)c->a[0]);
+          if (!side) { usf::set_error("usf_run_ops: op %d carries a null side buffer", i); return -1; }
+          if (gemm)
+            rc = usf::gemm_planes_side(&ops[i + 1].u.gemm_planes, side, (int64_t)c->a[1], (int64_t)c->a[2], (int64_t)c->a[3],
+                                       (int64_t)c->a[4], (hipStream_t)stream);
+          else
+            rc = usf::coupling_planes_side(&ops[i + 1].u.coupling_planes, side, (int64_t)c->a[1], (hipStream_t)stream);
+          ++i;
+          break;
+        }
         rc = run_call(&ops[i].u.call, stream);
         break;
       default: usf::set_error("usf_run_ops: op %d has unknown kind %d", i, ops[i].kind); return -2;
diff --git a/usflows_amd/csrc/usf_coupling_planes.hip b/usflows_amd/csrc/usf_coupling_planes.hip
--- a/usflows_amd/csrc/usf_coupling_planes.hip
+++ b/usflows_amd/csrc/usf_coupling_planes.hip
@@ -1,4 +1,6 @@
 #include <stdlib.h>
+
+#include <type_traits>
 
 #include "usf_common.h"
 
@@ -83,6 +85,7 @@
   unsigned long long* dbg;
   char* hout[2]; const char* gate[2];
   const float* ctx; int ctx_stride; const float* w_ctx; const float* b_ctx;
+  const char* side;
 };
 
 #ifdef USF_STAMP
@@ -91,8 +94,9 @@
 #define CSTAMP(v)
 #endif
 
-template <int NPL, int NH, int MODE = 0, bool CTX = false>
+template <int NPL, int NH, int MODE = 0, bool CTX = false, bool SIDE = false>
 __global__ __launch_bounds__(512, 2) void coupling_planes_kernel(const CplPArgs p) {
+  static_assert(!SIDE || (MODE == 0 && !CTX), "the fp32 residual serves the plain inference launch");
   typedef CPlanes<NPL> PT;
   typedef typename PT::vec vec8;
   constexpr int T = 16;
@@ -360,14 +364,22 @@
     vec8 xp[KS][NPL];
 #pragma unroll
     for (int ks = 0; ks < KS; ++ks) { PT::split(X[2 * ks], X[2 * ks + 1], xp[ks]); save_hidden(NH - 1, ks, xp[ks]); }
-    vec8 res[NPL];
+    typename std::conditional<SIDE, f32x4, vec8>::type res[SIDE ? 2 : NPL];
     f32x4 bo[2];
+    unsigned soff = (unsigned)lane * 32u;
+    const char* const srow = SIDE ? p.side + ((size_t)panc * p.nk_t) * 2048u : nullptr;
     auto issue_res = [&](int nt) {
       if constexpr (A32) { cp_pin(loff); cp_pin(goff); }
-#pragma unroll
-      for (int q = 0; q < NPL; ++q) {
-        if constexpr (A32) res[q] = cp_load<vec8>(zrow + ((size_t)(p.kb_t0 + nt) * CHB + q * 1024), loff);
-        else res[q] = *reinterpret_cast<const vec8*>(p.z + zbase + (size_t)(p.kb_t0 + nt) * CHB + q * 1024);
+      if constexpr (SIDE) {
+        if constexpr (A32) cp_pin(soff);
+#pragma unroll
+        for (int u = 0; u < 2; ++u) res[u] = cp_load<f32x4>(srow + ((size_t)nt * 2048u + 16 * u), soff);
+      } else {
+#pragma unroll
+        for (int q = 0; q < NPL; ++q) {
+          if constexpr (A32) res[q] = cp_load<vec8>(zrow + ((size_t)(p.kb_t0 + nt) * CHB + q * 1024), loff);
+          else res[q] = *reinterpret_cast<const vec8*>(p.z + zbase + (size_t)(p.kb_t0 + nt) * CHB + q * 1024);
+        }
       }
 #pragma unroll
       for (int u = 0; u < 2; ++u) {
@@ -381,8 +393,13 @@
       for (int u = 0; u < 2; ++u) {
 #pragma unroll
         for (int e = 0; e < 4; ++e) {
-          float r = (float)rs[0][4 * u + e] + (float)rs[1][4 * u + e];
-          if (NPL == 3) r = r + (float)rs[NPL - 1][4 * u + e];
+          float r;
+          if constexpr (SIDE) {
+            r = rs[u][e];
+          } else {
+            r = (float)rs[0][4 * u + e] + (float)rs[1][4 * u + e];
+            if (NPL == 3) r = r + (float)rs[NPL - 1][4 * u + e];
+          }
           v[u][e] = __builtin_fmaf(p.sign, ac[u][e], r);
         }
         guard(v[u]);
@@ -420,7 +437,7 @@
       for (int i = 0; i < 2 * KS; ++i) {
         __builtin_amdgcn_sched_group_barrier(0x008, NPR, 0);
         if (i + AHEAD < 2 * KS) __builtin_amdgcn_sched_group_barrier(0x100, NPL, 0);
-        if (i < NST + NPL + 2) __builtin_amdgcn_sched_group_barrier(0x020, 1, 0);
+        if (i < NST + (SIDE ? 2 : NPL) + 2) __builtin_amdgcn_sched_group_barrier(0x020, 1, 0);
       }
       __builtin_amdgcn_sched_barrier(0);
       store_n(buf ^ 1, st);
@@ -449,8 +466,8 @@
 unsigned long long* g_cdbg = nullptr;
 #endif
 
-int coupling_planes_ctx(const usf_coupling_planes_desc* d, const float* ctx, int64_t ctx_stride, const float* w_ctx,
-                        const float* b_ctx, hipStream_t stream) {
+static int coupling_planes_launch(const usf_coupling_planes_desc* d, const float* ctx, int64_t ctx_stride, const float* w_ctx,
+                                  const float* b_ctx, const void* side, int64_t side_nkb, hipStream_t stream) {
   if (!d) { set_error("usf_coupling_planes: null descriptor"); return -1; }
   if (ctx) {
     if (d->act == USF_ACT_GATE) { set_error("usf_coupling_planes_ctx: USF_ACT_GATE takes no context (the context enters no data gradient)"); return -2; }
@@ -493,7 +510,20 @@
       return -3;
     }
   }
+  if (side) {
+    if (ctx || d->hidden_out[0] || d->hidden_out[1] || d->act == USF_ACT_GATE) {
+      set_error("usf_coupling_planes_side: the fp32 residual serves the inference launch without a context (no hidden_out, no USF_ACT_GATE)");
+      return -2;
+    }
+    if (!aligned16(side)) { set_error("usf_coupling_planes_side: side must be 16-byte aligned"); return -2; }
+    if (side_nkb != d->nk_t) {
+      set_error("usf_coupling_planes_side: the side buffer holds %lld blocks per panel, the layer transforms %lld", (long long)side_nkb, (long long)d->nk_t);
+      return -2;
+    }
+    if (npanels * d->nk_t * 2048 >= (1LL << 32)) { set_error("usf_coupling_planes_side: side buffer of 4 GiB or more"); return -3; }
+  }
   CplPArgs a;
+  a.side = reinterpret_cast<const char*>(side);
   a.z = reinterpret_cast<char*>(d->z); a.z_nkb = (int)d->z_nkb; a.npanels = (int)npanels; a.M = (int)d->M;
   a.kb_p0 = (int)d->kb_p0; a.nk_p = (int)d->nk_p; a.kb_t0 = (int)d->kb_t0; a.nk_t = (int)d->nk_t;
   a.Win = reinterpret_cast<const char*>(d->W_in); a.ld_in = d->ldw_in; a.pl_in = d->w_in_plane; a.b_in = d->b_in;
@@ -542,7 +572,14 @@
   const dim3 block(512);
 #define USF_CPL(NPL_, NH_) hipLaunchKernelGGL((coupling_planes_kernel<NPL_, NH_>), grid, block, 0, stream, a)
 #define USF_CPLC(NPL_, NH_) hipLaunchKernelGGL((coupling_planes_kernel<NPL_, NH_, 0, true>), grid, block, 0, stream, a)
-  if (ctx) {
+#define USF_CPLS(NPL_, NH_) hipLaunchKernelGGL((coupling_planes_kernel<NPL_, NH_, 0, false, true>), grid, block, 0, stream, a)
+  if (side) {
+    if (npl == 2) {
+      switch (d->n_hidden) { case 1: USF_CPLS(2, 1); break; case 2: USF_CPLS(2, 2); break; default: USF_CPLS(2, 3); break; }
+    } else {
+      switch (d->n_hidden) { case 1: USF_CPLS(3, 1); break; case 2: USF_CPLS(3, 2); break; default: USF_CPLS(3, 3); break; }
+    }
+  } else if (ctx) {
     if (npl == 2) {
       switch (d->n_hidden) { case 1: USF_CPLC(2, 1); break; case 2: USF_CPLC(2, 2); break; default: USF_CPLC(2, 3); break; }
     } else {
@@ -553,11 +590,21 @@
   } else {
     switch (d->n_hidden) { case 1: USF_CPL(3, 1); break; case 2: USF_CPL(3, 2); break; default: USF_CPL(3, 3); break; }
   }
+#undef USF_CPLS
 #undef USF_CPLC
 #undef USF_CPL
   return check_launch("usf_coupling_planes");
 }
 
+int coupling_planes_ctx(const usf_coupling_planes_desc* d, const float* ctx, int64_t ctx_stride, const float* w_ctx,
+                        const float* b_ctx, hipStream_t stream) {
+  return coupling_planes_launch(d, ctx, ctx_stride, w_ctx, b_ctx, nullptr, 0, stream);
+}
+
+int coupling_planes_side(const usf_coupling_planes_desc* d, const void* side, int64_t side_nkb, hipStream_t stream) {
+  return coupling_planes_launch(d, nullptr, 0, nullptr, nullptr, side, side_nkb, stream);
+}
+
 int coupling_planes(const usf_coupling_planes_desc* d, hipStream_t stream) { return coupling_planes_ctx(d, nullptr, 0, nullptr, nullptr, stream); }
 
 }
diff --git a/usflows_amd/csrc/usf_planes.hip b/usflows_amd/csrc/usf_planes.hip
--- a/usflows_amd/csrc/usf_planes.hip
+++ b/usflows_amd/csrc/usf_planes.hip
@@ -226,12 +226,13 @@
   int32_t* range_flag;
   int skip_dead;
   const float* b_tab; float* b_part; int b_stride; int b_base;
+  char* S; int s_kb0, s_kbn, s_both0, s_bothn;
   unsigned long long* clk;
   unsigned long long* dbg;
   unsigned long long* span;
 };
 
-template <int NPL, int TN, bool F32OUT>
+template <int NPL, int TN, bool F32OUT, bool SIDE = false>
 __global__ __launch_bounds__(512, 2) void gemm_planes_kernel(const PlArgs p) {
   typedef Planes<NPL> PT;
   typedef typename PT::vec vec8;
@@ -530,6 +531,8 @@
 #pragma unroll
     for (int t = 0; t < TN; ++t) {
       const int kbo = bn * TN + t;
+      const bool to_side = SIDE && (unsigned)(kbo - p.s_kb0) < (unsigned)p.s_kbn;
+      const bool to_planes = !to_side || (unsigned)(kbo - p.s_both0) < (unsigned)p.s_bothn;
 #pragma unroll
       for (int b = 0; b < 2; ++b) {
         if (kbo < p.c_kbn && pw[b] < p.npanels) {
@@ -537,6 +540,28 @@
           float x[8];
 #pragma unroll
           for (int u = 0; u < 8; ++u) x[u] = acc[2 * t + (u >> 2)][b][u & 3];
+          if constexpr (SIDE) {
+            if (to_side) {
+              const unsigned soff = ((unsigned)pw[b] * (unsigned)p.s_kbn + (unsigned)(kbo - p.s_kb0)) * 2048u + (unsigned)lane * 32u;
+              f32x4 s0 = {x[0], x[1], x[2], x[3]}, s1 = {x[4], x[5], x[6], x[7]};
+              if constexpr (NPL == 2) {
+                bool sb = false;
+#pragma unroll
+                for (int u = 0; u < 8; ++u) sb = sb || (16 * pw[b] + lj < p.M && !(fabsf(x[u]) < USF_F16_GUARD));
+                bad = bad || sb;
+                vec8 so[NPL];
+                PT::split(x, so);
+#pragma unroll
+                for (int u = 0; u < 4; ++u) {
+                  s0[u] = (float)so[0][u] + (float)so[1][u];
+                  s1[u] = (float)so[0][4 + u] + (float)so[1][4 + u];
+                }
+              }
+              *reinterpret_cast<f32x4*>(p.S + soff) = s0;
+              *reinterpret_cast<f32x4*>(p.S + (soff + 16u)) = s1;
+            }
+            if (!to_planes) continue;
+          }
           if (p.R) {
             vec8 r[NPL];
 #pragma unroll
@@ -600,6 +625,7 @@
 
 template <int NPL, int TN>
 static int launch_planes(PlArgs a, bool f32out, hipStream_t stream) {
+  const bool side = a.S != nullptr;
   constexpr int BN = TN * 32;
   a.nbm = (a.npanels + 15) / 16;
   a.nbn = f32out ? (a.N + BN - 1) / BN : (a.c_kbn + TN - 1) / TN;
@@ -611,6 +637,7 @@
   cus = (cus / 8) * 8 > 0 ? (cus / 8) * 8 : 8;
   if (persist && grid > cus) grid = cus;
   if (f32out) hipLaunchKernelGGL((gemm_planes_kernel<NPL, TN, true>), dim3((unsigned)grid), dim3(512), 0, stream, a);
+  else if (side) hipLaunchKernelGGL((gemm_planes_kernel<NPL, TN, false, true>), dim3((unsigned)grid), dim3(512), 0, stream, a);
   else hipLaunchKernelGGL((gemm_planes_kernel<NPL, TN, false>), dim3((unsigned)grid), dim3(512), 0, stream, a);
   return check_launch("usf_gemm_planes");
 }
@@ -628,7 +655,8 @@
   return 5000 + 10 * gemm_planes_tn(nblk) + (f32out ? 1 : 0);
 }
 
-int gemm_planes(const usf_gemm_planes_desc* d, hipStream_t stream) {
+int gemm_planes_side(const usf_gemm_planes_desc* d, void* side, int64_t side_kb0, int64_t side_kbn, int64_t both_kb0,
+                     int64_t both_kbn, hipStream_t stream) {
   if (!d) { set_error("usf_gemm_planes_bf16x3: null descriptor"); return -1; }
   if (d->M < 0 || d->M > 0x7fffffff || d->nk <= 0 || d->a_nkb <= 0 || d->a_kb0 < 0 || d->a_kb0 + d->nk > d->a_nkb ||
       d->w_rows < 4 || d->w_rows > 0x7fffffff) {
@@ -666,6 +694,20 @@
   a.skip_dead = (int)tuning("planes_skip_dead", 1);
   a.b_tab = d->base_tab; a.b_part = d->base_part; a.b_stride = (int)d->base_tab_stride; a.b_base = d->base;
   a.dbg = nullptr; a.span = nullptr;
+  a.S = nullptr; a.s_kb0 = a.s_kbn = a.s_both0 = a.s_bothn = 0;
+  if (side) {
+    if (f32out || d->residual) { set_error("usf_gemm_planes_side: the side output needs planes output and no residual"); return -2; }
+    if (!aligned16(side)) { set_error("usf_gemm_planes_side: side must be 16-byte aligned"); return -2; }
+    if (side_kbn <= 0 || side_kb0 < 0 || side_kb0 + side_kbn > d->c_kbn || both_kbn < 0 ||
+        (both_kbn > 0 && (both_kb0 < side_kb0 || both_kb0 + both_kbn > side_kb0 + side_kbn))) {
+      set_error("usf_gemm_planes_side: bad block ranges (side %lld + %lld of c_kbn=%lld, both %lld + %lld)", (long long)side_kb0,
+                (long long)side_kbn, (long long)d->c_kbn, (long long)both_kb0, (long long)both_kbn);
+      return -2;
+    }
+    if (npanels * side_kbn * 2048 >= (1LL << 32)) { set_error("usf_gemm_planes_side: side buffer larger than the kernel's 32-bit offsets"); return -3; }
+    a.S = reinterpret_cast<char*>(side); a.s_kb0 = (int)side_kb0; a.s_kbn = (int)side_kbn;
+    a.s_both0 = (int)both_kb0; a.s_bothn = (int)both_kbn;
+  }
   a.clk = clock_buffer();
 #ifdef USF_STAMP
   a.dbg = g_pdbg; a.span = g_pspan;
@@ -704,4 +746,6 @@
   return tn == 4 ? launch_planes<3, 4>(a, f32out, stream) : launch_planes<3, 5>(a, f32out, stream);
 }
 
-}
+int gemm_planes(const usf_gemm_planes_desc* d, hipStream_t stream) { return gemm_planes_side(d, nullptr, 0, 0, 0, 0, stream); }
+
+}
diff --git a/usflows_amd/engine.py b/usflows_amd/engine.py
--- a/usflows_amd/engine.py
+++ b/usflows_amd/engine.py
@@ -246,6 +246,8 @@
         self.use_planes = config.planes
         self.planes_min_rows = int(config.planes_min_rows)
         self.planes_min_rows_bf16x3 = 24576
+        self.planes_side_f32 = bool(config.planes_side_f32)
+        self.planes_side_min_rows = 8192
         self.use_train_planes = config.train_planes
         self.train_planes_min_rows = 16384
         self.ctx_planes_min_rows = None
@@ -691,7 +693,8 @@
         key = (direction, B, str(device), has_ctx, final, self.use_fused_coupling, self.gemm_mode, self.fused_min_rows,
                config.tiny_coupling, config.get_lib("coupling_tiny", 1), train, self.use_planes, self.planes_min_rows, self._planes_fmt(), self.planes_min_rows_bf16x3,
                (not train) and self._merge_on(direction), train and self.use_train_planes, train and self.train_planes_min_rows,
-               has_ctx and (self.train_ctx_planes_min_rows if train else self.ctx_planes_min_rows), has_ctx and self.ctx_dim)
+               has_ctx and (self.train_ctx_planes_min_rows if train else self.ctx_planes_min_rows), has_ctx and self.ctx_dim,
+               (not train) and self.planes_side_f32 and B >= self.planes_side_min_rows)
         plan = self._plans.get(key)
         if plan is None:
             plan = self._build_plan(direction, B, device, has_ctx, final, train)
@@ -797,10 +800,13 @@
                 while j < end:
                     op = arr[j]
                     n_run = 2 if _ext.is_ctx_prefix(op) else 1
-                    if n_run == 2 and arr[j + 1].kind == _ext.OP_COUPLING:
+                    side = _ext.is_side_prefix(op)
+                    if side:
+                        n_run, op = 2, arr[j + 1]
+                    if n_run == 2 and not side and arr[j + 1].kind == _ext.OP_COUPLING:
                         c_ = arr[j + 1].u.coupling
                         tag = ("coupling_vctx", c_.M, c_.n_trans, c_.n_pass)
-                    elif n_run == 2:
+                    elif n_run == 2 and not side:
                         c_ = arr[j + 1].u.coupling_planes
                         tag = ("coupling_planes_ctx", c_.M, 32 * c_.nk_t, 32 * c_.nk_p)
                     elif op.kind == _ext.OP_LINEAR:
diff --git a/usflows_amd/engine_planes.py b/usflows_amd/engine_planes.py
--- a/usflows_amd/engine_planes.py
+++ b/usflows_amd/engine_planes.py
@@ -222,6 +222,7 @@
         self.meta: List[dict] = []
         self.patch_in, self.patch_out = [], []
         self.head_scale, self.bias_in_head, self.out_buf = None, False, None
+        self.side_for = None
 
     def planes_buf(self, name: str, blocks: int) -> torch.Tensor:
         ws, n = self.ws, (-(-self.B // 16)) * blocks * 3072
@@ -296,10 +297,40 @@
                 self.n_z += 1
             kw.update(C_planes=self.other.data_ptr(), c_nkb=nkb, c_kb0=0, c_kbn=nkb)
             self.z, self.z_name, self.other, self.other_name = self.other, self.other_name, self.z, self.z_name
+            self._side_output(k + taken)
         if self.train:
             self.meta[-1]["out_buf"] = self.out_buf[0] if is_last else self.z_name
         self.ops.append(self.gemm_op(W, **kw))
         return taken
+
+    def side_range(self, k: int):
+        e = self.eng
+        if self.train or not e.planes_side_f32 or self.B < e.planes_side_min_rows or k >= len(self.prims):
+            return None
+        prim, i = self.prims[k]
+        if prim not in ("coupling_fwd", "coupling_bwd"):
+            return None
+        cp = self.pk["coupling"][i]
+        if (self.has_ctx and cp["has_ctx"]) or not e._planes_coupling_fused(list(cp["raw"]["h"]), self.B, self.fmt):
+            return None
+        geo = e._coupling_geometry(cp)
+        t0, t1 = geo["kb_t0"], geo["kb_t0"] + geo["nk_t"]
+        b0, b1 = max(t0, geo["kb_p0"]), min(t1, geo["kb_p0"] + geo["nk_p"])
+        return (i, t0, t1 - t0, b0, b1 - b0) if b1 > b0 else (i, t0, t1 - t0, t0, 0)
+
+    def _side_output(self, k: int) -> None:
+        self.side_for = None
+        r = self.side_range(k)
+        if r is None:
+            return
+        i, t0, nt, b0, nb = r
+        ws = self.ws
+        nmax = max(self.eng._coupling_geometry(cp)["nk_t"] for cp in self.pk["coupling"].values())
+        n = (-(-self.B // 16)) * nmax * 2048
+        if "pside" not in ws or ws["pside"].numel() < n:
+            ws["pside"] = torch.empty(n, dtype=torch.uint8, device=self.device)
+        self.ops.append(_ext.gemm_planes_side_prefix(ws["pside"], t0, nt, b0, nb))
+        self.side_for = (i, nt)
 
     def _final_store(self, kw: dict) -> None:
         e, ws, B, final = self.eng, self.ws, self.B, self.final
@@ -349,6 +380,9 @@
         if self.train:
             self.meta.append(dict(kind="coupling", op=len(self.ops), step=i, buf=self.z_name, sign=sign, use_ctx=use_ctx,
                                   hidden_planes=hnames, **geo))
+        if self.side_for == (i, geo["nk_t"]) and not use_ctx:
+            self.ops.append(_ext.coupling_planes_side_prefix(ws["pside"], geo["nk_t"]))
+        self.side_for = None
         self.ops.append(op)
 
     def _coupling_chained(self, i: int, cp: dict, geo: dict, sign: float) -> None:
```

After: 3.522 million samples/s, median of 6. 1.01x the previous value.
